# danielmtzbarba/carlabev-env

Hardware: NVIDIA B200
Metric: env-steps/sec (obs+reward+done) at N envs, 1/2/4/8 B200; % HBM roofline (higher is better)
Workload: dtype f64

## Files before the change

carlabev_env_b200/csrc/api.cu:

```cuda
#include <cuda.h>
#include <math.h>
#include <stdarg.h>
#include <stdio.h>
#include <stdlib.h>
#include <string.h>

#include <algorithm>
#include <chrono>
#include <cmath>
#include <new>
#include <random>
#include <vector>

#include "engine.h"

static thread_local char g_err[512] = "";

void cbev_set_error(const char* fmt, ...) {
  va_list ap;
  va_start(ap, fmt);
  vsnprintf(g_err, sizeof(g_err), fmt, ap);
  va_end(ap);
}

// ... 105 lines not shown
      cbev_set_error("cuTensorMapEncodeTiled failed with CUresult %d (map %dx%d, box %dx%d)", (int)r, e->map_w, e->map_h,
                     (int)box[0], (int)box[1]);
      return CBEV_ERR_CUDA;
    }
  }
  return CBEV_OK;
}

}

static int use_device(cbev_handle e) {
  if (!e) { cbev_set_error("null handle"); return CBEV_ERR_ARG; }
  int cur = -1;
  if (cudaGetDevice(&cur) != cudaSuccess || cur != e->device) CU_TRY(cudaSetDevice(e->device));
  return CBEV_OK;
}

static int install_pool(cbev_engine* e, PoolDev& d, const int32_t* actor_off_host, bool live) {
  const int n = d.n_scenes;
  const size_t na = (size_t)d.n_actors_total;
  const int max_retreat = d.max_retreat, max_tl = d.max_tl;
  int rc = 0;
  const size_t Rn = (size_t)(max_retreat ? max_retreat : 1), Ro = (size_t)(e->pool.max_retreat ? e->pool.max_retreat : 1);
  const int32_t new_max_rects = e->cfg.max_actors + CBEV_MAX_TARGETS + max_tl + 1;
  uint32_t* rects = nullptr;
  double* retreat = nullptr;
  int32_t* retreat_n = nullptr;
  const bool grow_rects = !e->rects || new_max_rects > e->max_rects;
  const bool grow_retreat = !e->st.retreat || !live || Rn != Ro;
  if (grow_rects) rc |= dev_alloc(&rects, (size_t)e->N * CBEV_RECT_WORDS * new_max_rects);
  if (grow_retreat) {
    rc |= dev_alloc(&retreat, (size_t)e->N * Rn * 3 * CBEV_SG_MAX);
    rc |= dev_alloc(&retreat_n, (size_t)e->N * Rn);
    if (!rc && live && e->st.retreat) {
      const size_t row_o = Ro * 3 * CBEV_SG_MAX * sizeof(double), row_n = Rn * 3 * CBEV_SG_MAX * sizeof(double);
      if (cudaMemcpy2D(retreat, row_n, e->st.retreat, row_o, row_o, (size_t)e->N, cudaMemcpyDeviceToDevice) != cudaSuccess ||
          cudaMemcpy2D(retreat_n, Rn * sizeof(int32_t), e->st.retreat_n, Ro * sizeof(int32_t), Ro * sizeof(int32_t),
                       (size_t)e->N, cudaMemcpyDeviceToDevice) != cudaSuccess) {
        cbev_set_error("copying the retreat routes failed");
        rc = CBEV_ERR_CUDA;
      }
    }
  }
  int T = live ? e->pool.traj_steps : e->cfg.trajectory_steps;
  if (!rc && T > 0 && na > 0) {
    const size_t budget = (size_t)4 << 30;
    if (!live) {
      while (T > 16 && (size_t)T * na * sizeof(double4) > budget) T /= 2;
    } else if ((size_t)T * na * sizeof(double4) > 2 * budget) {
      cbev_set_error("the extended pool needs %zu bytes of trajectory tables at the %d steps fixed by the first upload",
                     (size_t)T * na * sizeof(double4), T);
      rc = CBEV_ERR_NOMEM;
    }
    std::vector<long long> off((size_t)n);
    long long acc = 0;
    for (int s2 = 0; s2 < n; ++s2) {
      off[s2] = acc;
      acc += (long long)T * (actor_off_host[s2 + 1] - actor_off_host[s2]);
    }
    const size_t S = (size_t)n, A = (size_t)(e->cfg.max_actors > 0 ? e->cfg.max_actors : 1);
    EnvState& r = d.roll;
    if (!rc) {
      rc |= dev_upload(&d.traj_off, off.data(), S);
      rc |= dev_alloc(&d.traj, (size_t)acc);
      rc |= dev_alloc(&r.ax, S * A); rc |= dev_alloc(&r.ay, S * A); rc |= dev_alloc(&r.ayaw, S * A);
      rc |= dev_alloc(&r.av, S * A); rc |= dev_alloc(&r.atarget_mps, S * A); rc |= dev_alloc(&r.aelapsed, S * A);
      rc |= dev_alloc(&r.astate_elapsed, S * A); rc |= dev_alloc(&r.atidx, S * A); rc |= dev_alloc(&r.arxlen, S * A);
      rc |= dev_alloc(&r.aflags, S * A);
      rc |= dev_alloc(&r.retreat, S * Rn * 3 * CBEV_SG_MAX);
      rc |= dev_alloc(&r.retreat_n, S * Rn);
    }
    if (!rc) d.traj_steps = T;
  }
  if (rc) {
    free_pool(d);
    dev_free(rects); dev_free(retreat); dev_free(retreat_n);
    return rc;
  }
  free_pool(e->pool);
  e->pool = d;
  if (grow_rects) { dev_free(e->rects); e->rects = rects; e->max_rects = new_max_rects; }
  if (grow_retreat) { dev_free(e->st.retreat); dev_free(e->st.retreat_n); e->st.retreat = retreat; e->st.retreat_n = retreat_n; }
  e->has_pool = true;
  if (!live) e->pool_epoch += 1;
  if (e->pool.traj_steps > 0) {
    cbev_launch_rollout(e, 0);
    cudaError_t ce = cudaDeviceSynchronize();
    if (ce != cudaSuccess) {
      cbev_set_error("trajectory roll-out failed: %s", cudaGetErrorString(ce));
      e->has_pool = false;
      return CBEV_ERR_CUDA;
    }
  }
  return CBEV_OK;
}

extern "C" {

int cbev_version(void) { return CBEV_VERSION; }
const char* cbev_last_error(void) { return g_err; }

static void area_table(int ssize, int dsize, std::vector<int32_t>& off, std::vector<int32_t>& si,
                       std::vector<float>& alpha) {
  const double scale = (double)ssize / dsize;
  off.assign(1, 0);
  for (int dx = 0; dx < dsize; ++dx) {
    const double fsx1 = dx * scale, fsx2 = fsx1 + scale;
    const double cell = std::min(scale, ssize - fsx1);
    int sx1 = (int)std::ceil(fsx1), sx2 = (int)std::floor(fsx2);
    sx2 = std::min(sx2, ssize - 1);
    sx1 = std::min(sx1, sx2);
    if (sx1 - fsx1 > 1e-3) { si.push_back(sx1 - 1); alpha.push_back((float)((sx1 - fsx1) / cell)); }
    for (int sx = sx1; sx < sx2; ++sx) { si.push_back(sx); alpha.push_back((float)(1.0 / cell)); }
    if (fsx2 - sx2 > 1e-3) {
      si.push_back(sx2);
      alpha.push_back((float)(std::min(std::min(fsx2 - sx2, 1.0), cell) / cell));
    }
    off.push_back((int32_t)si.size());
  }
}

static void linear_area_table(int ssize, int dsize, std::vector<int32_t>& ofs, std::vector<int32_t>& a0,
                              std::vector<int32_t>& a1) {
  const double scale = (double)ssize / dsize, inv = 1.0 / scale;
  for (int dx = 0; dx < dsize; ++dx) {
    int sx = (int)std::floor(dx * scale);
    float fx = (float)((dx + 1) - (sx + 1) * inv);
    fx = fx <= 0 ? 0.f : fx - std::floor(fx);
    if (sx >= ssize - 1) { fx = 0.f; sx = ssize - 1; }
    ofs.push_back(sx);
    a0.push_back((int32_t)std::lrintf((1.f - fx) * 2048.f));
    a1.push_back((int32_t)std::lrintf(fx * 2048.f));
  }
}

static int build_resize_tables(cbev_engine* e) {
  const int S = e->cfg.fov_size, oh = e->cfg.obs_h, ow = e->cfg.obs_w;
  e->rs_words = 0;
  if (e->cfg.obs_mode == CBEV_OBS_RGB) { e->rs_mode = CBEV_RS_FAST96; return CBEV_OK; }
  if (oh > S || ow > S) {
    e->rs_mode = CBEV_RS_LINEAR;
    std::vector<int32_t> xo, xa0, xa1, yo, yb0, yb1, tab(2, 0);
    linear_area_table(S, ow, xo, xa0, xa1);
    linear_area_table(S, oh, yo, yb0, yb1);
    bool unit = true;
    for (size_t i = 0; i < xa0.size(); ++i) unit = unit && xa0[i] + xa1[i] == 2048;
    for (size_t i = 0; i < yb0.size(); ++i) unit = unit && yb0[i] + yb1[i] == 2048;
    tab[0] = unit ? 1 : 0;
    for (auto* v : {&xo, &yo, &xa0, &xa1, &yb0, &yb1}) tab.insert(tab.end(), v->begin(), v->end());
    e->rs_words = (int32_t)tab.size();
    return dev_upload(&e->rs_tab, tab.data(), tab.size());
  }
  if (S == 128 && oh == 96 && ow == 96) e->rs_mode = CBEV_RS_FAST96;
  else if (oh == S && ow == S) e->rs_mode = CBEV_RS_COPY;
  else if (2 * oh == S && 2 * ow == S) e->rs_mode = CBEV_RS_HALF;
  else e->rs_mode = CBEV_RS_TABLE;
  std::vector<int32_t> xo, yo, xs, ys;
  std::vector<float> xa, ya;
  area_table(S, ow, xo, xs, xa);
  area_table(S, oh, yo, ys, ya);
  std::vector<int32_t> tab;
  tab.push_back((int32_t)xs.size());
  tab.push_back((int32_t)ys.size());
  tab.insert(tab.end(), xo.begin(), xo.end());
  tab.insert(tab.end(), yo.begin(), yo.end());
  tab.insert(tab.end(), xs.begin(), xs.end());
  tab.insert(tab.end(), ys.begin(), ys.end());
  for (float a : xa) { int32_t b; memcpy(&b, &a, 4); tab.push_back(b); }
  for (float a : ya) { int32_t b; memcpy(&b, &a, 4); tab.push_back(b); }
  for (int d = 0; d < ow; ++d) tab.push_back(xs[xo[d]]);
  for (int d = 0; d < ow; ++d) tab.push_back(xs[xo[d + 1] - 1]);
  for (int d = 0; d < oh; ++d) tab.push_back(ys[yo[d]]);
  for (int d = 0; d < oh; ++d) tab.push_back(ys[yo[d + 1] - 1]);
  e->rs_words = (int32_t)tab.size();
  return dev_upload(&e->rs_tab, tab.data(), tab.size());
}

int cbev_create(const cbev_config* cfg, cbev_handle* out) {
  if (!cfg || !out) { cbev_set_error("null argument"); return CBEV_ERR_ARG; }
  *out = nullptr;
  if (cfg->num_envs < 1) { cbev_set_error("num_envs must be >= 1"); return CBEV_ERR_ARG; }
  if (cfg->fov_size != 64 && cfg->fov_size != 128 && cfg->fov_size != 256) {
    cbev_set_error("size must be 64, 128 or 256 (Town01 map scales the reference can reset on), got %d", cfg->fov_size);
    return CBEV_ERR_ARG;
  }
  if (cfg->obs_mode < 0 || cfg->obs_mode > 3) { cbev_set_error("bad obs_mode %d", cfg->obs_mode); return CBEV_ERR_ARG; }
  const bool masks = cfg->obs_mode == CBEV_OBS_SEMANTIC || cfg->obs_mode == CBEV_OBS_SEMANTIC_U8;
  if (cfg->obs_mode != CBEV_OBS_RGB) {
    const int px = cfg->obs_h * cfg->obs_w;
    const int mult = cfg->obs_mode == CBEV_OBS_SEMANTIC ? 4 : 16;
    if (cfg->obs_h < 8 || cfg->obs_w < 8 || cfg->obs_h > 256 || cfg->obs_w > 256 || px % mult != 0) {
      cbev_set_error("obs_size must be within 8..256 per side with height*width a multiple of %d (%s), got (%d, %d)",
                     mult, mult == 4 ? "float32 masks" : "16-byte stores of uint8 planes", cfg->obs_h, cfg->obs_w);
      return CBEV_ERR_ARG;
    }
  }
  if (masks && channels_of(cfg->mask_mode) < 0) { cbev_set_error("bad mask_mode %d", cfg->mask_mode); return CBEV_ERR_ARG; }
  if (cfg->frame_stack < 1) { cbev_set_error("frame_stack must be >= 1"); return CBEV_ERR_ARG; }
  if (!(cfg->anchor_x_frac >= 0.0 && cfg->anchor_x_frac <= 1.0 && cfg->anchor_y_frac >= 0.0 && cfg->anchor_y_frac <= 1.0)) {
    cbev_set_error("ego anchor fractions must be within [0, 1]");
    return CBEV_ERR_ARG;
  }
  const int F = cfg->obs_mode == CBEV_OBS_RGB ? 1 : cfg->frame_stack;
  if (F > 1 && cfg->ring_slots < 2 * F - 1) { cbev_set_error("ring_slots must be >= 2*frame_stack-1 (%d), got %d", 2 * F - 1, cfg->ring_slots); return CBEV_ERR_ARG; }
  if (F == 1 && cfg->ring_slots < 1) { cbev_set_error("ring_slots must be >= 1"); return CBEV_ERR_ARG; }
  if (cfg->action_mode == CBEV_ACTION_DISCRETE && (cfg->n_discrete < 1 || cfg->n_discrete > 16)) { cbev_set_error("n_discrete must be in [1, 16]"); return CBEV_ERR_ARG; }
  if (cfg->max_actors < 0) { cbev_set_error("max_actors must be >= 0"); return CBEV_ERR_ARG; }

  cbev_engine* e = new (std::nothrow) cbev_engine();
  if (!e) return CBEV_ERR_NOMEM;
  e->cfg = *cfg;
  e->cfg.frame_stack = F;
  if (F == 1) e->cfg.ring_slots = 1;
  e->N = cfg->num_envs;
  cudaGetDevice(&e->device);
  const int m = cfg->fov_size - 1;
  int ax = (int)nearbyint((double)m * cfg->anchor_x_frac), ay = (int)nearbyint((double)m * cfg->anchor_y_frac);
  ax = ax < 0 ? 0 : (ax > m ? m : ax);
  ay = ay < 0 ? 0 : (ay > m ? m : ay);
  e->anchor_x = ax;
  e->anchor_y = ay;
  int mx = ax > m - ax ? ax : m - ax, my = ay > m - ay ? ay : m - ay;
  int crop = (int)ceil(2.0 * hypot((double)mx, (double)my));
  if (crop < cfg->fov_size) crop = cfg->fov_size;
  e->crop = crop;
  e->pad = crop;
  {
    const int S = cfg->fov_size;
    const int win = (int)ceil(S * sqrt(2.0)) + 2;
    const int tile_h = (win + 7) & ~7;
    e->any_nby = (tile_h + 255) / 256;
    e->any_box_h = ((tile_h + e->any_nby - 1) / e->any_nby + 7) & ~7;
    e->any_nbx = (win + 15 + CBEV_ANY_BOX_W - 1) / CBEV_ANY_BOX_W;
    e->win_max = S == 128 ? CBEV_TILE_H : e->any_box_h * e->any_nby;
  }
  e->channels = masks ? channels_of(cfg->mask_mode) : 1;
  if (cfg->obs_mode == CBEV_OBS_SEMANTIC) e->frame_bytes = (int64_t)e->channels * cfg->obs_h * cfg->obs_w * 4;
  else if (cfg->obs_mode == CBEV_OBS_SEMANTIC_U8) e->frame_bytes = (int64_t)e->channels * cfg->obs_h * cfg->obs_w;
  else if (cfg->obs_mode == CBEV_OBS_GRAY) e->frame_bytes = (int64_t)cfg->obs_h * cfg->obs_w;
  else e->frame_bytes = (int64_t)cfg->fov_size * cfg->fov_size * 3;

  const size_t N = (size_t)e->N, A = (size_t)(cfg->max_actors > 0 ? cfg->max_actors : 1);
  int rc = 0;
  rc |= dev_alloc(&e->st.scene, N);
  rc |= dev_alloc(&e->st.episode, N);
  rc |= dev_alloc(&e->st.done, N);
  rc |= dev_alloc(&e->st.ego, N * 24);
  rc |= dev_alloc(&e->st.egoi, N * 8);
  rc |= dev_alloc(&e->st.tgt_vis, N * CBEV_TGT_WORDS);
  rc |= dev_alloc(&e->st.stats, N * 12);
  rc |= dev_alloc(&e->st.ax, N * A);
  rc |= dev_alloc(&e->st.ay, N * A);
  rc |= dev_alloc(&e->st.ayaw, N * A);
  rc |= dev_alloc(&e->st.av, N * A);
  rc |= dev_alloc(&e->st.atarget_mps, N * A);
  rc |= dev_alloc(&e->st.aelapsed, N * A);
  rc |= dev_alloc(&e->st.astate_elapsed, N * A);
  rc |= dev_alloc(&e->st.atidx, N * A);
  rc |= dev_alloc(&e->st.arxlen, N * A);
  rc |= dev_alloc(&e->st.aflags, N * A);
  rc |= dev_alloc(&e->desc, N * CBEV_DESC_WORDS);
  rc |= dev_alloc(&e->order, N);
  rc |= dev_alloc(&e->order_cnt, (size_t)2);
  rc |= dev_alloc(&e->move_order, N);
  rc |= dev_alloc(&e->move_cnt, (size_t)2);
  rc |= dev_alloc(&e->fov, N * (size_t)cfg->fov_size * cfg->fov_size);
  rc |= dev_alloc(&e->gstats, (size_t)CBEV_STATS_FIELDS);
  rc |= build_resize_tables(e);
  rc |= dev_alloc((uint8_t**)&e->h_reward_dev, N * 10);
  e->h_term_dev = (uint8_t*)e->h_reward_dev + N * 8;
  e->h_trunc_dev = e->h_term_dev + N;
  rc |= dev_alloc((uint8_t**)&e->h_actions_dev, N * 16);
  if (rc) { cbev_destroy(e); return rc; }
  cudaMemset(e->st.scene, 0xff, N * sizeof(int32_t));
  {
    uint64_t z = (uint64_t)std::chrono::steady_clock::now().time_since_epoch().count() ^ (uint64_t)(uintptr_t)e;
    try {
      std::random_device rd;
      z ^= ((uint64_t)rd() << 32) | (uint64_t)rd();
    } catch (...) {
    }
    z += 0x9E3779B97F4A7C15ull;
    z = (z ^ (z >> 30)) * 0xBF58476D1CE4E5B9ull;
    z = (z ^ (z >> 27)) * 0x94D049BB133111EBull;
    e->token = z ^ (z >> 31);
  }
  *out = e;
  return CBEV_OK;
}

int cbev_destroy(cbev_handle e) {
  if (!e) return CBEV_OK;
  use_device(e);
  free_pool(e->pool);
  free_state(e->st);
  free_state(e->branch);
  dev_free(e->br_stage_desc); dev_free(e->br_stage_rects); dev_free(e->br_desc); dev_free(e->br_rects);
  dev_free(e->br_window);
  dev_free(e->fov_mask); dev_free(e->rs_tab); dev_free(e->trace);
  dev_free(e->order); dev_free(e->order_cnt); dev_free(e->move_order); dev_free(e->move_cnt);
  dev_free(e->map); dev_free(e->desc); dev_free(e->rects); dev_free(e->fov); dev_free(e->gstats);
  dev_free(e->h_reward_dev);
  { uint8_t* p = (uint8_t*)e->h_actions_dev; dev_free(p); }
  if (e->side_stream) cudaStreamDestroy(e->side_stream);
  if (e->ev_sim) cudaEventDestroy(e->ev_sim);
  if (e->ev_copy) cudaEventDestroy(e->ev_copy);
  if (e->ev_judge) cudaEventDestroy(e->ev_judge);
  if (e->prof_ev) {
    for (int i = 0; i < CBEV_PROF_EVENTS * CBEV_PROF_MAX; ++i) cudaEventDestroy(e->prof_ev[i]);
    delete[] e->prof_ev;
  }
  delete e;
  return CBEV_OK;
}

int cbev_upload_map(cbev_handle e, const uint8_t* cls_host, int32_t w, int32_t h_px) {
  if (!e || !cls_host) { cbev_set_error("null argument"); return CBEV_ERR_ARG; }
  { int rc0 = use_device(e); if (rc0) return rc0; }
  if (w < 16 || h_px < 16 || (w % 16) != 0) { cbev_set_error("map width must be a multiple of 16 (TMA row pitch), got %dx%d", w, h_px); return CBEV_ERR_ARG; }
  for (size_t i = 0; i < (size_t)w * h_px; ++i)
    if (cls_host[i] > 2) { cbev_set_error("map classes must be 0 (non-drivable), 1 (drivable) or 2 (sidewalk)"); return CBEV_ERR_ARG; }
  dev_free(e->map);
  int rc = dev_upload(&e->map, cls_host, (size_t)w * h_px);
  if (rc) return rc;
  e->map_w = w;
  e->map_h = h_px;
  rc = build_tensor_map(e);
  if (rc) return rc;
  e->has_map = true;
  return CBEV_OK;
}

int cbev_upload_scene_pool(cbev_handle e, const cbev_pool_desc* p) {
  if (!e || !p) { cbev_set_error("null argument"); return CBEV_ERR_ARG; }
  { int rc0 = use_device(e); if (rc0) return rc0; }
  if (p->n_scenes < 1) { cbev_set_error("scene pool is empty"); return CBEV_ERR_ARG; }
  const int n = p->n_scenes;
  int max_actors = 0, max_targets = 0, max_tl = 0, max_retreat = 0;
  std::vector<int32_t> slots((size_t)(p->n_actors_total > 0 ? p->n_actors_total : 1), -1);
  for (int s = 0; s < n; ++s) {
    int nt = p->ego_off[s + 1] - p->ego_off[s];
    if (nt < 2 || nt > CBEV_MAX_TARGETS) { cbev_set_error("scene %d: ego route has %d points, supported range is [2, %d]", s, nt, CBEV_MAX_TARGETS); return CBEV_ERR_ARG; }
    if (p->ego_tidx0[s] < 0 || p->ego_tidx0[s] >= nt) { cbev_set_error("scene %d: ego target index out of range", s); return CBEV_ERR_ARG; }
    int a0 = p->actor_off[s], a1 = p->actor_off[s + 1];
    if (a1 < a0 || a1 > p->n_actors_total) { cbev_set_error("scene %d: bad actor offsets", s); return CBEV_ERR_ARG; }
    int nret = 0;
    bool seen_ped = false;
    for (int a = a0; a < a1; ++a) {
      if (p->act_kind[a] > 1) { cbev_set_error("scene %d: bad actor kind", s); return CBEV_ERR_ARG; }
      if (p->act_kind[a] == 1) seen_ped = true;
      else if (seen_ped) { cbev_set_error("scene %d: vehicles must precede pedestrians (draw / collision order)", s); return CBEV_ERR_ARG; }
      int np = p->act_route_off[a + 1] - p->act_route_off[a];
      if (np < 2) { cbev_set_error("scene %d: actor route needs >= 2 points", s); return CBEV_ERR_ARG; }
      if (p->act_beh[a] > CBEV_BEH_STOP_RETURN) { cbev_set_error("scene %d: unknown behaviour id %d", s, p->act_beh[a]); return CBEV_ERR_ARG; }
      if (p->act_beh[a] == CBEV_BEH_STOP_RETURN) {
        if (!p->sg_mat) { cbev_set_error("scene %d: StopReturn behaviour needs sg_mat (retreat smoothing operators)", s); return CBEV_ERR_ARG; }
        int nr = p->act_raw_off[a + 1] - p->act_raw_off[a];
        if (nr + 1 > CBEV_SG_MAX) { cbev_set_error("scene %d: retreat route of %d points exceeds CBEV_SG_MAX", s, nr + 1); return CBEV_ERR_ARG; }
        slots[a] = nret++;
      }
    }
    if (a1 - a0 > max_actors) max_actors = a1 - a0;
    if (nt > max_targets) max_targets = nt;
    int ntl = p->tl_off[s + 1] - p->tl_off[s];
    if (ntl > max_tl) max_tl = ntl;
    if (nret > max_retreat) max_retreat = nret;
  }
  if (max_actors > e->cfg.max_actors) { cbev_set_error("pool has scenes with %d actors but the engine was created with max_actors=%d", max_actors, e->cfg.max_actors); return CBEV_ERR_ARG; }

  const bool live = e->was_reset && e->has_pool;
  if (live) {
    if (n < e->pool.n_scenes) { cbev_set_error("a pool uploaded while environments are running must extend the previous one (%d scenes < %d)", n, e->pool.n_scenes); return CBEV_ERR_ARG; }
    CU_TRY(cudaDeviceSynchronize());
    if (max_retreat < e->pool.max_retreat) max_retreat = e->pool.max_retreat;
  }
  PoolDev d;
  d.n_scenes = n;
  d.n_actors_total = p->n_actors_total;
  d.max_actors = max_actors;
  d.max_targets = max_targets;
  d.max_tl = max_tl;
  d.max_retreat = max_retreat;
  const size_t na = (size_t)p->n_actors_total, nr = (size_t)p->ego_off[n], nq = (size_t)p->rew_off[n];
  const size_t npts = na ? (size_t)p->act_route_off[na] : 0, nraw = na ? (size_t)p->act_raw_off[na] : 0;
  const size_t ntl = (size_t)p->tl_off[n];
  int rc = 0;
  rc |= dev_upload(&d.ego_state0, p->ego_state0, (size_t)n * 4);
  rc |= dev_upload(&d.ego_target_speed, p->ego_target_speed, (size_t)n);
  rc |= dev_upload(&d.len_ego_route, p->len_ego_route, (size_t)n);
  rc |= dev_upload(&d.ego_tidx0, p->ego_tidx0, (size_t)n);
  rc |= dev_upload(&d.num_vehicles, p->num_vehicles, (size_t)n);
  rc |= dev_upload(&d.ego_off, p->ego_off, (size_t)n + 1);
  rc |= dev_upload(&d.rew_off, p->rew_off, (size_t)n + 1);
  rc |= dev_upload(&d.actor_off, p->actor_off, (size_t)n + 1);
  rc |= dev_upload(&d.tl_off, p->tl_off, (size_t)n + 1);
  rc |= dev_upload(&d.ego_cx, p->ego_cx, nr);
  rc |= dev_upload(&d.ego_cy, p->ego_cy, nr);
  rc |= dev_upload(&d.ego_cyaw, p->ego_cyaw, nr);
  rc |= dev_upload(&d.rew_rx, p->rew_rx, nq);
  rc |= dev_upload(&d.rew_ry, p->rew_ry, nq);
  rc |= dev_upload(&d.rew_cum, p->rew_cum, nq);
  rc |= dev_upload(&d.act_kind, p->act_kind, na);
  rc |= dev_upload(&d.act_beh, p->act_beh, na);
  rc |= dev_upload(&d.act_state0, p->act_state0, na * 4);
  rc |= dev_upload(&d.act_cruise_px, p->act_cruise_px, na);
  rc |= dev_upload(&d.act_cruise_mps, p->act_cruise_mps, na);
  rc |= dev_upload(&d.act_beh_p, p->act_beh_p, na * 4);
  rc |= dev_upload(&d.act_tidx0, p->act_tidx0, na);
  rc |= dev_upload(&d.act_route_off, p->act_route_off, na + 1);
// ... 83 lines not shown
    cbev_launch_generate(e, d, kinds_d, levels_d, seeds_d, att_d, 0);
    cudaError_t ce = cudaDeviceSynchronize();
    if (ce == cudaSuccess) ce = cudaMemcpy(att.data(), att_d, (size_t)n * sizeof(int32_t), cudaMemcpyDeviceToHost);
    if (ce != cudaSuccess) { cbev_set_error("scene generation failed: %s", cudaGetErrorString(ce)); rc = CBEV_ERR_CUDA; }
  }
  dev_free(kinds_d); dev_free(levels_d); dev_free(seeds_d); dev_free(att_d);
  if (!rc)
    for (int s = 0; s < n; ++s)
      if (att[s] < 0) {
        cbev_set_error("Failed to reset into a valid initial state after 10 attempts (scene %d, seed %lld)", s, (long long)seeds[s]);
        rc = CBEV_ERR_ARG;
        break;
      }
  if (attempts_host) memcpy(attempts_host, att.data(), (size_t)n * sizeof(int32_t));
  if (rc) { free_pool(d); return rc; }
  return install_pool(e, d, actor_off.data(), live);
}

int cbev_pool_counts(cbev_handle e, int32_t counts[8]) {
  if (!e || !counts) { cbev_set_error("null argument"); return CBEV_ERR_ARG; }
  { int rc0 = use_device(e); if (rc0) return rc0; }
  if (!e->has_pool) { cbev_set_error("no scene pool"); return CBEV_ERR_STATE; }
  const PoolDev& d = e->pool;
  int32_t last[5] = {0, 0, 0, 0, 0};
  const int n = d.n_scenes, na = d.n_actors_total;
  CU_TRY(cudaMemcpy(&last[0], d.ego_off + n, 4, cudaMemcpyDeviceToHost));
  CU_TRY(cudaMemcpy(&last[1], d.rew_off + n, 4, cudaMemcpyDeviceToHost));
  CU_TRY(cudaMemcpy(&last[2], d.tl_off + n, 4, cudaMemcpyDeviceToHost));
  if (na) {
    CU_TRY(cudaMemcpy(&last[3], d.act_route_off + na, 4, cudaMemcpyDeviceToHost));
    CU_TRY(cudaMemcpy(&last[4], d.act_raw_off + na, 4, cudaMemcpyDeviceToHost));
  }
  counts[0] = n; counts[1] = na; counts[2] = last[0]; counts[3] = last[1]; counts[4] = last[3]; counts[5] = last[4];
  counts[6] = last[2]; counts[7] = d.traj_steps;
  return CBEV_OK;
}

int cbev_read_scene_pool(cbev_handle e, const cbev_pool_desc* dst) {
  if (!e || !dst) { cbev_set_error("null argument"); return CBEV_ERR_ARG; }
  { int rc0 = use_device(e); if (rc0) return rc0; }
  if (!e->has_pool) { cbev_set_error("no scene pool"); return CBEV_ERR_STATE; }
  int32_t c[8];
  int rc = cbev_pool_counts(e, c);
  if (rc) return rc;
  const PoolDev& d = e->pool;
  const size_t n = (size_t)c[0], na = (size_t)c[1], nr = (size_t)c[2], nq = (size_t)c[3], np = (size_t)c[4], nw = (size_t)c[5],
               ntl = (size_t)c[6];
#define RD(field, count)                                                                                          \
  if (dst->field && (count))                                                                                      \
    CU_TRY(cudaMemcpy((void*)dst->field, d.field, (count) * sizeof(*d.field), cudaMemcpyDeviceToHost));
  RD(ego_state0, n * 4) RD(ego_target_speed, n) RD(ego_tidx0, n) RD(len_ego_route, n) RD(num_vehicles, n)
  RD(ego_off, n + 1) RD(rew_off, n + 1) RD(actor_off, n + 1) RD(tl_off, n + 1)
  RD(ego_cx, nr) RD(ego_cy, nr) RD(ego_cyaw, nr) RD(rew_rx, nq) RD(rew_ry, nq) RD(rew_cum, nq)
  RD(act_kind, na) RD(act_state0, na * 4) RD(act_tidx0, na) RD(act_cruise_px, na) RD(act_cruise_mps, na)
  RD(act_beh, na) RD(act_beh_p, na * 4) RD(act_route_off, na + 1) RD(act_raw_off, na + 1)
  RD(act_cx, np) RD(act_cy, np) RD(act_cyaw, np) RD(act_raw_x, nw) RD(act_raw_y, nw) RD(tl_rect, ntl * 4) RD(tl_color, ntl)
#undef RD
  return CBEV_OK;
}

int64_t cbev_frame_bytes(cbev_handle e) { return e ? e->frame_bytes : -1; }

int cbev_bind_obs_ring(cbev_handle e, void* ring_dev, int64_t bytes) {
  if (!e || !ring_dev) { cbev_set_error("null argument"); return CBEV_ERR_ARG; }
  { int rc0 = use_device(e); if (rc0) return rc0; }
  int64_t need = (int64_t)e->N * e->cfg.ring_slots * e->frame_bytes;
  if (bytes < need) { cbev_set_error("observation ring needs %lld bytes, got %lld", (long long)need, (long long)bytes); return CBEV_ERR_ARG; }
  if (((uintptr_t)ring_dev & 15) != 0) { cbev_set_error("observation ring must be 16-byte aligned"); return CBEV_ERR_ARG; }
  e->ring = ring_dev;
  e->ring_bytes = bytes;
  return CBEV_OK;
}

static int check_ready(cbev_handle e, bool need_reset) {
  if (!e) { cbev_set_error("null handle"); return CBEV_ERR_ARG; }
  { int rc0 = use_device(e); if (rc0) return rc0; }
  if (!e->has_map) { cbev_set_error("no map uploaded (cbev_upload_map)"); return CBEV_ERR_STATE; }
  if (!e->has_pool) { cbev_set_error("no scene pool uploaded (cbev_upload_scene_pool)"); return CBEV_ERR_STATE; }
  if (!e->ring) { cbev_set_error("no observation ring bound (cbev_bind_obs_ring)"); return CBEV_ERR_STATE; }
  if (need_reset && !e->was_reset) { cbev_set_error("step() called before reset()"); return CBEV_ERR_STATE; }
  return CBEV_OK;
}

int cbev_reset(cbev_handle e, const uint8_t* mask_dev, const int32_t* scene_ids_dev, void* stream) {
  int rc = check_ready(e, false);
  if (rc) return rc;
  if (!scene_ids_dev) { cbev_set_error("scene_ids is required"); return CBEV_ERR_ARG; }
  if (mask_dev && !e->was_reset) { cbev_set_error("the first reset must cover every env (mask = NULL)"); return CBEV_ERR_STATE; }
  cudaStream_t s = (cudaStream_t)stream;
  const int F = e->cfg.frame_stack, L = e->cfg.ring_slots;
  if (e->head < 0) e->head = F - 1;
  cbev_launch_reset(e, mask_dev, scene_ids_dev, s);
  if ((rc = debug_sync("k_reset", s))) return rc;
  if (cbev_launch_render(e, e->head, F > 1 ? L - F + 1 : 0, s)) return CBEV_ERR_CUDA;
  if ((rc = debug_sync("k_render (reset frame)", s))) return rc;
  CU_TRY(cudaGetLastError());
  e->was_reset = true;
  return CBEV_OK;
}

static int ensure_side_stream(cbev_engine* e) {
  if (e->side_stream) return CBEV_OK;
  int lo = 0, hi = 0;
  CU_TRY(cudaDeviceGetStreamPriorityRange(&lo, &hi));
  CU_TRY(cudaStreamCreateWithPriority(&e->side_stream, cudaStreamNonBlocking, hi));
  CU_TRY(cudaEventCreateWithFlags(&e->ev_sim, cudaEventDisableTiming));
  CU_TRY(cudaEventCreateWithFlags(&e->ev_judge, cudaEventDisableTiming));
  CU_TRY(cudaEventCreateWithFlags(&e->ev_copy, cudaEventDisableTiming));
  return CBEV_OK;
}

int cbev_step_ex(cbev_handle e, const void* actions_dev, const cbev_step_out* out, const cbev_host_out* host, void* stream);

int cbev_step(cbev_handle e, const void* actions_dev, const cbev_step_out* out, void* stream) {
  return cbev_step_ex(e, actions_dev, out, nullptr, stream);
}

int cbev_step_ex(cbev_handle e, const void* actions_dev, const cbev_step_out* out, const cbev_host_out* host,
                 void* stream) {
  int rc = check_ready(e, true);
  if (rc) return rc;
  if (!actions_dev || !out || !out->reward || !out->terminated || !out->truncated) { cbev_set_error("actions, reward, terminated and truncated are required"); return CBEV_ERR_ARG; }
  if (host && (!host->reward || !host->terminated || !host->truncated)) { cbev_set_error("null host buffer"); return CBEV_ERR_ARG; }
  if ((rc = ensure_side_stream(e))) return rc;
  cudaStream_t s = (cudaStream_t)stream;
  const int F = e->cfg.frame_stack, L = e->cfg.ring_slots;
  int head = e->head + 1;
  if (head >= L) head = F - 1;
  const int mirror = F > 1 ? L - F + 1 : 0;
  const bool prof = e->profiling && e->prof_n < CBEV_PROF_MAX;
  cudaEvent_t* pe = prof ? e->prof_ev + CBEV_PROF_EVENTS * e->prof_n : nullptr;
  if (prof) cudaEventRecord(pe[0], s);
  cbev_launch_move(e, actions_dev, out, s);
  if (prof) cudaEventRecord(pe[1], s);
  if ((rc = debug_sync("k_move", s))) return rc;
  cudaStream_t js = (e->debug_flags & CBEV_DBG_JUDGE_SERIAL) ? s : e->side_stream;
  if (js != s) {
    CU_TRY(cudaEventRecord(e->ev_sim, s));
    CU_TRY(cudaStreamWaitEvent(js, e->ev_sim, 0));
  }
  if (prof) cudaEventRecord(pe[3], js);
  cbev_launch_judge(e, out, js);
  if (prof) cudaEventRecord(pe[4], js);
  if ((rc = debug_sync("k_judge", js))) return rc;
  if (host) {
    const size_t N = (size_t)e->N;
    const cbev_host_out* ho = host;
    const bool packed_dev = out->terminated == (uint8_t*)out->reward + N * 8 && out->truncated == out->terminated + N;
    const bool packed_host = ho->terminated == (uint8_t*)ho->reward + N * 8 && ho->truncated == ho->terminated + N;
    if (packed_dev && packed_host) {
      CU_TRY(cudaMemcpyAsync(ho->reward, out->reward, N * 10, cudaMemcpyDeviceToHost, js));
    } else {
      CU_TRY(cudaMemcpyAsync(ho->reward, out->reward, N * 8, cudaMemcpyDeviceToHost, js));
      CU_TRY(cudaMemcpyAsync(ho->terminated, out->terminated, N, cudaMemcpyDeviceToHost, js));
      CU_TRY(cudaMemcpyAsync(ho->truncated, out->truncated, N, cudaMemcpyDeviceToHost, js));
    }
    if (ho->cause && out->cause) CU_TRY(cudaMemcpyAsync(ho->cause, out->cause, N, cudaMemcpyDeviceToHost, js));
    if (ho->episode && out->episode)
      CU_TRY(cudaMemcpyAsync(ho->episode, out->episode, N * CBEV_EPISODE_FIELDS * sizeof(double), cudaMemcpyDeviceToHost,
                             js));
    CU_TRY(cudaEventRecord(e->ev_copy, js));
    e->host_copy_pending = true;
  }
  CU_TRY(cudaEventRecord(e->ev_judge, js));
  if (cbev_launch_render(e, head, mirror, s)) return CBEV_ERR_CUDA;
  if (prof) { cudaEventRecord(pe[2], s); e->prof_n += 1; }
  if ((rc = debug_sync("k_render", s))) return rc;
  CU_TRY(cudaStreamWaitEvent(s, e->ev_judge, 0));
  CU_TRY(cudaGetLastError());
  e->head = head;
  e->steps += 1;
  return CBEV_OK;
}

int cbev_step_host_ex(cbev_handle e, const void* actions_host, const cbev_step_out* dev_out, const cbev_host_out* host,
                      void* stream) {
  int rc = check_ready(e, true);
  if (rc) return rc;
  if (!actions_host || !host || !host->reward || !host->terminated || !host->truncated) { cbev_set_error("null host buffer"); return CBEV_ERR_ARG; }
  cudaStream_t s = (cudaStream_t)stream;
  const size_t N = (size_t)e->N;
  const size_t abytes = e->cfg.action_mode == CBEV_ACTION_DISCRETE ? N * 8 : N * 12;
  CU_TRY(cudaMemcpyAsync(e->h_actions_dev, actions_host, abytes, cudaMemcpyHostToDevice, s));
  cbev_step_out out;
  if (dev_out) {
    out = *dev_out;
  } else {
    memset(&out, 0, sizeof(out));
    out.reward = e->h_reward_dev;
    out.terminated = e->h_term_dev;
    out.truncated = e->h_trunc_dev;
  }
  return cbev_step_ex(e, e->h_actions_dev, &out, host, stream);
}

int cbev_step_host(cbev_handle e, const void* actions_host, double* reward_host, uint8_t* terminated_host,
                   uint8_t* truncated_host, void* stream) {
  cbev_host_out host;
  memset(&host, 0, sizeof(host));
  host.reward = reward_host;
  host.terminated = terminated_host;
  host.truncated = truncated_host;
  return cbev_step_host_ex(e, actions_host, nullptr, &host, stream);
}

int cbev_invalidate(cbev_handle e) {
  if (!e) { cbev_set_error("null handle"); return CBEV_ERR_ARG; }
  { int rc0 = use_device(e); if (rc0) return rc0; }
  CU_TRY(cudaDeviceSynchronize());
  e->was_reset = false;
  e->pool_epoch += 1;
  return CBEV_OK;
}

int64_t cbev_snapshot_row_bytes(cbev_handle e) { return e ? cbev_snap_layout(e, e->pool.max_retreat).row_bytes : -1; }

static int check_snapshot_args(cbev_handle e, const void* rows_mem, int32_t n, const char* what) {
  int rc = check_ready(e, false);
  if (rc) return rc;
  if (!e->was_reset) { cbev_set_error("%s before the first reset (or after cbev_invalidate): no env state", what); return CBEV_ERR_STATE; }
  if (n < 1 || n > e->N) { cbev_set_error("%s: n must be within 1..%d (num_envs), got %d", what, e->N, n); return CBEV_ERR_ARG; }
  if (((uintptr_t)rows_mem & 15) != 0) { cbev_set_error("%s: snapshot rows must be 16-byte aligned", what); return CBEV_ERR_ARG; }
  return CBEV_OK;
// ... 199 lines not shown
    if (si->row_bytes != src.L.row_bytes) {
      cbev_set_error("%s: src row_bytes %lld does not match the %lld of this engine at %d retreat slots", what,
                     (long long)si->row_bytes, (long long)src.L.row_bytes, si->retreat_slots);
      return CBEV_ERR_ARG;
    }
    if (si->n_rows < 1 || (!io->roots && n_branches > si->n_rows)) {
      cbev_set_error("%s: with NULL roots branch b starts from row b, so n_branches must be <= %d (src n_rows), got %d",
                     what, si->n_rows, n_branches);
      return CBEV_ERR_ARG;
    }
    src.rows = io->src_rows;
    src.n_rows = si->n_rows;
  }
  const int64_t win_bytes = (int64_t)n_branches * e->cfg.frame_stack * e->frame_bytes;
  if (io->obs) {
    if (((uintptr_t)io->obs & 15) != 0) { cbev_set_error("%s: obs must be 16-byte aligned", what); return CBEV_ERR_ARG; }
    if (io->obs_bytes < win_bytes) {
      cbev_set_error("%s: obs holds %lld bytes, %d leaf windows of %d frames need %lld", what,
                     (long long)io->obs_bytes, n_branches, e->cfg.frame_stack, (long long)win_bytes);
      return CBEV_ERR_ARG;
    }
  }
  const int64_t row_bytes = cbev_snap_layout(e, e->pool.max_retreat).row_bytes;
  if (io->leaf_rows) {
    if (!io->leaf_info) { cbev_set_error("%s: leaf_info is required with leaf_rows", what); return CBEV_ERR_ARG; }
    if (((uintptr_t)io->leaf_rows & 15) != 0) { cbev_set_error("%s: leaf_rows must be 16-byte aligned", what); return CBEV_ERR_ARG; }
    if (io->leaf_bytes < (int64_t)n_branches * row_bytes) {
      cbev_set_error("%s: leaf_rows holds %lld bytes, %d leaf rows need %lld (%lld per row)", what,
                     (long long)io->leaf_bytes, n_branches, (long long)n_branches * row_bytes, (long long)row_bytes);
      return CBEV_ERR_ARG;
    }
  }
  const bool frames = io->obs || io->leaf_rows;
  if (frames && !out->steps) { cbev_set_error("%s: out->steps is required with obs or leaf_rows (the window copy reads it)", what); return CBEV_ERR_ARG; }
  if (frames && !e->ring) { cbev_set_error("%s: no observation ring bound (cbev_bind_obs_ring)", what); return CBEV_ERR_STATE; }
  if ((rc = check_ready(e, false))) return rc;
  if (!e->was_reset) { cbev_set_error("%s before the first reset (or after cbev_invalidate): no env state", what); return CBEV_ERR_STATE; }
  if ((rc = ensure_branch_state(e, n_branches))) return rc;
  if (frames && (rc = ensure_branch_render(e, n_branches))) return rc;
  if (io->leaf_rows && !io->obs && (rc = ensure_branch_window(e, win_bytes))) return rc;
  cudaStream_t s = (cudaStream_t)stream;
  const RowSource* sp = si ? &src : nullptr;
  void* win = io->obs ? io->obs : (io->leaf_rows ? (void*)e->br_window : nullptr);
  cbev_launch_lookahead(e, io->roots, n_branches, horizon, actions_dev, gamma, out, frames, sp, io->leaf_rows != nullptr,
                        s);
  if ((rc = debug_sync("k_lookahead_ex", s))) return rc;
  if (frames) {
    if (cbev_launch_render_branches(e, n_branches * e->cfg.frame_stack, win, s)) return CBEV_ERR_CUDA;
    if ((rc = debug_sync("k_render (leaf windows)", s))) return rc;
    cbev_launch_leaf_window(e, io->roots, n_branches, out->steps, win, sp, s);
    if ((rc = debug_sync("k_leaf_window", s))) return rc;
  }
  if (io->leaf_rows) {
    cbev_launch_leaf_rows(e, n_branches, win, io->leaf_rows, s);
    if ((rc = debug_sync("k_leaf_rows", s))) return rc;
  }
  CU_TRY(cudaGetLastError());
  if (io->leaf_rows) {
    cbev_snapshot_info* li = io->leaf_info;
    memset(li, 0, sizeof(*li));
    li->engine_token = e->token;
    li->pool_epoch = e->pool_epoch;
    li->retreat_slots = e->pool.max_retreat;
    li->row_bytes = row_bytes;
    li->n_rows = n_branches;
  }
  return CBEV_OK;
}

int cbev_wait_host_outputs(cbev_handle e) {
  if (!e) { cbev_set_error("null handle"); return CBEV_ERR_ARG; }
  { int rc0 = use_device(e); if (rc0) return rc0; }
  if (!e->host_copy_pending) return CBEV_OK;
  CU_TRY(cudaEventSynchronize(e->ev_copy));
  e->host_copy_pending = false;
  return CBEV_OK;
}

int cbev_upload_fov_mask(cbev_handle e, const uint8_t* mask_host) {
  if (!e) { cbev_set_error("null handle"); return CBEV_ERR_ARG; }
  { int rc0 = use_device(e); if (rc0) return rc0; }
  CU_TRY(cudaDeviceSynchronize());
  dev_free(e->fov_mask);
  if (!mask_host) return CBEV_OK;
  const size_t n = (size_t)e->cfg.fov_size * e->cfg.fov_size;
  std::vector<uint8_t> m(n);
  for (size_t i = 0; i < n; ++i) m[i] = mask_host[i] ? 0xff : 0x00;
  return dev_upload(&e->fov_mask, m.data(), n);
}

static int check_fuse_mode(cbev_handle e, int32_t mode) {
  if (mode != CBEV_FUSE_VEHICLE_TEMPORAL && mode != CBEV_FUSE_VEHICLE_WEIGHTED) { cbev_set_error("bad fusion mode %d", mode); return CBEV_ERR_ARG; }
  if (e->cfg.obs_mode != CBEV_OBS_SEMANTIC && e->cfg.obs_mode != CBEV_OBS_SEMANTIC_U8) { cbev_set_error("temporal_fusion_mode requires obs_mode='bev_semantic'"); return CBEV_ERR_ARG; }
  if (e->cfg.frame_stack < 3) { cbev_set_error("temporal_fusion_mode requires frame_stack >= 3"); return CBEV_ERR_ARG; }
  return CBEV_OK;
}

int cbev_fuse(cbev_handle e, int32_t mode, void* out_dev, void* stream) {
  int rc = check_ready(e, true);
  if (rc) return rc;
  if (!out_dev) { cbev_set_error("null output"); return CBEV_ERR_ARG; }
  if ((rc = check_fuse_mode(e, mode))) return rc;
  if (cbev_launch_fuse(e, mode, e->ring, e->N, e->cfg.ring_slots, e->head, out_dev, (cudaStream_t)stream)) {
    cbev_set_error("temporal_fusion_mode requires a semantic_mask_ch with a vehicle channel");
    return CBEV_ERR_ARG;
  }
  CU_TRY(cudaGetLastError());
  return CBEV_OK;
}

int cbev_fuse_windows(cbev_handle e, int32_t mode, const void* windows_dev, int32_t n, void* out_dev, void* stream) {
  if (!e) { cbev_set_error("null handle"); return CBEV_ERR_ARG; }
  if (!windows_dev || !out_dev) { cbev_set_error("cbev_fuse_windows: null windows or output"); return CBEV_ERR_ARG; }
  if ((((uintptr_t)windows_dev | (uintptr_t)out_dev) & 15) != 0) { cbev_set_error("cbev_fuse_windows: windows and output must be 16-byte aligned"); return CBEV_ERR_ARG; }
  if (n < 1) { cbev_set_error("cbev_fuse_windows: n must be >= 1, got %d", n); return CBEV_ERR_ARG; }
  int rc = check_fuse_mode(e, mode);
  if (rc) return rc;
  { int rc0 = use_device(e); if (rc0) return rc0; }
  const int F = e->cfg.frame_stack;
  if (cbev_launch_fuse(e, mode, windows_dev, n, F, F - 1, out_dev, (cudaStream_t)stream)) {
    cbev_set_error("temporal_fusion_mode requires a semantic_mask_ch with a vehicle channel");
    return CBEV_ERR_ARG;
  }
  CU_TRY(cudaGetLastError());
  return CBEV_OK;
}

int cbev_obs_head(cbev_handle e, int32_t* head) {
  if (!e || !head) { cbev_set_error("null argument"); return CBEV_ERR_ARG; }
  *head = e->head;
  return CBEV_OK;
}

int cbev_get_state(cbev_handle e, double* ego_host, double* actors_host) {
  if (!e) { cbev_set_error("null handle"); return CBEV_ERR_ARG; }
  { int rc0 = use_device(e); if (rc0) return rc0; }
  CU_TRY(cudaDeviceSynchronize());
  const size_t N = (size_t)e->N, A = (size_t)(e->cfg.max_actors > 0 ? e->cfg.max_actors : 1);
  if (ego_host) {
    std::vector<double> eg(N * 24);
    std::vector<int32_t> ei(N * 8);
    std::vector<unsigned long long> tv(N * CBEV_TGT_WORDS);
    CU_TRY(cudaMemcpy(eg.data(), e->st.ego, N * 24 * 8, cudaMemcpyDeviceToHost));
    CU_TRY(cudaMemcpy(ei.data(), e->st.egoi, N * 8 * 4, cudaMemcpyDeviceToHost));
    CU_TRY(cudaMemcpy(tv.data(), e->st.tgt_vis, N * CBEV_TGT_WORDS * 8, cudaMemcpyDeviceToHost));
    for (size_t i = 0; i < N; ++i) {
      double* o = ego_host + i * 16;
      for (int k = 0; k < 9; ++k) o[k] = eg[i * 24 + k];
      o[9] = (double)ei[i * 8 + 0];
      o[10] = eg[i * 24 + 9];
      o[11] = eg[i * 24 + 10];
      o[12] = eg[i * 24 + 11];
      o[13] = eg[i * 24 + 12];
      o[14] = (double)(uint32_t)(tv[i * CBEV_TGT_WORDS] & 0xffffffffull);
      o[15] = (double)(uint32_t)(tv[i * CBEV_TGT_WORDS] >> 32);
    }
  }
  if (actors_host) {
    std::vector<double> x(N * A), y(N * A), yaw(N * A), v(N * A), tm(N * A);
    std::vector<int32_t> ti(N * A);
    std::vector<uint8_t> fl(N * A);
    CU_TRY(cudaMemcpy(x.data(), e->st.ax, N * A * 8, cudaMemcpyDeviceToHost));
    CU_TRY(cudaMemcpy(y.data(), e->st.ay, N * A * 8, cudaMemcpyDeviceToHost));
    CU_TRY(cudaMemcpy(yaw.data(), e->st.ayaw, N * A * 8, cudaMemcpyDeviceToHost));
    CU_TRY(cudaMemcpy(v.data(), e->st.av, N * A * 8, cudaMemcpyDeviceToHost));
    CU_TRY(cudaMemcpy(tm.data(), e->st.atarget_mps, N * A * 8, cudaMemcpyDeviceToHost));
// ... 1 lines not shown
    CU_TRY(cudaMemcpy(fl.data(), e->st.aflags, N * A, cudaMemcpyDeviceToHost));
    for (size_t i = 0; i < N * A; ++i) {
      double* o = actors_host + i * 8;
      o[0] = x[i]; o[1] = y[i]; o[2] = yaw[i]; o[3] = v[i]; o[4] = (double)ti[i]; o[5] = (double)(fl[i] & 15);
      o[6] = tm[i]; o[7] = (double)fl[i];
    }
  }
  return CBEV_OK;
}

int cbev_set_ego_state(cbev_handle e, const double* ego_host) {
  if (!e || !ego_host) { cbev_set_error("null argument"); return CBEV_ERR_ARG; }
  { int rc0 = use_device(e); if (rc0) return rc0; }
  CU_TRY(cudaDeviceSynchronize());
  const size_t N = (size_t)e->N;
  std::vector<double> eg(N * 24);
  std::vector<int32_t> ei(N * 8);
  CU_TRY(cudaMemcpy(eg.data(), e->st.ego, N * 24 * 8, cudaMemcpyDeviceToHost));
  CU_TRY(cudaMemcpy(ei.data(), e->st.egoi, N * 8 * 4, cudaMemcpyDeviceToHost));
  for (size_t i = 0; i < N; ++i) {
    const double* o = ego_host + i * 16;
    for (int k = 0; k < 9; ++k) eg[i * 24 + k] = o[k];
    ei[i * 8 + 0] = (int32_t)o[9];
  }
  CU_TRY(cudaMemcpy(e->st.ego, eg.data(), N * 24 * 8, cudaMemcpyHostToDevice));
  CU_TRY(cudaMemcpy(e->st.egoi, ei.data(), N * 8 * 4, cudaMemcpyHostToDevice));
  return CBEV_OK;
}

int cbev_set_state(cbev_handle e, const double* ego_host, const double* actors_host) {
  if (!e) { cbev_set_error("null handle"); return CBEV_ERR_ARG; }
  { int rc0 = use_device(e); if (rc0) return rc0; }
  if (ego_host) {
    int rc = cbev_set_ego_state(e, ego_host);
    if (rc) return rc;
  }
  if (actors_host) {
    CU_TRY(cudaDeviceSynchronize());
    const size_t N = (size_t)e->N, A = (size_t)(e->cfg.max_actors > 0 ? e->cfg.max_actors : 1);
    std::vector<double> x(N * A), y(N * A), yaw(N * A), v(N * A), tm(N * A);
    std::vector<int32_t> ti(N * A);
    std::vector<uint8_t> fl(N * A);
    for (size_t i = 0; i < N * A; ++i) {
      const double* o = actors_host + i * 8;
      x[i] = o[0]; y[i] = o[1]; yaw[i] = o[2]; v[i] = o[3];
      ti[i] = (int32_t)o[4];
      tm[i] = o[6];
      fl[i] = (uint8_t)(((int)o[7] & ~15) | ((int)o[5] & 15));
    }
    CU_TRY(cudaMemcpy(e->st.ax, x.data(), N * A * 8, cudaMemcpyHostToDevice));
    CU_TRY(cudaMemcpy(e->st.ay, y.data(), N * A * 8, cudaMemcpyHostToDevice));
    CU_TRY(cudaMemcpy(e->st.ayaw, yaw.data(), N * A * 8, cudaMemcpyHostToDevice));
    CU_TRY(cudaMemcpy(e->st.av, v.data(), N * A * 8, cudaMemcpyHostToDevice));
    CU_TRY(cudaMemcpy(e->st.atarget_mps, tm.data(), N * A * 8, cudaMemcpyHostToDevice));
    CU_TRY(cudaMemcpy(e->st.atidx, ti.data(), N * A * 4, cudaMemcpyHostToDevice));
    CU_TRY(cudaMemcpy(e->st.aflags, fl.data(), N * A, cudaMemcpyHostToDevice));
  }
  return CBEV_OK;
}

int cbev_set_debug_flags(cbev_handle e, int32_t flags) {
  if (!e) { cbev_set_error("null handle"); return CBEV_ERR_ARG; }
  if (flags & ~CBEV_DBG_KNOWN) {
    cbev_set_error("unknown debug flags 0x%x (accepted bits: 1, 2, 4, 32, 128, 256, 512)",
                   (unsigned)(flags & ~CBEV_DBG_KNOWN));
    return CBEV_ERR_ARG;
  }
  e->debug_flags = flags;
  if ((flags & CBEV_DBG_TRACE) && !e->trace) return dev_alloc(&e->trace, (size_t)e->N * 8);
  return CBEV_OK;
}

int cbev_debug_read_trace(cbev_handle e, uint64_t* host_out) {
  if (!e || !host_out) { cbev_set_error("null argument"); return CBEV_ERR_ARG; }
  { int rc0 = use_device(e); if (rc0) return rc0; }
  if (!e->trace) { cbev_set_error("tracing is off (set debug flag 4 first)"); return CBEV_ERR_STATE; }
  CU_TRY(cudaDeviceSynchronize());
  CU_TRY(cudaMemcpy(host_out, e->trace, (size_t)e->N * 8 * sizeof(uint64_t), cudaMemcpyDeviceToHost));
  return CBEV_OK;
}

int cbev_keep_fov(cbev_handle e, int32_t on) {
  if (!e) { cbev_set_error("null handle"); return CBEV_ERR_ARG; }
  e->keep_fov = on != 0;
  return CBEV_OK;
}

int cbev_copy_fov(cbev_handle e, uint8_t* fov_dev, void* stream) {
  if (!e || !fov_dev) { cbev_set_error("null argument"); return CBEV_ERR_ARG; }
  { int rc0 = use_device(e); if (rc0) return rc0; }
  if (!e->keep_fov) { cbev_set_error("palette frames are not kept: call cbev_keep_fov(h, 1) before stepping"); return CBEV_ERR_STATE; }
  size_t bytes = (size_t)e->N * e->cfg.fov_size * e->cfg.fov_size;
  CU_TRY(cudaMemcpyAsync(fov_dev, e->fov, bytes, cudaMemcpyDeviceToDevice, (cudaStream_t)stream));
  return CBEV_OK;
}

int cbev_read_stats(cbev_handle e, double* stats_dev, int32_t reset_after, void* stream) {
  if (!e || !stats_dev) { cbev_set_error("null argument"); return CBEV_ERR_ARG; }
  { int rc0 = use_device(e); if (rc0) return rc0; }
  cudaStream_t s = (cudaStream_t)stream;
  CU_TRY(cudaMemcpyAsync(stats_dev, e->gstats, CBEV_STATS_FIELDS * sizeof(double), cudaMemcpyDeviceToDevice, s));
  double steps = (double)e->steps * (double)e->N;
  CU_TRY(cudaMemcpyAsync(stats_dev + CBEV_S_STEPS, &steps, sizeof(double), cudaMemcpyHostToDevice, s));
  CU_TRY(cudaStreamSynchronize(s));
  if (reset_after) {
    CU_TRY(cudaMemsetAsync(e->gstats, 0, CBEV_STATS_FIELDS * sizeof(double), s));
    e->steps = 0;
  }
  return CBEV_OK;
}

int64_t cbev_launch_count(cbev_handle e) { return e ? e->launches : -1; }

int cbev_profile_enable(cbev_handle e, int32_t on) {
  if (!e) { cbev_set_error("null handle"); return CBEV_ERR_ARG; }
  { int rc0 = use_device(e); if (rc0) return rc0; }
  if (on && !e->prof_ev) {
    e->prof_ev = new (std::nothrow) cudaEvent_t[CBEV_PROF_EVENTS * CBEV_PROF_MAX];
    if (!e->prof_ev) return CBEV_ERR_NOMEM;
    for (int i = 0; i < CBEV_PROF_EVENTS * CBEV_PROF_MAX; ++i) CU_TRY(cudaEventCreate(&e->prof_ev[i]));
  }
  e->profiling = on != 0;
  e->prof_n = 0;
  return CBEV_OK;
}

int cbev_profile_read_ex(cbev_handle e, double* move_ms, double* render_ms, double* judge_ms, int64_t* steps) {
  if (!e || !move_ms || !render_ms || !judge_ms || !steps) { cbev_set_error("null argument"); return CBEV_ERR_ARG; }
  { int rc0 = use_device(e); if (rc0) return rc0; }
  double a = 0.0, b = 0.0, c = 0.0;
  if (e->prof_n > 0) CU_TRY(cudaDeviceSynchronize());
  for (int i = 0; i < e->prof_n; ++i) {
    const cudaEvent_t* pe = e->prof_ev + CBEV_PROF_EVENTS * i;
    float t0 = 0.f, t1 = 0.f, t2 = 0.f;
    CU_TRY(cudaEventElapsedTime(&t0, pe[0], pe[1]));
    CU_TRY(cudaEventElapsedTime(&t1, pe[1], pe[2]));
    CU_TRY(cudaEventElapsedTime(&t2, pe[3], pe[4]));
    a += t0;
    b += t1;
    c += t2;
  }
  *move_ms = a;
  *render_ms = b;
  *judge_ms = c;
  *steps = e->prof_n;
  e->prof_n = 0;
  return CBEV_OK;
}

int cbev_profile_read(cbev_handle e, double* sim_ms, double* render_ms, int64_t* steps) {
  double judge = 0.0;
  return cbev_profile_read_ex(e, sim_ms, render_ms, &judge, steps);
}

int cbev_abi_sizes(int32_t* config_bytes, int32_t* pool_desc_bytes, int32_t* step_out_bytes) {
  if (config_bytes) *config_bytes = (int32_t)sizeof(cbev_config);
  if (pool_desc_bytes) *pool_desc_bytes = (int32_t)sizeof(cbev_pool_desc);
  if (step_out_bytes) *step_out_bytes = (int32_t)sizeof(cbev_step_out);
  return CBEV_OK;
}

}
```

carlabev_env_b200/csrc/engine.h:

```cpp
#pragma once
#include <cuda_runtime.h>
#include <stdint.h>

#include "../../include/cbev.h"

#define CBEV_TGT_WORDS 2
#define CBEV_MAX_TARGETS (64 * CBEV_TGT_WORDS)
#define CBEV_RECT_WORDS 2
#define CBEV_DESC_WORDS 20
#define CBEV_TILE_H 184
#define CBEV_TILE_W 208
#define CBEV_WARPS_PER_BLOCK 4
#define CBEV_PROF_MAX 2048
#define CBEV_PROF_EVENTS 5

enum {
  RD_OX = 0,
  RD_OY,
  RD_MODE,
  RD_TURNS,
  RD_NX, RD_NY, RD_ISIN, RD_ICOS, RD_AX, RD_AY, RD_XD, RD_YD, RD_CY,
  RD_NRECTS,
  RD_FLAGS,
  RD_FX, RD_FY,
  RD_BG
};

struct EnvState {
  int32_t* scene = nullptr;
  int32_t* episode = nullptr;
  uint8_t* done = nullptr;
  double* ego = nullptr;
  int32_t* egoi = nullptr;
  unsigned long long* tgt_vis = nullptr;
  double* stats = nullptr;
  double *ax = nullptr, *ay = nullptr, *ayaw = nullptr, *av = nullptr, *atarget_mps = nullptr;
  double *aelapsed = nullptr, *astate_elapsed = nullptr;
  int32_t *atidx = nullptr, *arxlen = nullptr;
  uint8_t* aflags = nullptr;
  double* retreat = nullptr;
  int32_t* retreat_n = nullptr;
};

#define CBEV_STATE_SECTIONS 16
struct StateSections {
  void** field[CBEV_STATE_SECTIONS];
  int32_t esize[CBEV_STATE_SECTIONS], count[CBEV_STATE_SECTIONS];
};
inline StateSections cbev_state_sections(EnvState& st, int32_t A, int32_t R) {
  return StateSections{
      {(void**)&st.ego, (void**)&st.egoi, (void**)&st.tgt_vis, (void**)&st.stats, (void**)&st.ax, (void**)&st.ay,
       (void**)&st.ayaw, (void**)&st.av, (void**)&st.atarget_mps, (void**)&st.aelapsed, (void**)&st.astate_elapsed,
       (void**)&st.atidx, (void**)&st.arxlen, (void**)&st.aflags, (void**)&st.retreat, (void**)&st.retreat_n},
      {8, 4, 8, 8, 8, 8, 8, 8, 8, 8, 8, 4, 4, 1, 8, 4},
      {24, 8, CBEV_TGT_WORDS, 12, A, A, A, A, A, A, A, A, A, A, R * 3 * CBEV_SG_MAX, R}};
}

__device__ __forceinline__ void cbev_copy_elem(uint8_t* d, const uint8_t* s, int es) {
  if (es == 8) *(uint64_t*)d = *(const uint64_t*)s;
  else if (es == 4) *(uint32_t*)d = *(const uint32_t*)s;
  else *d = *s;
}
__device__ __forceinline__ void cbev_zero_elem(uint8_t* d, int es) {
  if (es == 8) *(uint64_t*)d = 0;
  else if (es == 4) *(uint32_t*)d = 0;
  else *d = 0;
}

struct PoolDev {
  int32_t n_scenes = 0, n_actors_total = 0, max_actors = 0, max_targets = 0, max_tl = 0, max_retreat = 0;
  double *ego_state0 = nullptr, *ego_target_speed = nullptr, *len_ego_route = nullptr;
  int32_t *ego_tidx0 = nullptr, *num_vehicles = nullptr;
  int32_t *ego_off = nullptr, *rew_off = nullptr, *actor_off = nullptr, *tl_off = nullptr;
  double *ego_cx = nullptr, *ego_cy = nullptr, *ego_cyaw = nullptr;
  int32_t *rew_rx = nullptr, *rew_ry = nullptr;
  double* rew_cum = nullptr;
  uint8_t *act_kind = nullptr, *act_beh = nullptr;
  double *act_state0 = nullptr, *act_cruise_px = nullptr, *act_cruise_mps = nullptr, *act_beh_p = nullptr;
  int32_t *act_tidx0 = nullptr, *act_route_off = nullptr, *act_raw_off = nullptr;
  int32_t* act_retreat_slot = nullptr;
  double *act_cx = nullptr, *act_cy = nullptr, *act_cyaw = nullptr, *act_raw_x = nullptr, *act_raw_y = nullptr;
  int32_t* tl_rect = nullptr;
  uint8_t* tl_color = nullptr;
  double* sg_mat = nullptr;
  int32_t traj_steps = 0;
  double4* traj = nullptr;
  long long* traj_off = nullptr;
  EnvState roll;
};

struct SimParams {
  int32_t N, max_actors, max_rects, max_retreat;
  int32_t map_w, map_h, fov, crop, pad, anchor_x, anchor_y;
  int32_t hero_w, win_max;
  float hero_scale;
  int32_t action_mode, n_discrete, reward_mode, autoreset;
  uint64_t seed;
  const uint8_t* map;
  float discrete_table[16 * 3];
  cbev_config cfg;
};

#define CBEV_RS_FAST96 0
#define CBEV_RS_TABLE 1
#define CBEV_RS_HALF 2
#define CBEV_RS_COPY 3
#define CBEV_RS_LINEAR 4
#define CBEV_ANY_BOX_W 128

enum {
  CBEV_DBG_GENERIC_ROTATE = 1,
  CBEV_DBG_JUDGE_SERIAL = 2,
  CBEV_DBG_TRACE = 4,
  CBEV_DBG_IDENTITY_RENDER_ORDER = 32,
  CBEV_DBG_IDENTITY_MOVE_ORDER = 128,
  CBEV_DBG_RENDER_ANY = 256,
  CBEV_DBG_NO_BLOCK83 = 512,
  CBEV_DBG_KNOWN = CBEV_DBG_GENERIC_ROTATE | CBEV_DBG_JUDGE_SERIAL | CBEV_DBG_TRACE | CBEV_DBG_IDENTITY_RENDER_ORDER |
                   CBEV_DBG_IDENTITY_MOVE_ORDER | CBEV_DBG_RENDER_ANY | CBEV_DBG_NO_BLOCK83
};

struct cbev_engine {
  cbev_config cfg;
  int device = 0;
  int32_t N = 0, crop = 0, pad = 0, anchor_x = 0, anchor_y = 0;
  int32_t map_w = 0, map_h = 0;
  uint8_t* map = nullptr;
  alignas(64) unsigned char tmap[128];
  alignas(64) unsigned char tmap_any[128];
  int32_t win_max = 0;
  int32_t any_nbx = 0, any_nby = 0, any_box_h = 0;
  bool has_map = false, has_pool = false, was_reset = false, keep_fov = false;
  PoolDev pool;
  EnvState st;
  int32_t max_rects = 0;
  int32_t debug_flags = 0;
  int32_t* desc = nullptr;
  uint32_t* rects = nullptr;
  int32_t* order = nullptr;
  int32_t* order_cnt = nullptr;
  int32_t* move_order = nullptr;
  int32_t* move_cnt = nullptr;
  uint8_t* fov = nullptr;
  unsigned long long* trace = nullptr;
  int32_t rs_mode = 0, rs_words = 0;
  int32_t* rs_tab = nullptr;
  uint8_t* fov_mask = nullptr;
  void* ring = nullptr;
  int64_t ring_bytes = 0, frame_bytes = 0;
  int32_t channels = 0;
  int32_t head = -1;
  double* gstats = nullptr;
  void* h_actions_dev = nullptr;
  double* h_reward_dev = nullptr;
  uint8_t *h_term_dev = nullptr, *h_trunc_dev = nullptr;
  cudaStream_t side_stream = nullptr;
  cudaEvent_t ev_sim = nullptr, ev_copy = nullptr, ev_judge = nullptr;
  bool host_copy_pending = false;
  int64_t launches = 0;
  int64_t steps = 0;
  bool profiling = false;
  cudaEvent_t* prof_ev = nullptr;
  int32_t prof_n = 0;
  uint64_t token = 0;
  int32_t pool_epoch = 0;
  EnvState branch;
  int32_t branch_rows = 0, branch_retreat = 0;
  uint8_t* br_window = nullptr;
  int64_t br_window_bytes = 0;
  int32_t* br_stage_desc = nullptr;
  uint32_t* br_stage_rects = nullptr;
  int32_t* br_desc = nullptr;
  uint32_t* br_rects = nullptr;
  int32_t br_rows = 0, br_max_rects = 0;
};

struct SnapLayout {
  int64_t off[CBEV_STATE_SECTIONS];
  int32_t esize[CBEV_STATE_SECTIONS], count[CBEV_STATE_SECTIONS];
  int64_t frames_off, row_bytes;
};
SnapLayout cbev_snap_layout(const cbev_engine* e, int32_t retreat_slots);
struct RowSource {
  SnapLayout L;
  const void* rows;
  int32_t n_rows;
};

void cbev_launch_reset(cbev_engine* e, const uint8_t* mask, const int32_t* scene_ids, cudaStream_t s);
void cbev_launch_move(cbev_engine* e, const void* actions, const cbev_step_out* out, cudaStream_t s);
void cbev_launch_judge(cbev_engine* e, const cbev_step_out* out, cudaStream_t s);
int cbev_launch_render(cbev_engine* e, int32_t head, int32_t mirror, cudaStream_t s);
void cbev_set_error(const char* fmt, ...);
int cbev_launch_fuse(cbev_engine* e, int32_t mode, const void* ring, int32_t n, int32_t L, int32_t head, void* out,
                     cudaStream_t s);
int cbev_launch_render_branches(cbev_engine* e, int32_t n, void* windows, cudaStream_t s);
void cbev_launch_rollout(cbev_engine* e, cudaStream_t s);
void cbev_launch_generate(cbev_engine* e, const PoolDev& pool, const uint8_t* kinds, const int32_t* levels,
                          const long long* seeds, int32_t* attempts, cudaStream_t s);
void cbev_launch_snapshot(cbev_engine* e, const int32_t* env_ids, int32_t n, void* dst, cudaStream_t s);
void cbev_launch_restore(cbev_engine* e, const SnapLayout& L, const void* src, int32_t n_rows, const int32_t* rows,
                         const int32_t* env_ids, int32_t n, cudaStream_t s);
void cbev_launch_lookahead(cbev_engine* e, const int32_t* roots, int32_t n_branches, int32_t horizon,
                           const void* actions, double gamma, const cbev_lookahead_out* out, bool record,
                           const RowSource* src, bool leaf, cudaStream_t s);
void cbev_launch_leaf_window(cbev_engine* e, const int32_t* roots, int32_t n_branches, const int32_t* steps,
                             void* windows, const RowSource* src, cudaStream_t s);
void cbev_launch_leaf_rows(cbev_engine* e, int32_t n_branches, const void* windows, void* dst, cudaStream_t s);
```

carlabev_env_b200/csrc/render.cu:

```cuda
#include <cuda.h>
#include <stdlib.h>

#include <type_traits>

#include "engine.h"

namespace {

constexpr int RT = 256;

__constant__ uint32_t c_pal_rg[CBEV_PAL_COUNT];
__constant__ uint32_t c_pal_b[CBEV_PAL_COUNT];
__constant__ uint32_t c_pal_key[CBEV_PAL_COUNT];
__constant__ uint8_t c_chan_mask[6][CBEV_PAL_COUNT + 1];

__device__ __forceinline__ uint32_t smem_u32(const void* p) { return (uint32_t)__cvta_generic_to_shared(p); }

__device__ __forceinline__ void mbar_init(uint64_t* bar, int count) {
  asm volatile("mbarrier.init.shared::cta.b64 [%0], %1;" ::"r"(smem_u32(bar)), "r"(count));
}
__device__ __forceinline__ void mbar_expect_tx(uint64_t* bar, uint32_t bytes) {
  asm volatile("mbarrier.arrive.expect_tx.shared::cta.b64 _, [%0], %1;" ::"r"(smem_u32(bar)), "r"(bytes) : "memory");
}
__device__ __forceinline__ void mbar_wait(uint64_t* bar, uint32_t parity) {
  asm volatile(
      "{\n"
      ".reg .pred p;\n"
      "WAIT_%=:\n"
      "mbarrier.try_wait.parity.shared::cta.b64 p, [%0], %1;\n"
      "@p bra DONE_%=;\n"
      "bra WAIT_%=;\n"
      "DONE_%=:\n"
      "}\n" ::"r"(smem_u32(bar)),
      "r"(parity)
      : "memory");
}
__device__ __forceinline__ void tma_load_2d(void* dst, const CUtensorMap* tmap, int x, int y, uint64_t* bar) {
  asm volatile(
      "cp.async.bulk.tensor.2d.shared::cluster.global.mbarrier::complete_tx::bytes [%0], [%1, {%3, %4}], [%2];" ::"r"(
          smem_u32(dst)),
      "l"(tmap), "r"(smem_u32(bar)), "r"(x), "r"(y)
      : "memory");
}
__device__ __forceinline__ void st_f4(float* p, float a, float b, float c, float d) {
  asm volatile("st.global.cs.v4.f32 [%0], {%1, %2, %3, %4};" ::"l"(p), "f"(a), "f"(b), "f"(c), "f"(d) : "memory");
}
__device__ __forceinline__ uint32_t bit_to_f32(uint32_t m, int pos) {
  int32_t s;
  asm("bfe.s32 %0, %1, %2, 1;" : "=r"(s) : "r"(m), "r"(pos));
  return (uint32_t)s & 0x3f800000u;
}
__device__ __forceinline__ void st_b4(void* p, uint32_t a, uint32_t b, uint32_t c, uint32_t d) {
  asm volatile("st.global.cs.v4.b32 [%0], {%1, %2, %3, %4};" ::"l"(p), "r"(a), "r"(b), "r"(c), "r"(d) : "memory");
}
__device__ __forceinline__ void st_u4(void* p, uint4 v) {
  asm volatile("st.global.cs.v4.u32 [%0], {%1, %2, %3, %4};" ::"l"(p), "r"(v.x), "r"(v.y), "r"(v.z), "r"(v.w)
               : "memory");
}

struct RenderParams {
  int32_t N, fov, crop, anchor_x, anchor_y;
  int32_t frame_stack, ring_slots, head, mirror;
  int64_t frame_bytes;
  int32_t generic_rotate;
  int32_t blk83;
  int32_t list_cap;
  const int32_t* desc;
  const uint32_t* rects;
  const int32_t* order;
  int32_t* order_cnt;
  int32_t max_rects;
  uint8_t* fov_out;
  const uint8_t* fov_mask;
  void* ring;
  int32_t obs_h, obs_w, rs_mode, rs_words;
  const int32_t* rs_tab;
  unsigned long long* trace;
  int32_t hero_w;
  int32_t nbx, nby, box_h, region_bytes;
};

__device__ __forceinline__ void trace_mark(const RenderParams& P, int env, int slot) {
  if (P.trace != nullptr && threadIdx.x == 0) {
    unsigned long long t;
    asm volatile("mov.u64 %0, %%globaltimer;" : "=l"(t));
    P.trace[(size_t)env * 8 + slot] = t;
    if (slot == 0) {
      unsigned sm;
      asm volatile("mov.u32 %0, %%smid;" : "=r"(sm));
      P.trace[(size_t)env * 8 + 6] = sm;
    }
  }
}

__device__ __forceinline__ uint32_t round_half_even_16(uint32_t s) {
  uint32_t q = s >> 4, r = s & 15u;
  return q + ((r > 8u) || (r == 8u && (q & 1u)));
}

__device__ __forceinline__ uint32_t blend_rgb(uint32_t c00, uint32_t c01, uint32_t c10, uint32_t c11, uint32_t wx0,
                                              uint32_t wx1, uint32_t wy0, uint32_t wy1, const uint32_t* s_rg,
                                              const uint32_t* s_b) {
  uint32_t rg = wy0 * (wx0 * s_rg[c00] + wx1 * s_rg[c01]) + wy1 * (wx0 * s_rg[c10] + wx1 * s_rg[c11]);
  uint32_t b = wy0 * (wx0 * s_b[c00] + wx1 * s_b[c01]) + wy1 * (wx0 * s_b[c10] + wx1 * s_b[c11]);
  uint32_t R = round_half_even_16(rg & 0xffffu), G = round_half_even_16(rg >> 16), B = round_half_even_16(b);
  return R | (G << 8) | (B << 16);
}

template <int OBS_MODE>
__device__ __forceinline__ uint32_t resolve_px(uint32_t c00, uint32_t c01, uint32_t c10, uint32_t c11, uint32_t wx0,
                                               uint32_t wx1, uint32_t wy0, uint32_t wy1, const uint32_t* s_rg,
                                               const uint32_t* s_b, const uint32_t* s_key, const uint8_t* s_cm) {
  const bool same = c00 == c01 && c00 == c10 && c00 == c11;
  if (OBS_MODE == CBEV_OBS_SEMANTIC) {
    uint32_t cls = c00;
    if (!same) {
      const uint32_t key = blend_rgb(c00, c01, c10, c11, wx0, wx1, wy0, wy1, s_rg, s_b);
      cls = CBEV_PAL_COUNT;
#pragma unroll
      for (int q = 0; q < CBEV_PAL_TL_YELLOW; ++q) cls = (key == s_key[q]) ? q : cls;
    }
    return s_cm[cls];
  }
  const uint32_t key = same ? s_key[c00] : blend_rgb(c00, c01, c10, c11, wx0, wx1, wy0, wy1, s_rg, s_b);
  const double g = __dadd_rn(__dadd_rn(__dmul_rn((double)(key & 255u), 0.2125),
                                       __dmul_rn((double)((key >> 8) & 255u), 0.7154)),
                             __dmul_rn((double)(key >> 16), 0.0721));
  return (uint32_t)(int)g & 255u;
}

template <int OBS_MODE>
__device__ __forceinline__ uint32_t classify_key(uint32_t key, const uint32_t* s_key, const uint8_t* s_cm) {
  if (OBS_MODE == CBEV_OBS_SEMANTIC) {
    uint32_t cls = CBEV_PAL_COUNT;
#pragma unroll
    for (int q = 0; q < CBEV_PAL_TL_YELLOW; ++q) cls = (key == s_key[q]) ? q : cls;
    return s_cm[cls];
  }
  const double g = __dadd_rn(__dadd_rn(__dmul_rn((double)(key & 255u), 0.2125),
                                       __dmul_rn((double)((key >> 8) & 255u), 0.7154)),
                             __dmul_rn((double)(key >> 16), 0.0721));
  return (uint32_t)(int)g & 255u;
}

template <int CHANNELS>
__device__ __forceinline__ void store_u8_planes(uint8_t* base, const uint8_t* s_out, int plane, int tid, int nt) {
  for (int q = tid; q < plane / 16; q += nt) {
    const uint4 m = ((const uint4*)s_out)[q];
#pragma unroll
    for (int c = 0; c < CHANNELS; ++c)
      st_u4(base + (size_t)c * plane + 16 * q,
            make_uint4((m.x >> c) & 0x01010101u, (m.y >> c) & 0x01010101u, (m.z >> c) & 0x01010101u,
                       (m.w >> c) & 0x01010101u));
  }
}

__device__ __forceinline__ int fov_word(int row, int cw) { return row * 32 + ((((cw >> 2) ^ row) & 7) << 2) + (cw & 3); }
__device__ __forceinline__ int fov_byte(int row, int x) { return row * 128 + ((((x >> 4) ^ row) & 7) << 4) + (x & 15); }

template <int OBS_MODE, int CHANNELS, bool U8 = false>
__global__ void __launch_bounds__(RT, 4)
k_render(RenderParams P, const __grid_constant__ CUtensorMap tmap, int mask_mode) {
  extern __shared__ __align__(128) uint8_t smem[];
  constexpr int S = 128;
  constexpr int pitch = CBEV_TILE_W;
  constexpr int tile_bytes = CBEV_TILE_W * CBEV_TILE_H;
  uint8_t* s_tile = smem;
  uint8_t* const s_region = smem;
  uint8_t* s_fov = smem + tile_bytes;
  uint32_t* s_rg = (uint32_t*)(s_fov + S * S);
  uint32_t* s_b = s_rg + 16;
  uint32_t* s_key = s_b + 16;
  int32_t* s_desc = (int32_t*)(s_key + 16);
  uint64_t* s_bar = (uint64_t*)(s_desc + CBEV_DESC_WORDS);
  uint8_t* s_cm = (uint8_t*)(s_bar + 2);
  int* s_count = (int*)(s_cm + 16);
  uint32_t* s_rects = (uint32_t*)(s_count + 4);

  const int env = P.order != nullptr ? P.order[blockIdx.x] : blockIdx.x;
  const int tid = threadIdx.x;
  const int lane = tid & 31, warp = tid >> 5;
  if (blockIdx.x == 0 && tid < 2 && P.order_cnt != nullptr) P.order_cnt[tid] = 0;
  const int32_t* d = P.desc + (size_t)env * CBEV_DESC_WORDS;
  const int flags = d[RD_FLAGS];
  if (flags & 2) return;
  trace_mark(P, env, 0);

  if (tid == 0) {
    mbar_init(s_bar, 1);
    asm volatile("fence.mbarrier_init.release.cluster;" ::: "memory");
    mbar_expect_tx(s_bar, (uint32_t)tile_bytes);
    tma_load_2d(s_tile, &tmap, d[RD_OX] & ~15, d[RD_OY], s_bar);
    *s_count = 0;
  }
  if (tid < CBEV_DESC_WORDS) s_desc[tid] = d[tid];
  if (tid < CBEV_PAL_COUNT) {
    s_rg[tid] = c_pal_rg[tid];
    s_b[tid] = c_pal_b[tid];
    s_key[tid] = c_pal_key[tid];
  }
  if (tid <= CBEV_PAL_COUNT) s_cm[tid] = c_chan_mask[mask_mode][tid];
  const int nrects = d[RD_NRECTS];
  {
    const uint32_t* rl = P.rects + (size_t)env * P.max_rects * CBEV_RECT_WORDS;
    for (int r = tid; r < P.max_rects * CBEV_RECT_WORDS; r += RT) s_rects[r] = rl[r];
  }
  __syncthreads();
  mbar_wait(s_bar, 0);
  s_tile += s_desc[RD_OX] & 15;
  trace_mark(P, env, 1);

  if (nrects > 0) {
    int r = 0;
    while (r < nrects) {
      const uint32_t pal = s_rects[2 * r + 1] >> 24;
      int e = r;
      for (;;) {
        const int idx = e + lane;
        const unsigned same = __ballot_sync(0xffffffffu, idx < nrects && (s_rects[2 * idx + 1] >> 24) == pal);
        if (same == 0xffffffffu) { e += 32; continue; }
        e += __ffs(~same) - 1;
        break;
      }
      for (int q = r + tid; q < e; q += RT) {
        const uint32_t w0 = s_rects[2 * q], w1 = s_rects[2 * q + 1];
        const int x0 = w0 & 0xffff, y0 = w0 >> 16, w = (w1 & 0xfff) + 1, h = ((w1 >> 12) & 0xfff) + 1;
        uint8_t* row = s_tile + y0 * pitch + x0;
        for (int yy = 0; yy < h; ++yy, row += pitch)
          for (int xx = 0; xx < w; ++xx) row[xx] = (uint8_t)pal;
      }
      r = e;
      __syncthreads();
    }
    trace_mark(P, env, 7);
  }

  trace_mark(P, env, 2);
// ... 33 lines not shown
          uint32_t pk = 0;
#pragma unroll
          for (int k = 0; k < 4; ++k) {
            pk |= (uint32_t)tile0[(dy >> 16) * pitch + (dx >> 16)] << (8 * k);
            dx += icos;
            dy += isin;
          }
          packed[g] = pk;
        }
#pragma unroll
        for (int g = 0; g < 4; ++g) {
          const int p = warp * 16 + i0 + g;
          fov32[fov_word((p >> 3) * 8 + ly, (p & 7) * 4 + lx)] = packed[g];
        }
      }
    } else if (fast) {
      int base, stepx, stepy;
      if (turns == 0) { base = 0; stepx = 1; stepy = pitch; }
      else if (turns == 1) { base = crop - 1; stepx = pitch; stepy = -1; }
      else if (turns == 2) { base = (crop - 1) * pitch + crop - 1; stepx = -1; stepy = -pitch; }
      else { base = (crop - 1) * pitch; stepx = -pitch; stepy = 1; }
      base += -left * stepx - top * stepy;
#pragma unroll 4
      for (int i = 0; i < 16; ++i) {
        const int p = warp * 16 + i;
        const int oy = (p >> 3) * 8 + ly, ox0 = (p & 7) * 16 + lx * 4;
        const int a = base + ox0 * stepx + oy * stepy;
        fov32[fov_word(oy, ox0 >> 2)] = (uint32_t)tile0[a] | ((uint32_t)tile0[a + stepx] << 8) |
                                         ((uint32_t)tile0[a + 2 * stepx] << 16) | ((uint32_t)tile0[a + 3 * stepx] << 24);
      }
    } else {
      for (int i = 0; i < 16; ++i) {
        const int p = warp * 16 + i;
        const int oy = (p >> 3) * 8 + ly, ox0 = (p & 7) * 16 + lx * 4;
        const int ryp = oy - top;
        const bool row_in = ryp >= 0 && ryp < ny;
        const int bx = rax + isin * (rcy - ryp);
        const int by = ray - icos * (rcy - ryp);
        uint32_t packed = 0;
#pragma unroll
        for (int k = 0; k < 4; ++k) {
          const int rxp = ox0 + k - left;
          uint32_t v = CBEV_PAL_BLACK;
          if (row_in && rxp >= 0 && rxp < nx) {
            if (mode == 0) {
              int sx, sy;
              if (turns == 0) { sx = rxp; sy = ryp; }
              else if (turns == 1) { sx = crop - 1 - ryp; sy = rxp; }
              else if (turns == 2) { sx = crop - 1 - rxp; sy = crop - 1 - ryp; }
              else { sx = ryp; sy = crop - 1 - rxp; }
              v = tile0[sy * pitch + sx];
            } else {
              int dx = bx + rxp * icos, dy = by + rxp * isin;
              if (dx < 0 || dy < 0 || dx > lim || dy > lim) v = bg;
              else v = tile0[(dy >> 16) * pitch + (dx >> 16)];
            }
          }
          packed |= v << (8 * k);
        }
        fov32[fov_word(oy, ox0 >> 2)] = packed;
      }
    }
    __syncthreads();
    if (P.fov_mask != nullptr) {
      for (int u = tid; u < S * S / 4; u += RT) {
        const uint32_t mk = ((const uint32_t*)P.fov_mask)[u];
        uint32_t* px = fov32 + fov_word(u >> 5, u & 31);
        *px = (*px & ~mk) | ((CBEV_PAL_BLACK * 0x01010101u) & mk);
      }
      __syncthreads();
    }
    if (tid < 16) {
      const int x = ex0 + (tid & 3), y = ey0 + (tid >> 2);
      if (x >= 0 && x < S && y >= 0 && y < S) s_fov[fov_byte(y, x)] = CBEV_PAL_BLACK;
    }
  }
  __syncthreads();
  trace_mark(P, env, 3);
  if (P.fov_out != nullptr) {
    uint4* dst = (uint4*)(P.fov_out + (size_t)env * S * S);
    for (int u = tid; u < S * S / 16; u += RT) dst[u] = *(const uint4*)(s_fov + fov_byte(u >> 3, (u & 7) << 4));
  }

  const int F = P.frame_stack;
  const int first = (flags & 1) ? P.head - F + 1 : P.head;

  if (OBS_MODE == CBEV_OBS_RGB) {
    uint32_t f[S * S / 4 / RT];
#pragma unroll
    for (int i = 0; i < S * S / 4 / RT; ++i) {
      const int u = tid + i * RT;
      f[i] = ((const uint32_t*)s_fov)[fov_word(u >> 5, u & 31)];
    }
    __syncthreads();
    uint8_t* s_rgb = s_region;
#pragma unroll
    for (int i = 0; i < S * S / 4 / RT; ++i) {
      const int u = tid + i * RT;
      const uint32_t p4 = f[i];
      const uint32_t k0 = s_key[p4 & 255u], k1 = s_key[(p4 >> 8) & 255u], k2 = s_key[(p4 >> 16) & 255u],
                     k3 = s_key[p4 >> 24];
      uint32_t* o = (uint32_t*)s_rgb + 3 * u;
      o[0] = k0 | (k1 << 24);
      o[1] = (k1 >> 8) | (k2 << 16);
      o[2] = (k2 >> 16) | (k3 << 8);
    }
    __syncthreads();
    uint8_t* dst = (uint8_t*)P.ring + (size_t)env * P.ring_slots * P.frame_bytes + (size_t)P.head * P.frame_bytes;
    for (int u = tid; u < S * S * 3 / 16; u += RT) st_u4(dst + 16 * u, ((const uint4*)s_rgb)[u]);
    return;
  }

  constexpr int OH = 96, OW = 96;
  uint8_t* s_out = s_region;
  {
  constexpr int O = 96;
  uint16_t* s_list = (uint16_t*)(s_region + O * O);
  {
    const int br = tid >> 3, j = tid & 7;
    uint4 R[4];
#pragma unroll
    for (int i = 0; i < 4; ++i) R[i] = *(const uint4*)(s_fov + fov_byte(4 * br + i, 16 * j));
    uint32_t m[4];
    uint32_t mixed = 0;
#pragma unroll
    for (int b = 0; b < 4; ++b) {
      const uint32_t w0 = (&R[0].x)[b], w1 = (&R[1].x)[b], w2 = (&R[2].x)[b], w3 = (&R[3].x)[b];
      const uint32_t c = w0 & 255u;
      const bool uni = w0 == w1 && w0 == w2 && w0 == w3 && w0 == c * 0x01010101u;
      m[b] = 0;
      if (uni) {
        if (OBS_MODE == CBEV_OBS_SEMANTIC) m[b] = s_cm[c];
        else m[b] = resolve_px<OBS_MODE>(c, c, c, c, 2, 2, 2, 2, s_rg, s_b, s_key, s_cm);
      } else {
        mixed |= 1u << b;
      }
    }
    const uint32_t o0 = m[0] | (m[0] << 8) | (m[0] << 16) | (m[1] << 24);
    const uint32_t o1 = m[1] | (m[1] << 8) | (m[2] << 16) | (m[2] << 24);
    const uint32_t o2 = m[2] | (m[3] << 8) | (m[3] << 16) | (m[3] << 24);
#pragma unroll
    for (int i = 0; i < 3; ++i) {
      uint32_t* o = (uint32_t*)(s_out + (3 * br + i) * O + 12 * j);
      o[0] = o0; o[1] = o1; o[2] = o2;
    }
    if (mixed) {
      const int n = __popc(mixed);
      int pos = atomicAdd(s_count, n);
#pragma unroll
      for (int b = 0; b < 4; ++b)
        if (mixed & (1u << b)) s_list[pos++] = (uint16_t)(br * 32 + j * 4 + b);
    }
  }
  __syncthreads();
  {
    const int n9 = *s_count * 9;
    for (int idx = tid; idx < n9; idx += RT) {
      const int blk = s_list[idx / 9], px = idx % 9;
      const int i = px / 3, jj = px % 3;
      const int bry = blk >> 5, bcx = blk & 31;
      const uint8_t* src0 = s_fov + fov_byte(4 * bry + i, 4 * bcx + jj);
      const uint8_t* src1 = s_fov + fov_byte(4 * bry + i + 1, 4 * bcx + jj);
      const uint32_t res = resolve_px<OBS_MODE>(src0[0], src0[1], src1[0], src1[1], 3 - jj, 1 + jj, 3 - i, 1 + i, s_rg,
                                                s_b, s_key, s_cm);
      s_out[(3 * bry + i) * O + 3 * bcx + jj] = (uint8_t)res;
    }
  }
  __syncthreads();
  }

  trace_mark(P, env, 4);
  for (int slot = first; slot <= P.head; ++slot) {
#pragma unroll 1
    for (int rep = 0; rep < 2; ++rep) {
      int sl = slot;
      if (rep == 1) {
        sl = slot - P.mirror;
        if (P.mirror <= 0 || sl < 0) break;
      }
      uint8_t* base = (uint8_t*)P.ring + ((size_t)env * P.ring_slots + sl) * P.frame_bytes;
      if (U8) {
        store_u8_planes<CHANNELS>(base, s_out, OH * OW, tid, RT);
      } else if (OBS_MODE == CBEV_OBS_SEMANTIC) {
        float* fb = (float*)base;
        const int plane = OH * OW;
        for (int q = tid; q < plane / 4; q += RT) {
          const uint32_t m4 = ((const uint32_t*)s_out)[q];
#pragma unroll
          for (int c = 0; c < CHANNELS; ++c)
            st_b4(fb + c * plane + 4 * q, bit_to_f32(m4, c), bit_to_f32(m4, c + 8), bit_to_f32(m4, c + 16),
                  bit_to_f32(m4, c + 24));
        }
      } else {
        for (int q = tid; q < OH * OW / 16; q += RT) st_u4(base + 16 * q, ((const uint4*)s_out)[q]);
      }
    }
  }
  trace_mark(P, env, 5);
}

template <int OBS_MODE, int CHANNELS, bool U8 = false>
__global__ void __launch_bounds__(1024, 1)
k_render_any(RenderParams P, const __grid_constant__ CUtensorMap tmap, int mask_mode) {
  extern __shared__ __align__(1024) uint8_t smem_raw[];
  uint8_t* const smem = smem_raw;
  if (smem_u32(smem_raw) & 1023u) __trap();
  const int S = P.fov, NT = blockDim.x;
  const int FP = S + 16;
  constexpr int BW = CBEV_ANY_BOX_W;
  const int tile_h = P.box_h * P.nby;
  const int tile_bytes = BW * P.nbx * tile_h;
  uint8_t* const s_tile = smem;
  uint8_t* const s_fov = smem + P.region_bytes;
  uint32_t* s_rg = (uint32_t*)(s_fov + S * FP);
  uint32_t* s_b = s_rg + 16;
  uint32_t* s_key = s_b + 16;
  int32_t* s_desc = (int32_t*)(s_key + 16);
  uint64_t* s_bar = (uint64_t*)(s_desc + CBEV_DESC_WORDS);
  uint8_t* s_cm = (uint8_t*)(s_bar + 2);
  uint8_t* s_cmu = s_cm + 16;
  float4* s_palf = (float4*)(s_cmu + 16);
  uint32_t* s_rects = (uint32_t*)(s_palf + 16);
  int32_t* s_tab = (int32_t*)(s_rects + ((P.max_rects * CBEV_RECT_WORDS + 3) & ~3));
  uint8_t* s_bflag = (uint8_t*)(s_tab + P.rs_words);
  uint8_t* s_out_sep = s_bflag + ((((S >> 3) * (S >> 3)) + 15) & ~15);

  const int env = P.order != nullptr ? P.order[blockIdx.x] : blockIdx.x;
  const int tid = threadIdx.x;
  const int lane = tid & 31, warp = tid >> 5, nwarps = NT >> 5;
  if (blockIdx.x == 0 && tid < 2 && P.order_cnt != nullptr) P.order_cnt[tid] = 0;
  const int32_t* d = P.desc + (size_t)env * CBEV_DESC_WORDS;
  const int flags = d[RD_FLAGS];
  if (flags & 2) return;
  trace_mark(P, env, 0);

  if (tid == 0) {
    mbar_init(s_bar, 1);
    asm volatile("fence.mbarrier_init.release.cluster;" ::: "memory");
    mbar_expect_tx(s_bar, (uint32_t)tile_bytes);
    const int x0 = d[RD_OX] & ~15, y0 = d[RD_OY];
    for (int bx = 0; bx < P.nbx; ++bx)
      for (int by = 0; by < P.nby; ++by)
        tma_load_2d(s_tile + (size_t)(bx * tile_h + by * P.box_h) * BW, &tmap, x0 + bx * BW, y0 + by * P.box_h, s_bar);
  }
  if (tid < CBEV_DESC_WORDS) s_desc[tid] = d[tid];
  if (tid < CBEV_PAL_COUNT) {
    s_rg[tid] = c_pal_rg[tid];
    s_b[tid] = c_pal_b[tid];
    s_key[tid] = c_pal_key[tid];
  }
  if (tid <= CBEV_PAL_COUNT) s_cm[tid] = c_chan_mask[mask_mode][tid];
  const int nrects = d[RD_NRECTS];
  {
    const uint32_t* rl = P.rects + (size_t)env * P.max_rects * CBEV_RECT_WORDS;
    for (int r = tid; r < P.max_rects * CBEV_RECT_WORDS; r += NT) s_rects[r] = rl[r];
  }
  for (int u = tid; u < P.rs_words; u += NT) s_tab[u] = P.rs_tab[u];
  __syncthreads();
  if (OBS_MODE != CBEV_OBS_RGB && tid < CBEV_PAL_COUNT) {
    const uint32_t kk = s_key[tid];
    s_cmu[tid] = (uint8_t)classify_key<OBS_MODE>(kk, s_key, s_cm);
    s_palf[tid] = make_float4((float)(kk & 255u), (float)((kk >> 8) & 255u), (float)(kk >> 16), 0.f);
  }
  mbar_wait(s_bar, 0);
  const int shift = s_desc[RD_OX] & 15;
  const int xmax = BW * P.nbx - 1, ymax = tile_h - 1;
  auto tile_raw = [&](int x, int y) { return (((x >> 7) * tile_h + y) * BW + (x & (BW - 1))) ^ ((y & 7) << 4); };
  auto tile_off = [&](int x, int y) { return tile_raw(min(max(x + shift, 0), xmax), min(max(y, 0), ymax)); };
  trace_mark(P, env, 1);

  {
    int r = 0;
    while (r < nrects) {
      const uint32_t pal = s_rects[2 * r + 1] >> 24;
      int e = r + 1;
      while (e < nrects && (s_rects[2 * e + 1] >> 24) == pal) ++e;
      for (int q = r + tid; q < e; q += NT) {
        const uint32_t w0 = s_rects[2 * q], w1 = s_rects[2 * q + 1];
        const int x0 = w0 & 0xffff, y0 = w0 >> 16, w = (w1 & 0xfff) + 1, h = ((w1 >> 12) & 0xfff) + 1;
// ... 50 lines not shown
        dy += isin;
      }
      return packed;
    };
    auto gather_generic = [&](int p) {
      const int oy = (p >> pw_log) * 8 + ly, ox0 = (p & (pw - 1)) * 16 + lx * 4;
      const int ryp = oy - top;
      const bool row_in = ryp >= 0 && ryp < ny;
      const int bx = rax + isin * (rcy - ryp);
      const int by = ray - icos * (rcy - ryp);
      uint32_t packed = 0;
#pragma unroll
      for (int k = 0; k < 4; ++k) {
        const int rxp = ox0 + k - left;
        uint32_t v = CBEV_PAL_BLACK;
        if (row_in && rxp >= 0 && rxp < nx) {
          if (mode == 0) {
            int sx, sy;
            if (turns == 0) { sx = rxp; sy = ryp; }
            else if (turns == 1) { sx = crop - 1 - ryp; sy = rxp; }
            else if (turns == 2) { sx = crop - 1 - rxp; sy = crop - 1 - ryp; }
            else { sx = ryp; sy = crop - 1 - rxp; }
            v = s_tile[tile_off(sx - s_desc[RD_FX], sy - fy)];
          } else {
            const int dx = bx + rxp * icos, dy = by + rxp * isin;
            if (dx < 0 || dy < 0 || dx > lim || dy > lim) v = bg;
            else v = s_tile[tile_off((dx >> 16) - s_desc[RD_FX], (dy >> 16) - fy)];
          }
        }
        packed |= v << (8 * k);
      }
      return packed;
    };
    auto finish = [&](int p, uint32_t packed) {
      const int oy = (p >> pw_log) * 8 + ly, ox0 = (p & (pw - 1)) * 16 + lx * 4;
      bool keep = true;
      if (blk83) {
        const uint32_t c = __shfl_sync(0xffffffffu, packed, lane & 2) & 255u;
        const unsigned agree = __ballot_sync(0xffffffffu, packed == c * 0x01010101u);
        const int pxp = p & (pw - 1), by = p >> pw_log, bx = 2 * pxp + (lx >> 1);
        const bool ego = (unsigned)(bx - ebx0) <= (unsigned)ebxn && (unsigned)(by - eby0) <= (unsigned)ebyn;
        const bool uni = (agree & mine) == mine && !ego;
        keep = !uni;
        if (local == 0) s_bflag[2 * p + (lx >> 1)] = uni ? 0 : 1;
        if (uni && local < 9) s_out_sep[3 * by * P.obs_w + 6 * pxp + loc_out] = s_cmu[c];
      }
      if (keep) *(uint32_t*)(s_fov + oy * FP + ox0) = packed;
    };
    if (fast) {
#pragma unroll 1
      for (int p = warp; p < npatch; p += 4 * nwarps) {
        uint32_t pk[4];
#pragma unroll
        for (int g = 0; g < 4; ++g) pk[g] = gather_fast(p + g * nwarps);
#pragma unroll
        for (int g = 0; g < 4; ++g) finish(p + g * nwarps, pk[g]);
      }
    } else {
      for (int p = warp; p < npatch; p += nwarps) finish(p, gather_generic(p));
    }
    __syncthreads();
    if (P.fov_mask != nullptr) {
      const int wq = S >> 2, wq_log = 31 - __clz(wq);
      for (int u = tid; u < S * wq; u += NT) {
        const uint32_t mk = ((const uint32_t*)P.fov_mask)[u];
        uint32_t* px = (uint32_t*)(s_fov + (u >> wq_log) * FP) + (u & (wq - 1));
        *px = (*px & ~mk) | ((CBEV_PAL_BLACK * 0x01010101u) & mk);
      }
      __syncthreads();
    }
    const int hw = P.hero_w;
    if (tid < hw * hw) {
      const int x = P.anchor_x - (hw >> 1) + tid % hw, y = P.anchor_y - (hw >> 1) + tid / hw;
      if (x >= 0 && x < S && y >= 0 && y < S) s_fov[y * FP + x] = CBEV_PAL_BLACK;
    }
  }
  __syncthreads();
  trace_mark(P, env, 3);
  const int cq = S >> 4, cq_log = 31 - __clz(cq);
  if (P.fov_out != nullptr) {
    uint4* dst = (uint4*)(P.fov_out + (size_t)env * S * S);
    for (int u = tid; u < S * cq; u += NT) dst[u] = *(const uint4*)(s_fov + (u >> cq_log) * FP + ((u & (cq - 1)) << 4));
  }

  const int F = P.frame_stack;
  const int first = (flags & 1) ? P.head - F + 1 : P.head;

  if (OBS_MODE == CBEV_OBS_RGB) {
    uint8_t* dst = (uint8_t*)P.ring + (size_t)env * P.ring_slots * P.frame_bytes + (size_t)P.head * P.frame_bytes;
    for (int u = tid; u < S * cq; u += NT) {
      const uint4 p16 = *(const uint4*)(s_fov + (u >> cq_log) * FP + ((u & (cq - 1)) << 4));
      uint32_t o[12];
#pragma unroll
      for (int g = 0; g < 4; ++g) {
        const uint32_t p4 = (&p16.x)[g];
        const uint32_t k0 = s_key[p4 & 255u], k1 = s_key[(p4 >> 8) & 255u], k2 = s_key[(p4 >> 16) & 255u],
                       k3 = s_key[p4 >> 24];
        o[3 * g] = k0 | (k1 << 24);
        o[3 * g + 1] = (k1 >> 8) | (k2 << 16);
        o[3 * g + 2] = (k2 >> 16) | (k3 << 8);
      }
#pragma unroll
      for (int g = 0; g < 3; ++g) st_b4(dst + 48 * (size_t)u + 16 * g, o[4 * g], o[4 * g + 1], o[4 * g + 2], o[4 * g + 3]);
    }
    return;
  }

  const int OH = P.obs_h, OW = P.obs_w;
  const bool blk83 = P.blk83 != 0;
  uint8_t* const s_out = blk83 ? s_out_sep : smem;
  uint8_t* const s_scratch = blk83 ? smem : smem + ((OH * OW + 15) & ~15);
  {
    const int rs_mode = P.rs_mode == CBEV_RS_FAST96 ? CBEV_RS_TABLE : P.rs_mode;
    const int nxt = s_tab[0], nyt = s_tab[1];
    const int32_t* xoff = s_tab + 2;
    const int32_t* yoff = xoff + OW + 1;
    const int32_t* xsi = yoff + OH + 1;
    const int32_t* ysi = xsi + nxt;
    const float* xal = (const float*)(ysi + nyt);
    const float* yal = xal + nxt;
    const int32_t* lxo = s_tab + 2;
    const int32_t* lyo = lxo + OW;
    const int32_t* lxa = lyo + OH;
    const int32_t* lyb = lxa + 2 * OW;
    const int qN = NT / OW, rN = NT - qN * OW;
    if (rs_mode == CBEV_RS_TABLE) {
      const int32_t* fxlo = (const int32_t*)(yal + nyt);
      const int32_t* fxhi = fxlo + OW;
      const int32_t* fylo = fxhi + OW;
      const int32_t* fyhi = fylo + OH;
      uint16_t* s_list = (uint16_t*)s_scratch;
      int* s_count = (int*)(s_bar + 1);
      if (tid < 2) s_count[tid] = 0;
      __syncthreads();
      auto pass_a = [&](bool valid, int o, int dx, int dy) {
        bool uni = true;
        if (valid) {
          uint32_t c0 = 0;
          const int xl = fxlo[dx], xh = fxhi[dx], yl = fylo[dy], yh = fyhi[dy];
          if (xh - xl < 4 && yh - yl < 4) {
            const int sh8 = (xl & 3) * 8, wlo = xl >> 2, whi = xh >> 2;
            const uint32_t msk = 0xffffffffu >> (8 * (3 - (xh - xl)));
            uint32_t diff = 0, c4 = 0;
#pragma unroll
            for (int i = 0; i < 4; ++i) {
              const uint32_t* row = (const uint32_t*)(s_fov + min(yl + i, yh) * FP);
              const uint32_t win = __funnelshift_r(row[wlo], row[whi], sh8);
              if (i == 0) { c0 = win & 255u; c4 = c0 * 0x01010101u; }
              diff |= (win ^ c4) & msk;
            }
            uni = diff == 0;
          } else {
            c0 = s_fov[yl * FP + xl];
            for (int yy = yl; yy <= yh; ++yy)
              for (int xx = xl; xx <= xh; ++xx) uni = uni && s_fov[yy * FP + xx] == c0;
          }
          if (uni) s_out[o] = s_cmu[c0];
        }
        const unsigned mixed = __ballot_sync(0xffffffffu, valid && !uni);
        if (mixed) {
          int pos = 0;
          if (lane == 0) pos = atomicAdd(s_count, __popc(mixed));
          pos = __shfl_sync(0xffffffffu, pos, 0);
          if (valid && !uni) s_list[pos + __popc(mixed & ((1u << lane) - 1u))] = (uint16_t)o;
        }
      };
      const int total = OH * OW, band = blk83 ? total : min(total, P.list_cap);
      int nmixed_all = 0;
      for (int b0 = 0; b0 < total; b0 += band) {
// ... 97 lines not shown
      }
      if (P.trace != nullptr && tid == 0)
        P.trace[(size_t)env * 8 + 7] = (unsigned)s_count[1] | ((unsigned long long)(unsigned)nmixed_all << 32);
    } else {
      uint16_t* s_list = (uint16_t*)s_scratch;
      int* s_count = (int*)(s_bar + 1);
      if (tid == 0) s_count[0] = 0;
      __syncthreads();
      const bool unit_taps = s_tab[0] == 1;
      const int total = OH * OW, band = min(total, P.list_cap);
      int nmixed_all = 0;
      for (int b0 = 0; b0 < total; b0 += band) {
        const int b1 = min(b0 + band, total);
        if (b0 > 0) {
          __syncthreads();
          if (tid == 0) s_count[0] = 0;
          __syncthreads();
        }
        int dy = (b0 + tid) / OW, dx = (b0 + tid) - dy * OW;
        for (int o0 = b0; o0 < b1; o0 += NT) {
          const int o = o0 + tid;
          const bool valid = o < b1;
          int same = -1;
          if (valid) {
            if (rs_mode == CBEV_RS_COPY) {
              same = s_fov[dy * FP + dx];
            } else if (rs_mode == CBEV_RS_HALF) {
              const uint8_t* q0 = s_fov + (2 * dy) * FP + 2 * dx;
              const uint32_t c0 = q0[0], c1 = q0[1], c2 = q0[FP], c3 = q0[FP + 1];
              if (c0 == c1 && c0 == c2 && c0 == c3) same = (int)c0;
            } else {
              const int sx0 = lxo[dx], sx1 = min(sx0 + 1, S - 1), sy0 = lyo[dy], sy1 = min(sy0 + 1, S - 1);
              const uint32_t i00 = s_fov[sy0 * FP + sx0], i01 = s_fov[sy0 * FP + sx1], i10 = s_fov[sy1 * FP + sx0],
                             i11 = s_fov[sy1 * FP + sx1];
              if (unit_taps && i00 == i01 && i00 == i10 && i00 == i11) same = (int)i00;
            }
            if (same >= 0) s_out[o] = s_cmu[same];
          }
          const unsigned mixed = __ballot_sync(0xffffffffu, valid && same < 0);
          if (mixed) {
            int pos = 0;
            if (lane == 0) pos = atomicAdd(s_count, __popc(mixed));
            pos = __shfl_sync(0xffffffffu, pos, 0);
            if (valid && same < 0) s_list[pos + __popc(mixed & ((1u << lane) - 1u))] = (uint16_t)o;
          }
          dy += qN;
          dx += rN;
          if (dx >= OW) { dx -= OW; ++dy; }
        }
        __syncthreads();
        const int nmixed = s_count[0];
        nmixed_all += nmixed;
        for (int idx = tid; idx < nmixed; idx += NT) {
          const int o = s_list[idx];
          const int oy = o / OW, ox = o - oy * OW;
          uint32_t key = 0;
          if (rs_mode == CBEV_RS_HALF) {
            const uint8_t* q0 = s_fov + (2 * oy) * FP + 2 * ox;
            const uint32_t c0 = q0[0], c1 = q0[1], c2 = q0[FP], c3 = q0[FP + 1];
            const uint32_t rg = s_rg[c0] + s_rg[c1] + s_rg[c2] + s_rg[c3] + 0x00020002u;
            const uint32_t b = s_b[c0] + s_b[c1] + s_b[c2] + s_b[c3] + 2u;
            key = ((rg & 0xffffu) >> 2) | ((rg >> 18) << 8) | ((b >> 2) << 16);
          } else {
            const int sx0 = lxo[ox], sx1 = min(sx0 + 1, S - 1), sy0 = lyo[oy], sy1 = min(sy0 + 1, S - 1);
            const int a0 = lxa[ox], a1 = lxa[OW + ox], b0 = lyb[oy], b1 = lyb[OH + oy];
            const uint32_t k00 = s_key[s_fov[sy0 * FP + sx0]], k01 = s_key[s_fov[sy0 * FP + sx1]],
                           k10 = s_key[s_fov[sy1 * FP + sx0]], k11 = s_key[s_fov[sy1 * FP + sx1]];
  #pragma unroll
            for (int ch = 0; ch < 3; ++ch) {
              const int r0 = (int)((k00 >> (8 * ch)) & 255u) * a0 + (int)((k01 >> (8 * ch)) & 255u) * a1;
              const int r1 = (int)((k10 >> (8 * ch)) & 255u) * a0 + (int)((k11 >> (8 * ch)) & 255u) * a1;
              const int v = (((b0 * (r0 >> 4)) >> 16) + ((b1 * (r1 >> 4)) >> 16) + 2) >> 2;
              key |= (uint32_t)min(max(v, 0), 255) << (8 * ch);
            }
          }
          s_out[o] = (uint8_t)classify_key<OBS_MODE>(key, s_key, s_cm);
        }
      }
      if (P.trace != nullptr && tid == 0) P.trace[(size_t)env * 8 + 7] = (unsigned long long)(unsigned)nmixed_all << 32;
    }
  }
  __syncthreads();

  trace_mark(P, env, 4);
  for (int slot = first; slot <= P.head; ++slot) {
#pragma unroll 1
    for (int rep = 0; rep < 2; ++rep) {
      int sl = slot;
      if (rep == 1) {
        sl = slot - P.mirror;
        if (P.mirror <= 0 || sl < 0) break;
      }
      uint8_t* base = (uint8_t*)P.ring + ((size_t)env * P.ring_slots + sl) * P.frame_bytes;
      if (U8) {
        store_u8_planes<CHANNELS>(base, s_out, OH * OW, tid, NT);
      } else if (OBS_MODE == CBEV_OBS_SEMANTIC) {
        float* fb = (float*)base;
        const int plane = OH * OW;
        for (int q = tid; q < plane / 4; q += NT) {
          const uint32_t m4 = ((const uint32_t*)s_out)[q];
#pragma unroll
          for (int c = 0; c < CHANNELS; ++c)
            st_b4(fb + c * plane + 4 * q, bit_to_f32(m4, c), bit_to_f32(m4, c + 8), bit_to_f32(m4, c + 16),
                  bit_to_f32(m4, c + 24));
        }
      } else {
        for (int q = tid; q < OH * OW / 16; q += NT) st_u4(base + 16 * q, ((const uint4*)s_out)[q]);
      }
    }
  }
  trace_mark(P, env, 5);
}

__device__ __forceinline__ float weighted3(float a, float b, float d) {
  return fminf(fmaxf(__fadd_rn(__fadd_rn(a, __fmul_rn(0.5f, b)), __fmul_rn(0.25f, d)), 0.f), 1.f);
}
__device__ __forceinline__ float u8_lane(const uint4& v, int k) { return (float)(((&v.x)[k >> 2] >> (8 * (k & 3))) & 255u); }

template <typename V, typename OutT>
__global__ void __launch_bounds__(256)
k_fuse(const V* __restrict__ ring, OutT* __restrict__ out, int N, int L, int C, int head, int veh, int mode,
       int HWV) {
  constexpr bool RING_U8 = std::is_same<V, uint4>::value;
  const int Cout = mode == CBEV_FUSE_VEHICLE_TEMPORAL ? C - 1 + 3 : C;
  const long long total = (long long)N * Cout * HWV;
  for (long long i = (long long)blockIdx.x * blockDim.x + threadIdx.x; i < total; i += (long long)gridDim.x * blockDim.x) {
    const int q = (int)(i % HWV);
    const int c = (int)((i / HWV) % Cout);
    const int env = (int)(i / ((long long)HWV * Cout));
    const V* frame = ring + ((size_t)env * L + head) * C * HWV;
    if (c == C - 1 && mode == CBEV_FUSE_VEHICLE_WEIGHTED) {
      const V a = frame[(size_t)veh * HWV + q];
      const V b = (frame - (size_t)C * HWV)[(size_t)veh * HWV + q];
      const V d = (frame - (size_t)2 * C * HWV)[(size_t)veh * HWV + q];
      if constexpr (RING_U8) {
        float* o = (float*)out + 16 * i;
#pragma unroll
        for (int g = 0; g < 4; ++g)
          st_f4(o + 4 * g, weighted3(u8_lane(a, 4 * g), u8_lane(b, 4 * g), u8_lane(d, 4 * g)),
                weighted3(u8_lane(a, 4 * g + 1), u8_lane(b, 4 * g + 1), u8_lane(d, 4 * g + 1)),
                weighted3(u8_lane(a, 4 * g + 2), u8_lane(b, 4 * g + 2), u8_lane(d, 4 * g + 2)),
                weighted3(u8_lane(a, 4 * g + 3), u8_lane(b, 4 * g + 3), u8_lane(d, 4 * g + 3)));
      } else {
        st_f4((float*)out + 4 * i, weighted3(a.x, b.x, d.x), weighted3(a.y, b.y, d.y), weighted3(a.z, b.z, d.z),
              weighted3(a.w, b.w, d.w));
      }
      continue;
    }
    V v;
    if (c < C - 1) {
      const int src = c < veh ? c : c + 1;
      v = frame[(size_t)src * HWV + q];
    } else {
      const int age = c - (C - 1);
      v = (frame - (size_t)age * C * HWV)[(size_t)veh * HWV + q];
    }
    if constexpr (!RING_U8) {
      st_f4((float*)out + 4 * i, v.x, v.y, v.z, v.w);
    } else if constexpr (sizeof(OutT) == 1) {
      st_u4((uint8_t*)out + 16 * i, v);
    } else {
      float* o = (float*)out + 16 * i;
#pragma unroll
      for (int g = 0; g < 4; ++g) st_f4(o + 4 * g, u8_lane(v, 4 * g), u8_lane(v, 4 * g + 1), u8_lane(v, 4 * g + 2), u8_lane(v, 4 * g + 3));
    }
  }
}

constexpr int MAX_DEVICES = 64;
bool g_tables_ready[MAX_DEVICES] = {};

void upload_tables() {
  static const uint8_t pal[CBEV_PAL_COUNT][3] = {{150, 150, 150}, {255, 255, 255}, {220, 220, 220}, {0, 7, 175},
                                                 {255, 0, 0},     {0, 255, 0},     {255, 64, 64},    {255, 255, 0},
                                                 {0, 0, 0},       {100, 100, 100}};
  uint32_t rg[CBEV_PAL_COUNT], b[CBEV_PAL_COUNT], key[CBEV_PAL_COUNT];
  for (int i = 0; i < CBEV_PAL_COUNT; ++i) {
    rg[i] = pal[i][0] | ((uint32_t)pal[i][1] << 16);
    b[i] = pal[i][2];
    key[i] = pal[i][0] | ((uint32_t)pal[i][1] << 8) | ((uint32_t)pal[i][2] << 16);
  }
  uint8_t cm[6][CBEV_PAL_COUNT + 1] = {};
  const int ND = CBEV_PAL_NON_DRIVABLE, DR = CBEV_PAL_DRIVABLE, SW = CBEV_PAL_SIDEWALK, VE = CBEV_PAL_VEHICLE,
            PE = CBEV_PAL_PEDESTRIAN, RO = CBEV_PAL_ROUTE, TL = CBEV_PAL_TL_RED;
  cm[CBEV_MASK_BINARY][DR] = 1; cm[CBEV_MASK_BINARY][RO] = 1;
  cm[CBEV_MASK_2][DR] = 1; cm[CBEV_MASK_2][RO] = 1 | 2;
  cm[CBEV_MASK_4][DR] = 1; cm[CBEV_MASK_4][VE] = 2; cm[CBEV_MASK_4][PE] = 4; cm[CBEV_MASK_4][RO] = 1 | 8;
  cm[CBEV_MASK_5][DR] = 1; cm[CBEV_MASK_5][SW] = 2; cm[CBEV_MASK_5][VE] = 4; cm[CBEV_MASK_5][PE] = 8;
  cm[CBEV_MASK_5][RO] = 1 | 16;
  for (int m = CBEV_MASK_6; m <= CBEV_MASK_7; ++m) {
    cm[m][ND] = 1; cm[m][DR] = 2; cm[m][SW] = 4; cm[m][VE] = 8; cm[m][PE] = 16; cm[m][RO] = 2 | 32;
  }
  cm[CBEV_MASK_7][TL] = 64;
  cudaMemcpyToSymbol(c_pal_rg, rg, sizeof(rg));
  cudaMemcpyToSymbol(c_pal_b, b, sizeof(b));
  cudaMemcpyToSymbol(c_pal_key, key, sizeof(key));
  cudaMemcpyToSymbol(c_chan_mask, cm, sizeof(cm));
}

template <int MODE, int CH, bool U8 = false>
int launch(cbev_engine* e, const RenderParams& P, size_t smem, size_t smem_any, bool any, cudaStream_t s) {
  static bool attr_done[MAX_DEVICES][2] = {};
  const int dev = e->device >= 0 && e->device < MAX_DEVICES ? e->device : 0;
  if (any) {
    auto kern = k_render_any<MODE, CH, U8>;
    if (!attr_done[dev][1]) {
      if (cudaFuncSetAttribute(kern, cudaFuncAttributeMaxDynamicSharedMemorySize, 227 * 1024) != cudaSuccess) {
        cbev_set_error("k_render_any: cannot opt in to 227 KB of dynamic shared memory: %s",
                       cudaGetErrorString(cudaGetLastError()));
        return 1;
      }
      attr_done[dev][1] = true;
    }
    kern<<<P.N, P.fov > 128 ? 1024 : 256, smem_any, s>>>(P, *reinterpret_cast<const CUtensorMap*>(e->tmap_any),
                                                        e->cfg.mask_mode);
    return 0;
  }
  auto kern = k_render<MODE, CH, U8>;
  if (!attr_done[dev][0]) {
    if (cudaFuncSetAttribute(kern, cudaFuncAttributeMaxDynamicSharedMemorySize, 100 * 1024) != cudaSuccess) {
      cbev_set_error("k_render: cannot opt in to 100 KB of dynamic shared memory: %s",
                     cudaGetErrorString(cudaGetLastError()));
      return 1;
    }
    attr_done[dev][0] = true;
  }
  kern<<<P.N, RT, smem, s>>>(P, *reinterpret_cast<const CUtensorMap*>(e->tmap), e->cfg.mask_mode);
  return 0;
}

template <bool U8>
int launch_semantic(cbev_engine* e, const RenderParams& P, size_t smem, size_t smem_any, bool any, cudaStream_t s) {
  switch (e->channels) {
    case 1: return launch<CBEV_OBS_SEMANTIC, 1, U8>(e, P, smem, smem_any, any, s);
    case 2: return launch<CBEV_OBS_SEMANTIC, 2, U8>(e, P, smem, smem_any, any, s);
    case 4: return launch<CBEV_OBS_SEMANTIC, 4, U8>(e, P, smem, smem_any, any, s);
    case 5: return launch<CBEV_OBS_SEMANTIC, 5, U8>(e, P, smem, smem_any, any, s);
    case 6: return launch<CBEV_OBS_SEMANTIC, 6, U8>(e, P, smem, smem_any, any, s);
    case 7: return launch<CBEV_OBS_SEMANTIC, 7, U8>(e, P, smem, smem_any, any, s);
    default: cbev_set_error("no raster kernel for %d mask channels", e->channels); return 1;
  }
}

int render_launch(cbev_engine* e, RenderParams& P, cudaStream_t s) {
  {
    const int dev = e->device >= 0 && e->device < MAX_DEVICES ? e->device : 0;
    if (!g_tables_ready[dev]) {
      upload_tables();
      g_tables_ready[dev] = true;
    }
  }
  P.fov = e->cfg.fov_size;
  P.crop = e->crop;
  P.anchor_x = e->anchor_x;
  P.anchor_y = e->anchor_y;
  P.frame_stack = e->cfg.frame_stack;
  P.frame_bytes = e->frame_bytes;
  P.max_rects = e->max_rects;
  P.fov_mask = e->fov_mask;
  const int S = P.fov;
  const size_t tile = (size_t)CBEV_TILE_W * CBEV_TILE_H;
  P.generic_rotate = (e->debug_flags & CBEV_DBG_GENERIC_ROTATE) != 0;
  P.obs_h = e->cfg.obs_h;
  P.obs_w = e->cfg.obs_w;
  P.rs_mode = e->rs_mode;
  P.rs_words = e->rs_words;
  P.rs_tab = e->rs_tab;
  P.hero_w = 32 / (1024 / S);
  P.nbx = e->any_nbx;
  P.nby = e->any_nby;
  P.box_h = e->any_box_h;
  const bool any = S != 128 || (e->cfg.obs_mode != CBEV_OBS_RGB && e->rs_mode != CBEV_RS_FAST96) ||
                   (e->debug_flags & CBEV_DBG_RENDER_ANY);
  const size_t rects_bytes = (size_t)((e->max_rects * CBEV_RECT_WORDS + 3) & ~3) * 4;
  const size_t smem = tile + (size_t)S * S + 3 * 16 * 4 + CBEV_DESC_WORDS * 4 + 16 + 16 + 16 + rects_bytes;
  size_t region = (size_t)CBEV_ANY_BOX_W * P.nbx * P.box_h * P.nby;
  const size_t ohw = (size_t)e->cfg.obs_h * e->cfg.obs_w, ohw16 = (ohw + 15) & ~(size_t)15;
  const size_t out_bytes = ohw16 + 2 * (ohw < 4096 ? ohw : 4096) + 16;
  const size_t nblk = (size_t)(S / 8) * (S / 8);
  P.blk83 = e->cfg.obs_mode != CBEV_OBS_RGB && e->rs_mode == CBEV_RS_TABLE && 3 * S == 8 * e->cfg.obs_w &&
            3 * S == 8 * e->cfg.obs_h && e->fov_mask == nullptr && !e->keep_fov &&
            !(e->debug_flags & CBEV_DBG_NO_BLOCK83);
  if (P.blk83 && 2 * ohw + 2 * nblk + 16 > region) P.blk83 = 0;
  if (e->cfg.obs_mode != CBEV_OBS_RGB && out_bytes > region) region = out_bytes;
  P.region_bytes = (int32_t)region;
  {
    const size_t room = region > ohw16 + 16 ? (region - ohw16 - 16) / 2 : 0;
    P.list_cap = (int32_t)(room < ohw ? room : ohw);
  }
  size_t sep_bytes = P.blk83 ? ((nblk + 15) & ~(size_t)15) + (((size_t)e->cfg.obs_h * e->cfg.obs_w + 15) & ~(size_t)15) : 0;
  size_t smem_any = region + (size_t)S * (S + 16) + 3 * 16 * 4 + CBEV_DESC_WORDS * 4 + 16 + 16 + 16 + 16 * 16 + rects_bytes +
                    (size_t)e->rs_words * 4;
  if (smem_any + sep_bytes > 227 * 1024) {
    P.blk83 = 0;
    sep_bytes = 0;
  }
  smem_any += sep_bytes;
  if (any && smem_any > 227 * 1024) {
    cbev_set_error("k_render_any needs %zu bytes of shared memory (max_rects %d): over the 227 KB of one CTA", smem_any,
                   e->max_rects);
    return 1;
  }
  int rc = 1;
  if (e->cfg.obs_mode == CBEV_OBS_RGB) rc = launch<CBEV_OBS_RGB, 1>(e, P, smem, smem_any, any, s);
  else if (e->cfg.obs_mode == CBEV_OBS_GRAY) rc = launch<CBEV_OBS_GRAY, 1>(e, P, smem, smem_any, any, s);
  else if (e->cfg.obs_mode == CBEV_OBS_SEMANTIC_U8) rc = launch_semantic<true>(e, P, smem, smem_any, any, s);
  else rc = launch_semantic<false>(e, P, smem, smem_any, any, s);
  if (rc == 0) e->launches += 1;
  return rc;
}

}

int cbev_launch_render(cbev_engine* e, int32_t head, int32_t mirror, cudaStream_t s) {
  RenderParams P;
  P.N = e->N;
  P.ring_slots = e->cfg.ring_slots;
  P.head = head;
  P.mirror = mirror;
  P.desc = e->desc;
  P.rects = e->rects;
  P.order = (e->debug_flags & CBEV_DBG_IDENTITY_RENDER_ORDER) ? nullptr : e->order;
  P.order_cnt = e->order_cnt;
  P.fov_out = e->keep_fov ? e->fov : nullptr;
  P.ring = e->ring;
  P.trace = (e->debug_flags & CBEV_DBG_TRACE) ? e->trace : nullptr;
  return render_launch(e, P, s);
}

int cbev_launch_render_branches(cbev_engine* e, int32_t n, void* windows, cudaStream_t s) {
  RenderParams P;
  P.N = n;
  P.ring_slots = 1;
  P.head = 0;
  P.mirror = 0;
  P.desc = e->br_desc;
  P.rects = e->br_rects;
  P.order = nullptr;
  P.order_cnt = nullptr;
  P.fov_out = nullptr;
  P.ring = windows;
  P.trace = nullptr;
  return render_launch(e, P, s);
}

int cbev_launch_fuse(cbev_engine* e, int32_t mode, const void* ring, int32_t n, int32_t L, int32_t head, void* out,
                     cudaStream_t s) {
  static const int veh_of[6] = {-1, -1, 1, 2, 3, 3};
  const int veh = veh_of[e->cfg.mask_mode];
  if (veh < 0) return 1;
  const int C = e->channels;
  const int Cout = mode == CBEV_FUSE_VEHICLE_TEMPORAL ? C - 1 + 3 : C;
  const bool u8 = e->cfg.obs_mode == CBEV_OBS_SEMANTIC_U8;
  const int HWV = e->cfg.obs_h * e->cfg.obs_w / (u8 ? 16 : 4);
  long long total = (long long)n * Cout * HWV;
  int blocks = (int)((total + 255) / 256);
  if (blocks > 148 * 32) blocks = 148 * 32;
  if (!u8)
    k_fuse<<<blocks, 256, 0, s>>>((const float4*)ring, (float*)out, n, L, C, head, veh, mode, HWV);
  else if (mode == CBEV_FUSE_VEHICLE_TEMPORAL)
    k_fuse<<<blocks, 256, 0, s>>>((const uint4*)ring, (uint8_t*)out, n, L, C, head, veh, mode, HWV);
  else
    k_fuse<<<blocks, 256, 0, s>>>((const uint4*)ring, (float*)out, n, L, C, head, veh, mode, HWV);
  e->launches += 1;
  return 0;
}
```

carlabev_env_b200/csrc/sim.cu:

```cuda
#include <limits.h>
#include <math.h>

#include "engine.h"

#ifndef CBEV_SIM_BLOCKS_PER_SM
#define CBEV_SIM_BLOCKS_PER_SM 7
#endif

namespace {

constexpr double DT = 0.1;
constexpr double WB = 2.9;
constexpr double KST = 2.0;
constexpr double KPS = 1.0;
constexpr double MPP = 0.3125;
constexpr double MAX_STEER = 0x1.0c152382d7365p-1;
constexpr double PI = 0x1.921fb54442d18p+1;
constexpr double TWO_PI = 0x1.921fb54442d18p+2;
constexpr double HALF_PI = 0x1.921fb54442d18p+0;
constexpr double DEG2RAD = 0x1.1df46a2529d39p-6;
constexpr double RAD2DEG = 0x1.ca5dc1a63c1f8p+5;
constexpr unsigned FULL = 0xffffffffu;

enum { E_X = 0, E_Y, E_YAW, E_V, E_X1, E_Y1, E_YAW1, E_V1, E_ACC, E_T, E_D2G, E_D2G1, E_SPREV, E_LAST_DYAW,
       E_PC_AL, E_PC_AT, E_PC_YR, E_TARGET, E_GAS, E_STEER, E_BRAKE, E_DELTA, E_SLOTS = 24 };
enum { I_TIDX = 0, I_FLAGS, I_K, I_OFFROAD, I_STEP, I_SLOTS = 8 };
enum { S_RET = 0, S_LEN, S_SPEED, S_C0, S_VIOL = 9, S_HARSH, S_CAUSE, S_SLOTS = 12 };
enum { FL_COMFORT = 1, FL_SPREV = 2 };
enum { ST_IDLE = 0, ST_WAITING, ST_ENTERING, ST_YIELDING, ST_CROSSING, ST_STALLED, ST_RETREATING, ST_CLEARED,
       ST_RETREATED };
enum { HIT_NONE = 0, HIT_VEHICLE, HIT_PEDESTRIAN, HIT_TARGET };

__device__ __forceinline__ double clipd(double x, double lo, double hi) { return fmin(fmax(x, lo), hi); }

__device__ __forceinline__ double angle_mod(double x) {
  double a = x + PI;
  double m = fmod(a, TWO_PI);
  if (m != 0.0) {
    if (m < 0.0) m += TWO_PI;
  } else {
    m = 0.0;
  }
  return m - PI;
}

__device__ __forceinline__ int rect_left(double c, int pad, int size) {
  return (int)rint((double)pad + c * 1.0) - (size >> 1);
}

__device__ __forceinline__ bool overlap(int ax, int ay, int aw, int bx, int by, int bw) {
  return ax < bx + bw && ay < by + bw && ax + aw > bx && ay + aw > by;
}

__device__ __forceinline__ uint64_t splitmix64(uint64_t z) {
  z += 0x9E3779B97F4A7C15ull;
  z = (z ^ (z >> 30)) * 0xBF58476D1CE4E5B9ull;
  z = (z ^ (z >> 27)) * 0x94D049BB133111EBull;
  return z ^ (z >> 31);
}

template <int G>
__device__ int warp_nearest(double fx, double fy, const double* __restrict__ cx, const double* __restrict__ cy, int n,
                            int lane, unsigned GM) {
  double best = INFINITY;
  int bi = 0x7fffffff;
  for (int i = lane; i < n; i += G) {
    double dx = fx - cx[i], dy = fy - cy[i];
    double d = dx * dx + dy * dy;
    if (d < best) { best = d; bi = i; }
  }
#pragma unroll
  for (int o = G / 2; o > 0; o >>= 1) {
    double ob = __shfl_xor_sync(GM, best, o);
    int oi = __shfl_xor_sync(GM, bi, o);
    if (ob < best || (ob == best && oi < bi)) { best = ob; bi = oi; }
  }
  return bi;
}

__device__ int scalar_nearest(double fx, double fy, const double* cx, const double* cy, int n) {
  double best = INFINITY;
  int bi = 0;
  for (int i = 0; i < n; ++i) {
    double dx = fx - cx[i], dy = fy - cy[i];
    double d = dx * dx + dy * dy;
    if (d < best) { best = d; bi = i; }
  }
  return bi;
}

struct Body {
  double x, y, yaw, v, x1, y1, yaw1, v1;
};

__device__ __forceinline__ void body_update(Body& b, double acc, double delta, double target) {
  delta = clipd(delta, -MAX_STEER, MAX_STEER);
  b.x1 = b.x; b.y1 = b.y; b.yaw1 = b.yaw; b.v1 = b.v;
  double sn, cs;
  sincos(b.yaw, &sn, &cs);
  b.x += (b.v * cs) * DT;
  b.y += (b.v * sn) * DT;
  b.yaw += ((b.v / WB) * tan(delta)) * DT;
  b.v += acc * DT;
  b.yaw = angle_mod(b.yaw);
  b.v = clipd(b.v, -1.0 * target, target);
}

struct View {
  int xmin, ymin;
  int mode, turns, nx, ny, isin, icos, ax, ay, xd, yd, cy;
  int fx, fy, bw, bh;
};

__device__ void compute_view(const SimParams& P, double x, double y, double theta, View& v) {
  const int crop = P.crop, pad = P.pad;
  int offx = (int)(((double)pad + x * 1.0) + (-(double)crop / 2.0));
  int offy = (int)(((double)pad + y * 1.0) + (-(double)crop / 2.0));
  int cx = (int)rint((double)offx + (double)crop / 2.0);
  int cy = (int)rint((double)offy + (double)crop / 2.0);
  v.xmin = max(0, min(max(0, P.map_w + 2 * pad - crop), cx - crop / 2));
  v.ymin = max(0, min(max(0, P.map_h + 2 * pad - crop), cy - crop / 2));
  float anglef = (float)(theta * RAD2DEG + 90.0);
  double angle = (double)anglef;
  if (fmod(angle, 90.0) == 0.0) {
    int a = (int)angle;
    int turns = (a / 90) % 4;
    if (turns < 0) turns += 4;
    v.mode = 0;
    v.turns = turns;
    v.nx = v.ny = crop;
    v.isin = v.icos = v.ax = v.ay = v.xd = v.yd = v.cy = 0;
  } else {
    double rad = angle * 0.01745329251994329;
    double s = sin(rad), c = cos(rad);
    double w = (double)crop, h = (double)crop;
    double cxx = c * w, cyy = c * h, sx = s * w, sy = s * h;
    int nx = (int)fmax(fmax(fmax(fabs(cxx + sy), fabs(cxx - sy)), fabs(-cxx + sy)), fabs(-cxx - sy));
    int ny = (int)fmax(fmax(fmax(fabs(sx + cyy), fabs(sx - cyy)), fabs(-sx + cyy)), fabs(-sx - cyy));
    v.mode = 1;
    v.turns = 0;
    v.nx = nx;
// ... 15 lines not shown
    int sx, sy;
    if (v.mode == 0) {
      if (v.turns == 0) { sx = rxp; sy = ryp; }
      else if (v.turns == 1) { sx = crop - 1 - ryp; sy = rxp; }
      else if (v.turns == 2) { sx = crop - 1 - rxp; sy = crop - 1 - ryp; }
      else { sx = ryp; sy = crop - 1 - rxp; }
    } else {
      sx = ((v.ax + v.xd) + v.isin * (v.cy - ryp) + rxp * v.icos) >> 16;
      sy = ((v.ay + v.yd) - v.icos * (v.cy - ryp) + rxp * v.isin) >> 16;
    }
    x_lo = min(x_lo, sx); x_hi = max(x_hi, sx);
    y_lo = min(y_lo, sy); y_hi = max(y_hi, sy);
  }
  x_lo = max(x_lo, 0); y_lo = max(y_lo, 0);
  x_hi = min(x_hi, crop - 1); y_hi = min(y_hi, crop - 1);
  if (x_hi < x_lo || y_hi < y_lo) { x_lo = y_lo = 0; x_hi = y_hi = 0; }
  v.fx = x_lo;
  v.fy = y_lo;
  v.bw = min(x_hi - x_lo + 1, P.win_max);
  v.bh = min(y_hi - y_lo + 1, P.win_max);
}

__device__ void write_desc_header(const SimParams& P, int32_t* __restrict__ d, const View& v, int nrects, int flags,
                                  int bg) {
  d[RD_OX] = v.xmin + v.fx - P.pad;
  d[RD_OY] = v.ymin + v.fy - P.pad;
  d[RD_MODE] = v.mode;
  d[RD_TURNS] = v.turns;
  d[RD_NX] = v.nx;
  d[RD_NY] = v.ny;
  d[RD_ISIN] = v.isin;
  d[RD_ICOS] = v.icos;
  d[RD_AX] = v.ax;
  d[RD_AY] = v.ay;
  d[RD_XD] = v.xd;
  d[RD_YD] = v.yd;
  d[RD_CY] = v.cy;
  d[RD_NRECTS] = nrects;
  d[RD_FLAGS] = flags;
  d[RD_FX] = v.fx;
  d[RD_FY] = v.fy;
  d[RD_BG] = bg;
}

__device__ __forceinline__ int crop_corner_class(const SimParams& P, const View& v) {
  const int mx = v.xmin - P.pad, my = v.ymin - P.pad;
  if (mx < 0 || my < 0 || mx >= P.map_w || my >= P.map_h) return CBEV_PAL_NON_DRIVABLE;
  return P.map[(size_t)my * P.map_w + mx];
}

__device__ __forceinline__ bool pack_rect(int rx, int ry, int rw, int rh, int pal, const View& v, uint32_t& w0,
                                          uint32_t& w1, bool& covers00) {
  covers00 = rx <= v.xmin && v.xmin < rx + rw && ry <= v.ymin && v.ymin < ry + rh;
  const int wx = v.xmin + v.fx, wy = v.ymin + v.fy;
  int x0 = max(rx - wx, 0), y0 = max(ry - wy, 0);
  int x1 = min(rx + rw - wx, v.bw), y1 = min(ry + rh - wy, v.bh);
  if (x1 <= x0 || y1 <= y0) return false;
  w0 = (uint32_t)x0 | ((uint32_t)y0 << 16);
  w1 = (uint32_t)(x1 - x0 - 1) | ((uint32_t)(y1 - y0 - 1) << 12) | ((uint32_t)pal << 24);
  return true;
}

__device__ void init_actors(const SimParams& P, const PoolDev& pool, const EnvState& S, size_t row, int scene, int lane,
                            int stride) {
  const int A0 = pool.actor_off[scene], A = pool.actor_off[scene + 1] - A0;
  for (int a = lane; a < A; a += stride) {
    size_t o = row * P.max_actors + a;
    const double* s0 = pool.act_state0 + (size_t)(A0 + a) * 4;
    S.ax[o] = s0[0];
    S.ay[o] = s0[1];
    S.ayaw[o] = s0[2];
    S.av[o] = s0[3];
    S.atidx[o] = pool.act_tidx0[A0 + a];
    int beh = pool.act_beh[A0 + a];
    bool jay = beh == CBEV_BEH_CROSS || beh == CBEV_BEH_STOP_MID || beh == CBEV_BEH_STOP_RETURN;
    S.atarget_mps[o] = jay ? 0.0 : pool.act_cruise_mps[A0 + a];
    S.aelapsed[o] = 0.0;
    S.astate_elapsed[o] = 0.0;
    S.arxlen[o] = pool.act_raw_off[A0 + a + 1] - pool.act_raw_off[A0 + a];
    S.aflags[o] = jay ? ST_WAITING : ST_IDLE;
  }
}

__device__ void reset_env(const SimParams& P, const PoolDev& pool, const EnvState& st, int env, int scene, int lane,
                          int stride = 32) {
  const int r0 = pool.ego_off[scene], nt = pool.ego_off[scene + 1] - r0;
  if (lane == 0) {
    double* e = st.ego + (size_t)env * E_SLOTS;
    const double* s0 = pool.ego_state0 + (size_t)scene * 4;
    e[E_X] = e[E_X1] = s0[0];
    e[E_Y] = e[E_Y1] = s0[1];
    e[E_YAW] = e[E_YAW1] = s0[2];
    e[E_V] = e[E_V1] = s0[3];
    e[E_ACC] = 0.0;
    e[E_T] = 0.0;
    double gx = pool.ego_cx[r0 + nt - 1], gy = pool.ego_cy[r0 + nt - 1];
    double dx = s0[0] - gx, dy = s0[1] - gy;
    double d2g = sqrt(dx * dx + dy * dy);
    e[E_D2G] = e[E_D2G1] = d2g;
    e[E_SPREV] = 0.0;
    e[E_LAST_DYAW] = 0.0;
    e[E_PC_AL] = e[E_PC_AT] = e[E_PC_YR] = 0.0;
    e[E_TARGET] = pool.ego_target_speed[scene];
    int32_t* ei = st.egoi + (size_t)env * I_SLOTS;
    ei[I_TIDX] = pool.ego_tidx0[scene];
    ei[I_FLAGS] = 0;
    ei[I_K] = 0;
    ei[I_OFFROAD] = 0;
    ei[I_STEP] = 0;
    st.scene[env] = scene;
    st.done[env] = 0;
    for (int w = 0; w < CBEV_TGT_WORDS; ++w) {
      const int n = nt - 64 * w;
      st.tgt_vis[(size_t)env * CBEV_TGT_WORDS + w] = n >= 64 ? ~0ull : (n > 0 ? ((1ull << n) - 1ull) : 0ull);
    }
    double* sa = st.stats + (size_t)env * S_SLOTS;
    for (int k = 0; k < S_SLOTS; ++k) sa[k] = 0.0;
  }
  init_actors(P, pool, st, (size_t)env, scene, lane, stride);
}

__global__ void __launch_bounds__(32 * CBEV_WARPS_PER_BLOCK)
k_reset(SimParams P, PoolDev pool, EnvState st, const uint8_t* __restrict__ mask,
        const int32_t* __restrict__ scene_ids, int32_t* __restrict__ desc, int32_t* __restrict__ order,
        int32_t* __restrict__ move_order) {
  const int env = blockIdx.x * CBEV_WARPS_PER_BLOCK + (threadIdx.x >> 5);
  const int lane = threadIdx.x & 31;
  if (env >= P.N) return;
  if (lane == 0) { order[env] = env; move_order[env] = env; }
  if (mask != nullptr && mask[env] == 0) {
    if (lane == 0) desc[(size_t)env * CBEV_DESC_WORDS + RD_FLAGS] = 2;
    return;
  }
  int scene = scene_ids[env];
  scene = min(max(scene, 0), pool.n_scenes - 1);
  reset_env(P, pool, st, env, scene, lane);
  if (lane == 0) {
    const double* s0 = pool.ego_state0 + (size_t)scene * 4;
    View v;
    compute_view(P, s0[0], s0[1], 0.0, v);
    write_desc_header(P, desc + (size_t)env * CBEV_DESC_WORDS, v, 0, 1, crop_corner_class(P, v));
  }
}

__device__ void start_retreat(const PoolDev& pool, double* rbuf, int32_t* rn, int ga, Body& b, int& tidx, int& rxlen) {
  const int w0 = pool.act_raw_off[ga];
  const double* rawx = pool.act_raw_x + w0;
  const double* rawy = pool.act_raw_y + w0;
  int cur = max(0, min(tidx, rxlen - 1));
  double ax[CBEV_SG_MAX], ay[CBEV_SG_MAX];
  int n0 = min(cur + 2, CBEV_SG_MAX);
  ax[0] = b.x;
  ay[0] = b.y;
  for (int i = 1; i < n0; ++i) {
    ax[i] = rawx[cur - (i - 1)];
    ay[i] = rawy[cur - (i - 1)];
  }
  int n = 1;
  for (int i = 1; i < n0; ++i) {
    double d = hypot(ax[i] - ax[i - 1], ay[i] - ay[i - 1]);
    if (d > 1e-9) { ax[n] = ax[i]; ay[n] = ay[i]; ++n; }
  }
  if (n < 2) { ax[1] = ax[0] + 1e-3; ay[1] = ay[0]; n = 2; }
  double* cx = rbuf;
  double* cy = rbuf + CBEV_SG_MAX;
  double* cyaw = rbuf + 2 * CBEV_SG_MAX;
  const double* M = pool.sg_mat + (size_t)n * CBEV_SG_MAX * CBEV_SG_MAX;
  for (int i = 0; i < n; ++i) {
    double sx = 0.0, sy = 0.0;
    for (int j = 0; j < n; ++j) {
      sx += M[i * CBEV_SG_MAX + j] * ax[j];
      sy += M[i * CBEV_SG_MAX + j] * ay[j];
    }
    cx[i] = sx;
    cy[i] = sy;
  }
  double s[CBEV_SG_MAX];
  s[0] = 0.0;
  for (int i = 1; i < n; ++i) s[i] = s[i - 1] + hypot(cx[i] - cx[i - 1], cy[i] - cy[i - 1]);
  if (s[n - 1] <= 1e-9) {
    for (int i = 0; i < n; ++i) cyaw[i] = 0.0;
  } else {
    double prev = 0.0, corr = 0.0;
    for (int i = 0; i < n; ++i) {
      double gx, gy;
      if (i == 0) {
        gx = (cx[1] - cx[0]) / (s[1] - s[0]);
        gy = (cy[1] - cy[0]) / (s[1] - s[0]);
      } else if (i == n - 1) {
        gx = (cx[n - 1] - cx[n - 2]) / (s[n - 1] - s[n - 2]);
        gy = (cy[n - 1] - cy[n - 2]) / (s[n - 1] - s[n - 2]);
      } else {
        double d1 = s[i] - s[i - 1], d2 = s[i + 1] - s[i];
        double a = -(d2) / (d1 * (d1 + d2)), bb = (d2 - d1) / (d1 * d2), c = d1 / (d2 * (d1 + d2));
        gx = a * cx[i - 1] + bb * cx[i] + c * cx[i + 1];
        gy = a * cy[i - 1] + bb * cy[i] + c * cy[i + 1];
      }
      double p = atan2(gy, gx);
      if (i > 0) {
        double dd = p - prev;
        double m = fmod(dd + PI, TWO_PI);
        if (m != 0.0 && m < 0.0) m += TWO_PI;
        double ddmod = m - PI;
        if (ddmod == -PI && dd > 0.0) ddmod = PI;
        double pc = ddmod - dd;
        if (fabs(dd) < PI) pc = 0.0;
        corr += pc;
      }
      prev = p;
      cyaw[i] = i > 0 ? p + corr : p;
    }
  }
  *rn = n;
  b.x = cx[0];
  b.y = cy[0];
  double fx = b.x + WB * cos(b.yaw), fy = b.y + WB * sin(b.yaw);
  tidx = scalar_nearest(fx, fy, cx, cy, n);
  b.yaw = cyaw[tidx];
  rxlen = cur + 2;
}

template <int G>
__device__ __forceinline__ void actor_chunk_step(const SimParams& P, const PoolDev& pool, const EnvState& S, size_t row,
                                                 int ga, size_t o, bool has, double t_sim, int lane, int gb, unsigned GM,
                                                 Body& b, int& kind) {
// ... 81 lines not shown
          } else if (fsm == ST_RETREATING) {
            target_mps = fmax(0.0, cruise_mps);
            int w0 = pool.act_raw_off[ga];
            double gx = b.x - pool.act_raw_x[w0], gy = b.y - pool.act_raw_y[w0];
            bool reached = sqrt(gx * gx + gy * gy) <= 1.0;
            if (reached || complete) { fsm = ST_RETREATED; state_elapsed = 0.0; target_mps = 0.0; }
          } else if (fsm == ST_CLEARED || fsm == ST_RETREATED) {
            target_mps = 0.0;
          }
        }
      }
    }
    const bool active = has && (atidx < np - 1);
    double fx = 0.0, fy = 0.0;
    if (active) {
      double sn, cs;
      sincos(b.yaw, &sn, &cs);
      fx = b.x + WB * cs; fy = b.y + WB * sn;
    }
    int my_idx = 0;
    unsigned am = __ballot_sync(GM, active) >> gb;
    while (am) {
      int src = __ffs(am) - 1;
      am &= am - 1;
      double bfx = __shfl_sync(GM, fx, gb + src), bfy = __shfl_sync(GM, fy, gb + src);
      unsigned long long pcx = __shfl_sync(GM, (unsigned long long)cxp, gb + src);
      unsigned long long pcy = __shfl_sync(GM, (unsigned long long)cyp, gb + src);
      int bn = __shfl_sync(GM, np, gb + src);
      int idx = warp_nearest<G>(bfx, bfy, (const double*)pcx, (const double*)pcy, bn, lane, GM);
      if (lane == src) my_idx = idx;
    }
    if (active) {
      const double target = target_mps / MPP;
      double ai = KPS * (target - b.v);
      double ddx = fx - cxp[my_idx], ddy = fy - cyp[my_idx];
      double sn2, cs2;
      sincos(b.yaw + HALF_PI, &sn2, &cs2);
      double err = ddx * (-cs2) + ddy * (-sn2);
      int cur = atidx >= my_idx ? atidx : my_idx;
      double theta_e = angle_mod(cyawp[cur] - b.yaw);
      double theta_d = atan2(KST * err, fmax(b.v, 1e-3));
      double di = clipd(theta_e + theta_d, -MAX_STEER, MAX_STEER);
      atidx = cur;
      body_update(b, ai, di, target);
    }
    if (has) {
      S.ax[o] = b.x; S.ay[o] = b.y; S.ayaw[o] = b.yaw; S.av[o] = b.v;
      S.atidx[o] = atidx;
      S.arxlen[o] = rxlen;
      S.atarget_mps[o] = target_mps;
      S.aelapsed[o] = elapsed;
      S.astate_elapsed[o] = state_elapsed;
      S.aflags[o] = (uint8_t)(fsm | (braking ? 16 : 0) | (on_retreat ? 32 : 0));
    }
}

template <int G>
__device__ __forceinline__ void live_actor_chunk(const SimParams& P, const PoolDev& pool, const EnvState& S, size_t row, int ga,
                                              size_t o, bool has, double t_sim, int lane, int gb, unsigned GM, Body& b,
                                              int& kind) {
  actor_chunk_step<G>(P, pool, S, row, ga, o, has, t_sim, lane, gb, GM, b, kind);
}

template <int G>
__device__ __forceinline__ void hand_over_to_live(const SimParams& P, const PoolDev& pool, const EnvState& st, int env, int scene,
                                               int A, int lane, unsigned GM) {
  for (int a = lane; a < A; a += G) {
    const size_t o = (size_t)env * P.max_actors + a, r = (size_t)scene * P.max_actors + a;
    st.ax[o] = pool.roll.ax[r]; st.ay[o] = pool.roll.ay[r]; st.ayaw[o] = pool.roll.ayaw[r]; st.av[o] = pool.roll.av[r];
    st.atarget_mps[o] = pool.roll.atarget_mps[r]; st.aelapsed[o] = pool.roll.aelapsed[r];
    st.astate_elapsed[o] = pool.roll.astate_elapsed[r]; st.atidx[o] = pool.roll.atidx[r];
    st.arxlen[o] = pool.roll.arxlen[r]; st.aflags[o] = pool.roll.aflags[r];
  }
  for (int k = lane; k < P.max_retreat * 3 * CBEV_SG_MAX; k += G)
    st.retreat[(size_t)env * P.max_retreat * 3 * CBEV_SG_MAX + k] = pool.roll.retreat[(size_t)scene * P.max_retreat * 3 * CBEV_SG_MAX + k];
  for (int k = lane; k < P.max_retreat; k += G)
    st.retreat_n[(size_t)env * P.max_retreat + k] = pool.roll.retreat_n[(size_t)scene * P.max_retreat + k];
  __syncwarp(GM);
}

template <int G>
__device__ __forceinline__ void auto_reset_env(const SimParams& P, const PoolDev& pool, const EnvState& st, const cbev_step_out& out,
                                            int32_t* d, int32_t* order, int32_t* order_cnt, int env, int lane, unsigned GM) {
  int ep = st.episode[env];
  uint64_t h = splitmix64(P.seed + (uint64_t)env * 0x9E3779B97F4A7C15ull + (uint64_t)ep * 0xD1B54A32D192ED03ull);
  int scene = (int)(h % (uint64_t)pool.n_scenes);
  __syncwarp(GM);
  reset_env(P, pool, st, env, scene, lane, G);
  if (lane == 0) {
    order[atomicAdd(order_cnt, 1)] = env;
    const double* s0 = pool.ego_state0 + (size_t)scene * 4;
    View v;
    compute_view(P, s0[0], s0[1], 0.0, v);
    write_desc_header(P, d, v, 0, 1, crop_corner_class(P, v));
    out.reward[env] = 0.0;
    out.terminated[env] = 0;
    out.truncated[env] = 0;
    if (out.cause) out.cause[env] = CBEV_CAUSE_NONE;
    if (out.hero) {
      double* hb = out.hero + (size_t)env * CBEV_HERO_FIELDS;
      for (int k = 0; k < CBEV_HERO_FIELDS; ++k) hb[k] = 0.0;
      hb[CBEV_H_X] = s0[0]; hb[CBEV_H_Y] = s0[1]; hb[CBEV_H_YAW] = s0[2]; hb[CBEV_H_V] = s0[3];
      hb[CBEV_H_SCENE] = (double)scene;
    }
  }
}

template <int G>
struct Group {
  int warp, lane, gb, grp;
  unsigned GM;
  int env;
  __device__ __forceinline__ Group(const SimParams& P, const int32_t* __restrict__ perm = nullptr) {
    constexpr int EPW = 32 / G;
    warp = threadIdx.x >> 5;
    const int wl = threadIdx.x & 31;
    lane = wl & (G - 1);
    gb = wl & ~(G - 1);
    grp = wl / G;
    GM = G == 32 ? 0xffffffffu : (((1u << G) - 1u) << gb);
    env = (blockIdx.x * CBEV_WARPS_PER_BLOCK + warp) * EPW + grp;
    if (perm != nullptr && env < P.N) env = perm[env];
  }
};

enum { MV_LIVE = 0, MV_BRANCH = 1, MV_BRANCH_DRAW = 2 };
template <int G, int MODE>
__device__ __forceinline__ void move_body(const SimParams& P, const PoolDev& pool, const EnvState& st,
                                          const void* __restrict__ actions, const cbev_step_out& out,
                                          int32_t* __restrict__ desc, uint32_t* __restrict__ rects,
                                          int32_t* __restrict__ order, int32_t* __restrict__ order_cnt, int env,
                                          int lane, int gb, unsigned GM) {
  constexpr bool BRANCH = MODE != MV_LIVE, DRAW = MODE != MV_BRANCH;
  int32_t* d = desc + (size_t)env * CBEV_DESC_WORDS;
  uint32_t* rl = rects + (size_t)env * P.max_rects * CBEV_RECT_WORDS;

  const uint8_t was_done = BRANCH ? 0 : st.done[env];
  const int scene = st.scene[env];
  double* eg = st.ego + (size_t)env * E_SLOTS;
  const int32_t* ei = st.egoi + (size_t)env * I_SLOTS;
  Body e;
  e.x = eg[E_X]; e.y = eg[E_Y]; e.yaw = eg[E_YAW]; e.v = eg[E_V];
  double acc = eg[E_ACC];
  const double etarget = eg[E_TARGET];
  const double t_sim = eg[E_T] + DT;
  const int step_idx = ei[I_STEP];
  const unsigned long long tv0 = st.tgt_vis[(size_t)env * CBEV_TGT_WORDS], tv1 = st.tgt_vis[(size_t)env * CBEV_TGT_WORDS + 1];
  float gas, steer, brake;
  if (P.action_mode == CBEV_ACTION_DISCRETE) {
    long long id = ((const long long*)actions)[env];
    const int nd = P.n_discrete;
    id = id < 0 ? 0 : (id >= nd ? nd - 1 : id);
    gas = P.discrete_table[id * 3 + 0];
    steer = P.discrete_table[id * 3 + 1];
    brake = P.discrete_table[id * 3 + 2];
  } else {
    const float* a = (const float*)actions + (size_t)env * 3;
    gas = fminf(fmaxf(a[0], 0.0f), 1.0f);
    steer = fminf(fmaxf(a[1], -1.0f), 1.0f);
    brake = fminf(fmaxf(a[2], 0.0f), 1.0f);
  }

  if constexpr (!BRANCH) {
    if (P.autoreset == CBEV_AUTORESET_NEXT_STEP && was_done) {
      auto_reset_env<G>(P, pool, st, out, d, order, order_cnt, env, lane, GM);
      return;
    }
  }

  const int r0 = pool.ego_off[scene], nt = pool.ego_off[scene + 1] - r0;
  const int A0 = pool.actor_off[scene], A = pool.actor_off[scene + 1] - A0;
  const int tl0 = pool.tl_off[scene], ntl = pool.tl_off[scene + 1] - tl0;
  const bool use_table = step_idx < pool.traj_steps;
  const long long toff = pool.traj_steps > 0 ? pool.traj_off[scene] : 0;
  const double* __restrict__ ecx = pool.ego_cx + r0;
  const double* __restrict__ ecy = pool.ego_cy + r0;

// ... 430 lines not shown
    for (int w = 0; w < CBEV_TGT_WORDS; ++w) st.tgt_vis[(size_t)env * CBEV_TGT_WORDS + w] = tvis[w];
    if constexpr (MODE == JG_BRANCH_ROW) {
      if (terminated) {
        st.episode[env] += 1;
        st.done[env] = 1;
        for (int k = 0; k < S_SLOTS; ++k) sa[k] = 0.0;
      } else {
        sa[S_RET] = ep_ret; sa[S_LEN] = ep_len; sa[S_SPEED] = ep_speed;
        for (int k = 0; k < 6; ++k) sa[S_C0 + k] += cm6[k];
        sa[S_VIOL] = ep_viol; sa[S_HARSH] = ep_harsh; sa[S_CAUSE] = ep_cause;
      }
    }
    if constexpr (!BRANCH) {
      out.reward[env] = reward;
      out.terminated[env] = terminated;
      out.truncated[env] = truncated;
      if (out.cause) out.cause[env] = (uint8_t)cause;
      if (terminated) {
        double inv = 1.0 / ep_len;
        if (out.episode) {
          double* ep = out.episode + (size_t)env * CBEV_EPISODE_FIELDS;
          ep[CBEV_E_RETURN] = ep_ret; ep[CBEV_E_LENGTH] = ep_len; ep[CBEV_E_CAUSE] = ep_cause;
          ep[CBEV_E_MEAN_SPEED] = ep_speed / ep_len;
          for (int k = 0; k < 6; ++k) ep[CBEV_E_ABS_ACCEL_LONG + k] = (sa[S_C0 + k] + cm6[k]) / ep_len;
          ep[CBEV_E_VIOL_RATE] = ep_viol / ep_len; ep[CBEV_E_HARSH_RATE] = ep_harsh / ep_len;
          ep[CBEV_E_SCENE] = (double)scene; ep[CBEV_E_NUM_VEHICLES] = (double)pool.num_vehicles[scene];
          ep[CBEV_E_LEN_ROUTE] = pool.len_ego_route[scene]; ep[CBEV_E_EPISODE] = (double)st.episode[env];
        }
        atomicAdd(gstats + CBEV_S_EPISODES, 1.0);
        atomicAdd(gstats + CBEV_S_RETURN, ep_ret);
        atomicAdd(gstats + CBEV_S_LENGTH, ep_len);
        atomicAdd(gstats + CBEV_S_MEAN_SPEED, ep_speed * inv);
        atomicAdd(gstats + CBEV_S_CAUSE0 + (int)ep_cause, 1.0);
        for (int k = 0; k < 6; ++k) atomicAdd(gstats + CBEV_S_ABS_COMFORT0 + k, (sa[S_C0 + k] + cm6[k]) * inv);
        atomicAdd(gstats + CBEV_S_VIOL_RATE, ep_viol * inv);
        atomicAdd(gstats + CBEV_S_HARSH_RATE, ep_harsh * inv);
        st.episode[env] += 1;
        st.done[env] = 1;
        move_order[atomicAdd(move_cnt, 1)] = env;
        for (int k = 0; k < S_SLOTS; ++k) sa[k] = 0.0;
      } else {
        move_order[P.N - 1 - atomicAdd(move_cnt + 1, 1)] = env;
        sa[S_RET] = ep_ret; sa[S_LEN] = ep_len; sa[S_SPEED] = ep_speed;
        for (int k = 0; k < 6; ++k) sa[S_C0 + k] += cm6[k];
        sa[S_VIOL] = ep_viol; sa[S_HARSH] = ep_harsh; sa[S_CAUSE] = ep_cause;
      }
    }
    if (hero_now) {
      double* hb = hb_s;
      hb[CBEV_H_X] = e.x; hb[CBEV_H_Y] = e.y; hb[CBEV_H_YAW] = e.yaw; hb[CBEV_H_V] = e.v;
      hb[CBEV_H_X1] = e.x1; hb[CBEV_H_Y1] = e.y1; hb[CBEV_H_YAW1] = e.yaw1; hb[CBEV_H_V1] = e.v1;
      hb[CBEV_H_DIST2WP] = dist2wp; hb[CBEV_H_SP_X] = ecx[tidx]; hb[CBEV_H_SP_Y] = ecy[tidx];
      hb[CBEV_H_SP_YAW] = ecyaw[tidx];
      hb[CBEV_H_CMD_GAS] = eg[E_GAS]; hb[CBEV_H_CMD_STEER] = eg[E_STEER]; hb[CBEV_H_CMD_BRAKE] = eg[E_BRAKE];
      hb[CBEV_H_DELTA] = eg[E_DELTA];
      hb[CBEV_H_SPEED_MPS] = speed_mps; hb[CBEV_H_ACCEL_LONG] = accel_long; hb[CBEV_H_ACCEL_LAT] = accel_lat;
      hb[CBEV_H_JERK_LONG] = jerk_long; hb[CBEV_H_JERK_LAT] = jerk_lat; hb[CBEV_H_YAW_RATE] = yaw_rate_deg;
      hb[CBEV_H_YAW_ACC] = yaw_acc;
      hb[CBEV_H_ACC] = acc; hb[CBEV_H_TIDX] = (double)tidx; hb[CBEV_H_HIT] = (double)hit;
      hb[CBEV_H_HIT_ID] = (double)hit_id; hb[CBEV_H_TILE] = (double)tile; hb[CBEV_H_NEARBY] = (double)n_nearby;
      hb[CBEV_H_DIST2GOAL] = d2g; hb[CBEV_H_T] = t_sim; hb[CBEV_H_SCENE] = (double)scene;
    }
  }
  __syncwarp(GM);
  if (hero_now) {
    for (int f = lane; f < CBEV_HERO_FIELDS; f += G) out.hero[(size_t)env * CBEV_HERO_FIELDS + f] = hb_s[f];
  }
  reward_out = reward;
  terminated_out = terminated;
  truncated_out = truncated;
  cause_out = cause;
}

template <int G>
__global__ void __launch_bounds__(32 * CBEV_WARPS_PER_BLOCK, 4)
k_judge(SimParams P, PoolDev pool, EnvState st, cbev_step_out out, const int32_t* __restrict__ desc,
        double* __restrict__ gstats, int32_t* __restrict__ move_order, int32_t* __restrict__ move_cnt) {
  constexpr int EPW = 32 / G;
  __shared__ double s_hero[CBEV_WARPS_PER_BLOCK][EPW][CBEV_HERO_FIELDS];
  const Group<G> g(P);
  const int lane = g.lane, env = g.env;
  if (env >= P.N) return;
  if (desc[(size_t)env * CBEV_DESC_WORDS + RD_FLAGS] & 1) {
    if (lane == 0) move_order[P.N - 1 - atomicAdd(move_cnt + 1, 1)] = env;
    return;
  }
  double reward;
  bool terminated, truncated;
  int cause;
  judge_body<G, JG_LIVE>(P, pool, st, out, gstats, move_order, move_cnt, s_hero[g.warp][g.grp], env, lane, g.gb, g.GM,
                       false, reward, terminated, truncated, cause);
}

__global__ void __launch_bounds__(32 * CBEV_WARPS_PER_BLOCK)
k_rollout(SimParams P, PoolDev pool) {
  const int scene = blockIdx.x * CBEV_WARPS_PER_BLOCK + (threadIdx.x >> 5);
  const int lane = threadIdx.x & 31;
  if (scene >= pool.n_scenes) return;
  const int A0 = pool.actor_off[scene], A = pool.actor_off[scene + 1] - A0;
  init_actors(P, pool, pool.roll, (size_t)scene, scene, lane, 32);
  __syncwarp();
  double t_sim = 0.0;
  for (int step = 0; step < pool.traj_steps; ++step) {
    t_sim += DT;
    for (int base = 0; base < A; base += 32) {
      const int a = base + lane;
      const bool has = a < A;
      const int ga = A0 + (has ? a : 0);
      const size_t o = (size_t)scene * P.max_actors + (has ? a : 0);
      Body b;
      int kind = 0;
      actor_chunk_step<32>(P, pool, pool.roll, (size_t)scene, ga, o, has, t_sim, lane, 0, FULL, b, kind);
      if (has) pool.traj[pool.traj_off[scene] + (size_t)step * A + a] = make_double4(b.x, b.y, b.yaw, b.v);
    }
    __syncwarp();
  }
}

struct LookaheadArgs {
  const uint8_t* src[CBEV_STATE_SECTIONS];
  uint8_t* dst[CBEV_STATE_SECTIONS];
  int32_t esize[CBEV_STATE_SECTIONS], count[CBEV_STATE_SECTIONS];
  const int32_t* live_scene;
  const uint8_t* live_done;
  const int32_t* roots;
  const void* actions;
  double gamma;
  int32_t n_live, horizon;
  cbev_lookahead_out out;
};

struct LookaheadRender {
  int32_t* stage_desc;
  uint32_t* stage_rects;
  int32_t* desc;
  uint32_t* rects;
  int32_t F;
};

struct LookaheadRoots {
  const int32_t* live_episode;
  const uint8_t* rows;
  int64_t row_bytes;
  int64_t off[CBEV_STATE_SECTIONS];
  int32_t count[CBEV_STATE_SECTIONS];
  int32_t n_rows;
};

template <int G, bool OBS, bool ROWS = false, bool LEAF = false>
__device__ __forceinline__ void lookahead_body(const SimParams& P, const PoolDev& pool, const EnvState& br,
                                               const LookaheadArgs& a, const LookaheadRender& rd,
                                               const LookaheadRoots& rr = LookaheadRoots{}) {
  constexpr int EPW = 32 / G;
  __shared__ double s_hero[CBEV_WARPS_PER_BLOCK][EPW][CBEV_HERO_FIELDS];
  const Group<G> g(P);
  const int lane = g.lane, b = g.env, B = P.N, H = a.horizon;
  const unsigned GM = g.GM;
  if (b >= B) return;
  const int root = a.roots ? a.roots[b] : b;
  bool live, valid;
  int4 hdr = make_int4(-1, 0, 1, 0);
  const uint8_t* row = nullptr;
  if constexpr (ROWS) {
    valid = root >= 0 && root < rr.n_rows;
    if (valid) {
      row = rr.rows + (size_t)root * rr.row_bytes;
      hdr = *(const int4*)row;
// ... 47 lines not shown
    int slot = 0;
    for (int t = 0; t < H; ++t) {
      const void* act = P.action_mode == CBEV_ACTION_DISCRETE
                            ? (const void*)((const long long*)a.actions + (size_t)t * B)
                            : (const void*)((const float*)a.actions + (size_t)t * B * 3);
      if constexpr (OBS) {
        move_body<G, MV_BRANCH_DRAW>(P, pool, br, act, so, rd.stage_desc + (size_t)slot * B * CBEV_DESC_WORDS,
                                     rd.stage_rects + (size_t)slot * B * P.max_rects * CBEV_RECT_WORDS, nullptr,
                                     nullptr, b, lane, g.gb, GM);
        slot = slot + 1 == rd.F ? 0 : slot + 1;
      } else {
        move_body<G, MV_BRANCH>(P, pool, br, act, so, nullptr, nullptr, nullptr, nullptr, b, lane, g.gb, GM);
      }
      __syncwarp(GM);
      double r;
      judge_body<G, LEAF ? JG_BRANCH_ROW : JG_BRANCH>(P, pool, br, so, nullptr, nullptr, nullptr,
                                                      s_hero[g.warp][g.grp], b, lane, g.gb, GM, t == H - 1, r,
                                                      terminated, truncated, cause);
      if (lane == 0 && o.reward) o.reward[(size_t)t * B + b] = r;
      ret = __dadd_rn(ret, __dmul_rn(w, r));
      w = __dmul_rn(w, a.gamma);
      steps = t + 1;
      if (terminated || truncated) break;
    }
  }
  if (o.reward)
    for (int t = steps + lane; t < H; t += G) o.reward[(size_t)t * B + b] = 0.0;
  if (steps == 0 && o.hero)
    for (int f = lane; f < CBEV_HERO_FIELDS; f += G) o.hero[(size_t)b * CBEV_HERO_FIELDS + f] = 0.0;
  if (lane == 0) {
    o.ret[b] = ret;
    if (o.steps) o.steps[b] = steps;
    if (o.terminated) o.terminated[b] = terminated;
    if (o.truncated) o.truncated[b] = truncated;
    if (o.cause) o.cause[b] = (uint8_t)cause;
  }
  if constexpr (OBS) {
    __syncwarp(GM);
    const int F = rd.F, first = F - (steps < F ? steps : F);
    const int RW = P.max_rects * CBEV_RECT_WORDS;
    for (int f = 0; f < F; ++f) {
      int32_t* dd = rd.desc + ((size_t)b * F + f) * CBEV_DESC_WORDS;
      if (f < first) {
        if (lane == 0) dd[RD_FLAGS] = 2;
        continue;
      }
      const int j = (steps - F + f) % F;
      const int32_t* sd = rd.stage_desc + ((size_t)j * B + b) * CBEV_DESC_WORDS;
      for (int k = lane; k < CBEV_DESC_WORDS; k += G) dd[k] = sd[k];
      const int nw = sd[RD_NRECTS] * CBEV_RECT_WORDS;
      const uint32_t* sr = rd.stage_rects + ((size_t)j * B + b) * RW;
      uint32_t* dr = rd.rects + ((size_t)b * F + f) * RW;
      for (int k = lane; k < nw; k += G) dr[k] = sr[k];
    }
  }
}

template <int G>
__global__ void __launch_bounds__(32 * CBEV_WARPS_PER_BLOCK, 4)
k_lookahead(SimParams P, PoolDev pool, EnvState br, LookaheadArgs a) {
  lookahead_body<G, false>(P, pool, br, a, LookaheadRender{});
}

template <int G>
__global__ void __launch_bounds__(32 * CBEV_WARPS_PER_BLOCK, 4)
k_lookahead_obs(SimParams P, PoolDev pool, EnvState br, LookaheadArgs a, LookaheadRender rd) {
  lookahead_body<G, true>(P, pool, br, a, rd);
}

template <int G, bool OBS, bool ROWS, bool LEAF>
__global__ void __launch_bounds__(32 * CBEV_WARPS_PER_BLOCK, 4)
k_lookahead_ex(SimParams P, PoolDev pool, EnvState br, LookaheadArgs a, LookaheadRender rd, LookaheadRoots rr) {
  lookahead_body<G, OBS, ROWS, LEAF>(P, pool, br, a, rd, rr);
}

}

static SimParams make_params(cbev_engine* e) {
  SimParams P;
  P.N = e->N;
  P.max_actors = e->cfg.max_actors;
  P.max_rects = e->max_rects;
  P.max_retreat = e->pool.max_retreat;
  P.map_w = e->map_w;
  P.map_h = e->map_h;
  P.fov = e->cfg.fov_size;
  P.hero_scale = (float)(1024 / e->cfg.fov_size);
  P.hero_w = 32 / (1024 / e->cfg.fov_size);
  P.win_max = e->win_max;
  P.crop = e->crop;
  P.pad = e->pad;
  P.anchor_x = e->anchor_x;
  P.anchor_y = e->anchor_y;
  P.action_mode = e->cfg.action_mode;
  P.n_discrete = e->cfg.n_discrete;
  P.reward_mode = e->cfg.reward_mode;
  P.autoreset = e->cfg.autoreset;
  P.seed = e->cfg.seed;
  P.map = e->map;
  for (int i = 0; i < 48; ++i) P.discrete_table[i] = e->cfg.discrete_table[i];
  P.cfg = e->cfg;
  return P;
}

void cbev_launch_reset(cbev_engine* e, const uint8_t* mask, const int32_t* scene_ids, cudaStream_t s) {
  SimParams P = make_params(e);
  int blocks = (e->N + CBEV_WARPS_PER_BLOCK - 1) / CBEV_WARPS_PER_BLOCK;
  k_reset<<<blocks, 32 * CBEV_WARPS_PER_BLOCK, 0, s>>>(P, e->pool, e->st, mask, scene_ids, e->desc, e->order, e->move_order);
  e->launches += 1;
}

static bool narrow_groups(const cbev_engine* e) {
  return e->pool.max_actors <= 8 || e->pool.traj_steps > 0;
}

void cbev_launch_move(cbev_engine* e, const void* actions, const cbev_step_out* out, cudaStream_t s) {
  SimParams P = make_params(e);
  const int32_t* mo = (e->debug_flags & CBEV_DBG_IDENTITY_MOVE_ORDER) ? nullptr : e->move_order;
  if (narrow_groups(e)) {
    constexpr int G = 8;
    int per_block = CBEV_WARPS_PER_BLOCK * (32 / G);
    int blocks = (e->N + per_block - 1) / per_block;
    k_move<G><<<blocks, 32 * CBEV_WARPS_PER_BLOCK, 0, s>>>(P, e->pool, e->st, actions, *out, e->desc, e->rects, e->order,
                                                           e->order_cnt, mo, e->move_cnt);
  } else {
    int blocks = (e->N + CBEV_WARPS_PER_BLOCK - 1) / CBEV_WARPS_PER_BLOCK;
    k_move<32><<<blocks, 32 * CBEV_WARPS_PER_BLOCK, 0, s>>>(P, e->pool, e->st, actions, *out, e->desc, e->rects, e->order,
                                                            e->order_cnt, mo, e->move_cnt);
  }
  e->launches += 1;
}

void cbev_launch_judge(cbev_engine* e, const cbev_step_out* out, cudaStream_t s) {
  SimParams P = make_params(e);
  constexpr int G = 8;
  int per_block = CBEV_WARPS_PER_BLOCK * (32 / G);
  int blocks = (e->N + per_block - 1) / per_block;
  k_judge<G><<<blocks, 32 * CBEV_WARPS_PER_BLOCK, 0, s>>>(P, e->pool, e->st, *out, e->desc, e->gstats, e->move_order,
                                                          e->move_cnt);
  e->launches += 1;
}

template <int G>
static void launch_lookahead(int blocks, cudaStream_t s, bool record, bool rows, bool leaf, const SimParams& P,
                             cbev_engine* e, const LookaheadArgs& a, const LookaheadRender& rd,
                             const LookaheadRoots& rr) {
  constexpr int T = 32 * CBEV_WARPS_PER_BLOCK;
  if (!rows && !leaf) {
    if (record) k_lookahead_obs<G><<<blocks, T, 0, s>>>(P, e->pool, e->branch, a, rd);
    else k_lookahead<G><<<blocks, T, 0, s>>>(P, e->pool, e->branch, a);
  } else if (leaf) {
    if (rows) k_lookahead_ex<G, true, true, true><<<blocks, T, 0, s>>>(P, e->pool, e->branch, a, rd, rr);
    else k_lookahead_ex<G, true, false, true><<<blocks, T, 0, s>>>(P, e->pool, e->branch, a, rd, rr);
  } else if (record) {
    k_lookahead_ex<G, true, true, false><<<blocks, T, 0, s>>>(P, e->pool, e->branch, a, rd, rr);
  } else {
    k_lookahead_ex<G, false, true, false><<<blocks, T, 0, s>>>(P, e->pool, e->branch, a, rd, rr);
  }
}

void cbev_launch_lookahead(cbev_engine* e, const int32_t* roots, int32_t n_branches, int32_t horizon,
                           const void* actions, double gamma, const cbev_lookahead_out* out, bool record,
                           const RowSource* rows, bool leaf, cudaStream_t s) {
  SimParams P = make_params(e);
  P.N = n_branches;
  LookaheadArgs a;
  const int32_t A = e->cfg.max_actors > 0 ? e->cfg.max_actors : 1, R = e->pool.max_retreat;
  const StateSections src = cbev_state_sections(e->st, A, R), dst = cbev_state_sections(e->branch, A, R);
  for (int k = 0; k < CBEV_STATE_SECTIONS; ++k) {
    a.src[k] = (const uint8_t*)*src.field[k];
    a.dst[k] = (uint8_t*)*dst.field[k];
    a.esize[k] = src.esize[k];
    a.count[k] = src.count[k];
  }
  a.live_scene = e->st.scene;
  a.live_done = e->st.done;
  a.roots = roots;
  a.actions = actions;
  a.gamma = gamma;
  a.n_live = e->N;
  a.horizon = horizon;
  a.out = *out;
  const LookaheadRender rd{e->br_stage_desc, e->br_stage_rects, e->br_desc, e->br_rects, e->cfg.frame_stack};
  LookaheadRoots rr = {};
  rr.live_episode = e->st.episode;
  if (rows) {
    rr.rows = (const uint8_t*)rows->rows;
    rr.row_bytes = rows->L.row_bytes;
    for (int k = 0; k < CBEV_STATE_SECTIONS; ++k) {
      rr.off[k] = rows->L.off[k];
      rr.count[k] = rows->L.count[k];
    }
    rr.n_rows = rows->n_rows;
  }
// ... 18 lines not shown
```

Baseline: 21.87 million.

## Pre-render per-scene reset frames and stamp them on a side stream

Renders each scene's initial observation once into a per-scene stamp buffer. Reset frames (explicit and next-step autoreset) are then filled by copying the stamp into the ring instead of re-rendering. The copy runs in a new k_stamp kernel on a separate stream that overlaps with the move kernel. Done-flag clearing moves so the stamp kernel can read the previous done state. This adds cache-invalidation logic, extra memory, and stream/event ordering dependencies.

```diff
diff --git a/carlabev_env_b200/csrc/api.cu b/carlabev_env_b200/csrc/api.cu
--- a/carlabev_env_b200/csrc/api.cu
+++ b/carlabev_env_b200/csrc/api.cu
@@ -211,6 +211,7 @@
   if (grow_rects) { dev_free(e->rects); e->rects = rects; e->max_rects = new_max_rects; }
   if (grow_retreat) { dev_free(e->st.retreat); dev_free(e->st.retreat_n); e->st.retreat = retreat; e->st.retreat_n = retreat_n; }
   e->has_pool = true;
+  e->stamps_valid = false;
   if (!live) e->pool_epoch += 1;
   if (e->pool.traj_steps > 0) {
     cbev_launch_rollout(e, 0);
@@ -343,6 +344,7 @@
   if (F == 1) e->cfg.ring_slots = 1;
   e->N = cfg->num_envs;
   cudaGetDevice(&e->device);
+  cudaDeviceGetAttribute(&e->num_sms, cudaDevAttrMultiProcessorCount, e->device);
   const int m = cfg->fov_size - 1;
   int ax = (int)nearbyint((double)m * cfg->anchor_x_frac), ay = (int)nearbyint((double)m * cfg->anchor_y_frac);
   ax = ax < 0 ? 0 : (ax > m ? m : ax);
@@ -431,7 +433,11 @@
   dev_free(e->map); dev_free(e->desc); dev_free(e->rects); dev_free(e->fov); dev_free(e->gstats);
   dev_free(e->h_reward_dev);
   { uint8_t* p = (uint8_t*)e->h_actions_dev; dev_free(p); }
+  dev_free(e->stamps); dev_free(e->stamp_fov);
   if (e->side_stream) cudaStreamDestroy(e->side_stream);
+  if (e->stamp_stream) cudaStreamDestroy(e->stamp_stream);
+  if (e->ev_head) cudaEventDestroy(e->ev_head);
+  if (e->ev_stamp) cudaEventDestroy(e->ev_stamp);
   if (e->ev_sim) cudaEventDestroy(e->ev_sim);
   if (e->ev_copy) cudaEventDestroy(e->ev_copy);
   if (e->ev_judge) cudaEventDestroy(e->ev_judge);
@@ -454,6 +460,7 @@
   if (rc) return rc;
   e->map_w = w;
   e->map_h = h_px;
+  e->stamps_valid = false;
   rc = build_tensor_map(e);
   if (rc) return rc;
   e->has_map = true;
@@ -703,6 +710,42 @@
   return CBEV_OK;
 }
 
+static int ensure_stamps(cbev_engine* e, cudaStream_t s) {
+  if (e->stamps_valid) return CBEV_OK;
+  const int n = e->pool.n_scenes;
+  const int stride = (e->cfg.obs_h * e->cfg.obs_w + 15) & ~15;
+  const size_t fov_bytes = (size_t)e->cfg.fov_size * e->cfg.fov_size;
+  if (n > e->stamp_rows || stride != e->stamp_stride || (e->keep_fov && !e->stamp_fov)) {
+    CU_TRY(cudaDeviceSynchronize());
+    dev_free(e->stamps);
+    dev_free(e->stamp_fov);
+    e->stamp_rows = 0;
+    int rc = dev_alloc(&e->stamps, (size_t)n * stride);
+    if (!rc && e->keep_fov) rc = dev_alloc(&e->stamp_fov, (size_t)n * fov_bytes);
+    if (rc) return rc;
+    e->stamp_rows = n;
+    e->stamp_stride = stride;
+  }
+  const size_t desc_bytes = (size_t)n * CBEV_DESC_WORDS * 4, rects_bytes = (size_t)n * e->max_rects * CBEV_RECT_WORDS * 4;
+  uint8_t* scratch = nullptr;
+  CU_TRY(cudaMalloc(&scratch, desc_bytes + rects_bytes));
+  int rc = CBEV_OK;
+  if (cudaMemsetAsync(scratch + desc_bytes, 0, rects_bytes, s) != cudaSuccess) {
+    cbev_set_error("zeroing the stamp draw lists failed: %s", cudaGetErrorString(cudaGetLastError()));
+    rc = CBEV_ERR_CUDA;
+  }
+  if (!rc) {
+    cbev_launch_stamp_desc(e, (int32_t*)scratch, s);
+    if (cbev_launch_render_stamps(e, (const int32_t*)scratch, (const uint32_t*)(scratch + desc_bytes), s)) rc = CBEV_ERR_CUDA;
+  }
+  const cudaError_t ce = cudaStreamSynchronize(s);
+  cudaFree(scratch);
+  if (rc) return rc;
+  if (ce != cudaSuccess) { cbev_set_error("rendering the reset stamps failed: %s", cudaGetErrorString(ce)); return CBEV_ERR_CUDA; }
+  e->stamps_valid = true;
+  return CBEV_OK;
+}
+
 int cbev_reset(cbev_handle e, const uint8_t* mask_dev, const int32_t* scene_ids_dev, void* stream) {
   int rc = check_ready(e, false);
   if (rc) return rc;
@@ -710,11 +753,16 @@
   if (mask_dev && !e->was_reset) { cbev_set_error("the first reset must cover every env (mask = NULL)"); return CBEV_ERR_STATE; }
   cudaStream_t s = (cudaStream_t)stream;
   const int F = e->cfg.frame_stack, L = e->cfg.ring_slots;
+  const int mirror = F > 1 ? L - F + 1 : 0;
   if (e->head < 0) e->head = F - 1;
+  const bool stamp = cbev_uses_stamps(e);
+  if (stamp && (rc = ensure_stamps(e, s))) return rc;
   cbev_launch_reset(e, mask_dev, scene_ids_dev, s);
   if ((rc = debug_sync("k_reset", s))) return rc;
-  if (cbev_launch_render(e, e->head, F > 1 ? L - F + 1 : 0, s)) return CBEV_ERR_CUDA;
-  if ((rc = debug_sync("k_render (reset frame)", s))) return rc;
+  if (stamp ? cbev_launch_stamp(e, e->head, mirror, nullptr, nullptr, mask_dev, scene_ids_dev, s)
+            : cbev_launch_render(e, e->head, mirror, s))
+    return CBEV_ERR_CUDA;
+  if ((rc = debug_sync("reset frames", s))) return rc;
   CU_TRY(cudaGetLastError());
   e->was_reset = true;
   return CBEV_OK;
@@ -728,6 +776,9 @@
   CU_TRY(cudaEventCreateWithFlags(&e->ev_sim, cudaEventDisableTiming));
   CU_TRY(cudaEventCreateWithFlags(&e->ev_judge, cudaEventDisableTiming));
   CU_TRY(cudaEventCreateWithFlags(&e->ev_copy, cudaEventDisableTiming));
+  CU_TRY(cudaStreamCreateWithFlags(&e->stamp_stream, cudaStreamNonBlocking));
+  CU_TRY(cudaEventCreateWithFlags(&e->ev_head, cudaEventDisableTiming));
+  CU_TRY(cudaEventCreateWithFlags(&e->ev_stamp, cudaEventDisableTiming));
   return CBEV_OK;
 }
 
@@ -749,17 +800,29 @@
   int head = e->head + 1;
   if (head >= L) head = F - 1;
   const int mirror = F > 1 ? L - F + 1 : 0;
+  const bool stamp = cbev_uses_stamps(e) && e->cfg.autoreset == CBEV_AUTORESET_NEXT_STEP;
+  if (stamp && (rc = ensure_stamps(e, s))) return rc;
   const bool prof = e->profiling && e->prof_n < CBEV_PROF_MAX;
   cudaEvent_t* pe = prof ? e->prof_ev + CBEV_PROF_EVENTS * e->prof_n : nullptr;
   if (prof) cudaEventRecord(pe[0], s);
+  if (stamp) {
+    CU_TRY(cudaEventRecord(e->ev_head, s));
+    CU_TRY(cudaStreamWaitEvent(e->stamp_stream, e->ev_head, 0));
+  }
   cbev_launch_move(e, actions_dev, out, s);
   if (prof) cudaEventRecord(pe[1], s);
   if ((rc = debug_sync("k_move", s))) return rc;
+  if (stamp) {
+    if (cbev_launch_stamp(e, head, mirror, e->st.done, e->st.episode, nullptr, nullptr, e->stamp_stream)) return CBEV_ERR_CUDA;
+    CU_TRY(cudaEventRecord(e->ev_stamp, e->stamp_stream));
+    if ((rc = debug_sync("k_stamp", e->stamp_stream))) return rc;
+  }
   cudaStream_t js = (e->debug_flags & CBEV_DBG_JUDGE_SERIAL) ? s : e->side_stream;
   if (js != s) {
     CU_TRY(cudaEventRecord(e->ev_sim, s));
     CU_TRY(cudaStreamWaitEvent(js, e->ev_sim, 0));
   }
+  if (stamp) CU_TRY(cudaStreamWaitEvent(js, e->ev_stamp, 0));
   if (prof) cudaEventRecord(pe[3], js);
   cbev_launch_judge(e, out, js);
   if (prof) cudaEventRecord(pe[4], js);
@@ -1125,6 +1188,7 @@
   { int rc0 = use_device(e); if (rc0) return rc0; }
   CU_TRY(cudaDeviceSynchronize());
   dev_free(e->fov_mask);
+  e->stamps_valid = false;
   if (!mask_host) return CBEV_OK;
   const size_t n = (size_t)e->cfg.fov_size * e->cfg.fov_size;
   std::vector<uint8_t> m(n);
@@ -1292,6 +1356,7 @@
 
 int cbev_keep_fov(cbev_handle e, int32_t on) {
   if (!e) { cbev_set_error("null handle"); return CBEV_ERR_ARG; }
+  if (on && !e->keep_fov) e->stamps_valid = false;
   e->keep_fov = on != 0;
   return CBEV_OK;
 }
diff --git a/carlabev_env_b200/csrc/engine.h b/carlabev_env_b200/csrc/engine.h
--- a/carlabev_env_b200/csrc/engine.h
+++ b/carlabev_env_b200/csrc/engine.h
@@ -91,6 +91,7 @@
 
 struct SimParams {
   int32_t N, max_actors, max_rects, max_retreat;
+  int32_t reset_flags;
   int32_t map_w, map_h, fov, crop, pad, anchor_x, anchor_y;
   int32_t hero_w, win_max;
   float hero_scale;
@@ -100,6 +101,17 @@
   float discrete_table[16 * 3];
   cbev_config cfg;
 };
+
+__device__ __forceinline__ uint64_t splitmix64(uint64_t z) {
+  z += 0x9E3779B97F4A7C15ull;
+  z = (z ^ (z >> 30)) * 0xBF58476D1CE4E5B9ull;
+  z = (z ^ (z >> 27)) * 0x94D049BB133111EBull;
+  return z ^ (z >> 31);
+}
+__device__ __forceinline__ int cbev_autoreset_scene(uint64_t seed, int env, int episode, int n_scenes) {
+  const uint64_t h = splitmix64(seed + (uint64_t)env * 0x9E3779B97F4A7C15ull + (uint64_t)episode * 0xD1B54A32D192ED03ull);
+  return (int)(h % (uint64_t)n_scenes);
+}
 
 #define CBEV_RS_FAST96 0
 #define CBEV_RS_TABLE 1
@@ -156,6 +168,13 @@
   uint8_t *h_term_dev = nullptr, *h_trunc_dev = nullptr;
   cudaStream_t side_stream = nullptr;
   cudaEvent_t ev_sim = nullptr, ev_copy = nullptr, ev_judge = nullptr;
+  uint8_t* stamps = nullptr;
+  uint8_t* stamp_fov = nullptr;
+  int32_t stamp_rows = 0, stamp_stride = 0;
+  bool stamps_valid = false;
+  int num_sms = 0;
+  cudaStream_t stamp_stream = nullptr;
+  cudaEvent_t ev_head = nullptr, ev_stamp = nullptr;
   bool host_copy_pending = false;
   int64_t launches = 0;
   int64_t steps = 0;
@@ -187,10 +206,18 @@
   int32_t n_rows;
 };
 
+inline bool cbev_uses_stamps(const cbev_engine* e) {
+  return e->cfg.obs_mode != CBEV_OBS_RGB && e->cfg.fov_size <= 128;
+}
+
 void cbev_launch_reset(cbev_engine* e, const uint8_t* mask, const int32_t* scene_ids, cudaStream_t s);
 void cbev_launch_move(cbev_engine* e, const void* actions, const cbev_step_out* out, cudaStream_t s);
 void cbev_launch_judge(cbev_engine* e, const cbev_step_out* out, cudaStream_t s);
 int cbev_launch_render(cbev_engine* e, int32_t head, int32_t mirror, cudaStream_t s);
+void cbev_launch_stamp_desc(cbev_engine* e, int32_t* desc, cudaStream_t s);
+int cbev_launch_render_stamps(cbev_engine* e, const int32_t* desc, const uint32_t* rects, cudaStream_t s);
+int cbev_launch_stamp(cbev_engine* e, int32_t head, int32_t mirror, const uint8_t* done, const int32_t* episode,
+                      const uint8_t* mask, const int32_t* scene_ids, cudaStream_t s);
 void cbev_set_error(const char* fmt, ...);
 int cbev_launch_fuse(cbev_engine* e, int32_t mode, const void* ring, int32_t n, int32_t L, int32_t head, void* out,
                      cudaStream_t s);
diff --git a/carlabev_env_b200/csrc/render.cu b/carlabev_env_b200/csrc/render.cu
--- a/carlabev_env_b200/csrc/render.cu
+++ b/carlabev_env_b200/csrc/render.cu
@@ -78,6 +78,8 @@
   unsigned long long* trace;
   int32_t hero_w;
   int32_t nbx, nby, box_h, region_bytes;
+  uint8_t* stamp_out;
+  int32_t stamp_stride;
 };
 
 __device__ __forceinline__ void trace_mark(const RenderParams& P, int env, int slot) {
@@ -143,16 +145,53 @@
   return (uint32_t)(int)g & 255u;
 }
 
-template <int CHANNELS>
-__device__ __forceinline__ void store_u8_planes(uint8_t* base, const uint8_t* s_out, int plane, int tid, int nt) {
-  for (int q = tid; q < plane / 16; q += nt) {
-    const uint4 m = ((const uint4*)s_out)[q];
-#pragma unroll
-    for (int c = 0; c < CHANNELS; ++c)
-      st_u4(base + (size_t)c * plane + 16 * q,
-            make_uint4((m.x >> c) & 0x01010101u, (m.y >> c) & 0x01010101u, (m.z >> c) & 0x01010101u,
-                       (m.w >> c) & 0x01010101u));
-  }
+template <int OBS_MODE, int CHANNELS, bool U8, int B = 1>
+__device__ __forceinline__ void store_frame(uint8_t* base, const uint8_t* src, int plane, int count, int tid, int nt) {
+  if (U8 || OBS_MODE != CBEV_OBS_SEMANTIC) {
+    const int n = count / 16;
+    for (int q0 = tid; q0 < n; q0 += B * nt) {
+      uint4 m[B];
+#pragma unroll
+      for (int j = 0; j < B; ++j)
+        if (q0 + j * nt < n) m[j] = ((const uint4*)src)[q0 + j * nt];
+#pragma unroll
+      for (int j = 0; j < B; ++j) {
+        const int q = q0 + j * nt;
+        if (q >= n) break;
+        if (U8) {
+#pragma unroll
+          for (int c = 0; c < CHANNELS; ++c)
+            st_u4(base + (size_t)c * plane + 16 * q,
+                  make_uint4((m[j].x >> c) & 0x01010101u, (m[j].y >> c) & 0x01010101u, (m[j].z >> c) & 0x01010101u,
+                             (m[j].w >> c) & 0x01010101u));
+        } else {
+          st_u4(base + 16 * q, m[j]);
+        }
+      }
+    }
+  } else {
+    float* fb = (float*)base;
+    const int n = count / 4;
+    for (int q0 = tid; q0 < n; q0 += B * nt) {
+      uint32_t m4[B];
+#pragma unroll
+      for (int j = 0; j < B; ++j)
+        if (q0 + j * nt < n) m4[j] = ((const uint32_t*)src)[q0 + j * nt];
+#pragma unroll
+      for (int j = 0; j < B; ++j) {
+        const int q = q0 + j * nt;
+        if (q >= n) break;
+#pragma unroll
+        for (int c = 0; c < CHANNELS; ++c)
+          st_b4(fb + c * plane + 4 * q, bit_to_f32(m4[j], c), bit_to_f32(m4[j], c + 8), bit_to_f32(m4[j], c + 16),
+                bit_to_f32(m4[j], c + 24));
+      }
+    }
+  }
+}
+
+__device__ __forceinline__ void write_stamp(uint8_t* dst, const uint8_t* s_out, int plane, int tid, int nt) {
+  for (int q = tid; q < plane / 4; q += nt) ((uint32_t*)dst)[q] = ((const uint32_t*)s_out)[q];
 }
 
 __device__ __forceinline__ int fov_word(int row, int cw) { return row * 32 + ((((cw >> 2) ^ row) & 7) << 2) + (cw & 3); }
@@ -352,9 +391,6 @@
     for (int u = tid; u < S * S / 16; u += RT) dst[u] = *(const uint4*)(s_fov + fov_byte(u >> 3, (u & 7) << 4));
   }
 
-  const int F = P.frame_stack;
-  const int first = (flags & 1) ? P.head - F + 1 : P.head;
-
   if (OBS_MODE == CBEV_OBS_RGB) {
     uint32_t f[S * S / 4 / RT];
 #pragma unroll
@@ -439,32 +475,17 @@
   __syncthreads();
   }
 
+  if (P.stamp_out != nullptr) {
+    write_stamp(P.stamp_out + (size_t)env * P.stamp_stride, s_out, OH * OW, tid, RT);
+    return;
+  }
   trace_mark(P, env, 4);
-  for (int slot = first; slot <= P.head; ++slot) {
 #pragma unroll 1
-    for (int rep = 0; rep < 2; ++rep) {
-      int sl = slot;
-      if (rep == 1) {
-        sl = slot - P.mirror;
-        if (P.mirror <= 0 || sl < 0) break;
-      }
-      uint8_t* base = (uint8_t*)P.ring + ((size_t)env * P.ring_slots + sl) * P.frame_bytes;
-      if (U8) {
-        store_u8_planes<CHANNELS>(base, s_out, OH * OW, tid, RT);
-      } else if (OBS_MODE == CBEV_OBS_SEMANTIC) {
-        float* fb = (float*)base;
-        const int plane = OH * OW;
-        for (int q = tid; q < plane / 4; q += RT) {
-          const uint32_t m4 = ((const uint32_t*)s_out)[q];
-#pragma unroll
-          for (int c = 0; c < CHANNELS; ++c)
-            st_b4(fb + c * plane + 4 * q, bit_to_f32(m4, c), bit_to_f32(m4, c + 8), bit_to_f32(m4, c + 16),
-                  bit_to_f32(m4, c + 24));
-        }
-      } else {
-        for (int q = tid; q < OH * OW / 16; q += RT) st_u4(base + 16 * q, ((const uint4*)s_out)[q]);
-      }
-    }
+  for (int rep = 0; rep < 2; ++rep) {
+    const int sl = rep == 0 ? P.head : P.head - P.mirror;
+    if (rep == 1 && (P.mirror <= 0 || sl < 0)) break;
+    store_frame<OBS_MODE, CHANNELS, U8>((uint8_t*)P.ring + ((size_t)env * P.ring_slots + sl) * P.frame_bytes, s_out,
+                                        OH * OW, OH * OW, tid, RT);
   }
   trace_mark(P, env, 5);
 }
@@ -681,9 +702,6 @@
     uint4* dst = (uint4*)(P.fov_out + (size_t)env * S * S);
     for (int u = tid; u < S * cq; u += NT) dst[u] = *(const uint4*)(s_fov + (u >> cq_log) * FP + ((u & (cq - 1)) << 4));
   }
-
-  const int F = P.frame_stack;
-  const int first = (flags & 1) ? P.head - F + 1 : P.head;
 
   if (OBS_MODE == CBEV_OBS_RGB) {
     uint8_t* dst = (uint8_t*)P.ring + (size_t)env * P.ring_slots * P.frame_bytes + (size_t)P.head * P.frame_bytes;
@@ -947,31 +965,18 @@
   }
   __syncthreads();
 
+  if (P.stamp_out != nullptr) {
+    write_stamp(P.stamp_out + (size_t)env * P.stamp_stride, s_out, OH * OW, tid, NT);
+    return;
+  }
   trace_mark(P, env, 4);
-  for (int slot = first; slot <= P.head; ++slot) {
+  for (int slot = (flags & 1) ? P.head - P.frame_stack + 1 : P.head; slot <= P.head; ++slot) {
 #pragma unroll 1
     for (int rep = 0; rep < 2; ++rep) {
-      int sl = slot;
-      if (rep == 1) {
-        sl = slot - P.mirror;
-        if (P.mirror <= 0 || sl < 0) break;
-      }
-      uint8_t* base = (uint8_t*)P.ring + ((size_t)env * P.ring_slots + sl) * P.frame_bytes;
-      if (U8) {
-        store_u8_planes<CHANNELS>(base, s_out, OH * OW, tid, NT);
-      } else if (OBS_MODE == CBEV_OBS_SEMANTIC) {
-        float* fb = (float*)base;
-        const int plane = OH * OW;
-        for (int q = tid; q < plane / 4; q += NT) {
-          const uint32_t m4 = ((const uint32_t*)s_out)[q];
-#pragma unroll
-          for (int c = 0; c < CHANNELS; ++c)
-            st_b4(fb + c * plane + 4 * q, bit_to_f32(m4, c), bit_to_f32(m4, c + 8), bit_to_f32(m4, c + 16),
-                  bit_to_f32(m4, c + 24));
-        }
-      } else {
-        for (int q = tid; q < OH * OW / 16; q += NT) st_u4(base + 16 * q, ((const uint4*)s_out)[q]);
-      }
+      const int sl = rep == 0 ? slot : slot - P.mirror;
+      if (rep == 1 && (P.mirror <= 0 || sl < 0)) break;
+      store_frame<OBS_MODE, CHANNELS, U8>((uint8_t*)P.ring + ((size_t)env * P.ring_slots + sl) * P.frame_bytes, s_out,
+                                          OH * OW, OH * OW, tid, NT);
     }
   }
   trace_mark(P, env, 5);
@@ -1029,6 +1034,101 @@
 #pragma unroll
       for (int g = 0; g < 4; ++g) st_f4(o + 4 * g, u8_lane(v, 4 * g), u8_lane(v, 4 * g + 1), u8_lane(v, 4 * g + 2), u8_lane(v, 4 * g + 3));
     }
+  }
+}
+
+constexpr int STAMP_PIECES = 4;
+struct StampParams {
+  int32_t N, F, ring_slots, head, mirror, plane, stamp_stride, n_scenes, fov_bytes;
+  int64_t frame_bytes;
+  uint64_t seed;
+  const uint8_t* stamps;
+  const uint8_t* stamp_fov;
+  uint8_t* fov_out;
+  void* ring;
+  const uint8_t* done;
+  const int32_t* episode;
+  const uint8_t* mask;
+  const int32_t* scene_ids;
+};
+
+template <int OBS_MODE, int CHANNELS, bool U8>
+__global__ void __launch_bounds__(128) k_stamp(StampParams P) {
+  constexpr unsigned FULL = 0xffffffffu;
+  const int lane = threadIdx.x & 31;
+  const int nw = gridDim.x * (blockDim.x >> 5);
+  const int gw = blockIdx.x * (blockDim.x >> 5) + (threadIdx.x >> 5);
+  const uint8_t* flag = P.done != nullptr ? P.done : P.mask;
+  const int per_env = P.F * STAMP_PIECES;
+  const int piece = ((P.plane / 16 + STAMP_PIECES - 1) / STAMP_PIECES) * 16;
+  long long next = gw;
+  int base = 0;
+  for (int c0 = 0; c0 < P.N; c0 += 512) {
+    const int e0 = c0 + 16 * lane;
+    uint32_t m = 0;
+    if (flag == nullptr) {
+      m = e0 + 16 <= P.N ? 0xffffu : (e0 < P.N ? (1u << (P.N - e0)) - 1u : 0u);
+    } else if (e0 + 16 <= P.N && ((uintptr_t)(flag + e0) & 15) == 0) {
+      const uint4 v = *(const uint4*)(flag + e0);
+#pragma unroll
+      for (int b = 0; b < 16; ++b) m |= (((&v.x)[b >> 2] >> (8 * (b & 3))) & 255u) != 0 ? 1u << b : 0u;
+    } else {
+      for (int b = 0; b < 16 && e0 + b < P.N; ++b) m |= flag[e0 + b] != 0 ? 1u << b : 0u;
+    }
+    const int cnt = __popc(m);
+    int incl = cnt;
+#pragma unroll
+    for (int o = 1; o < 32; o <<= 1) {
+      const int t = __shfl_up_sync(FULL, incl, o);
+      if (lane >= o) incl += t;
+    }
+    const int excl = incl - cnt, total = __shfl_sync(FULL, incl, 31);
+    while (next < (long long)(base + total) * per_env) {
+      const int k = (int)(next / per_env) - base, f = (int)(next % per_env) / STAMP_PIECES;
+      const int b0 = (int)(next % STAMP_PIECES) * piece, nb = min(piece, P.plane - b0);
+      const int src = __ffs(__ballot_sync(FULL, k >= excl && k < incl)) - 1;
+      int env = lane == src ? e0 + (int)__fns(m, 0, k - excl + 1) : 0;
+      env = __shfl_sync(FULL, env, src);
+      const int scene = P.done != nullptr ? cbev_autoreset_scene(P.seed, env, P.episode[env], P.n_scenes)
+                                          : min(max(P.scene_ids[env], 0), P.n_scenes - 1);
+      const uint8_t* st = P.stamps + (size_t)scene * P.stamp_stride;
+      const int slot = P.head - P.F + 1 + f;
+#pragma unroll 1
+      for (int rep = 0; rep < 2; ++rep) {
+        const int sl = rep == 0 ? slot : slot - P.mirror;
+        if (rep == 1 && (P.mirror <= 0 || sl < 0)) break;
+        uint8_t* fr = (uint8_t*)P.ring + ((size_t)env * P.ring_slots + sl) * P.frame_bytes;
+        if (nb > 0)
+          store_frame<OBS_MODE, CHANNELS, U8, U8 || OBS_MODE != CBEV_OBS_SEMANTIC ? 4 : 8>(
+              fr + (size_t)b0 * (U8 || OBS_MODE != CBEV_OBS_SEMANTIC ? 1 : 4), st + b0, P.plane, nb, lane, 32);
+      }
+      if (f == P.F - 1 && b0 == 0 && P.fov_out != nullptr) {
+        const uint4* fs = (const uint4*)(P.stamp_fov + (size_t)scene * P.fov_bytes);
+        uint4* fd = (uint4*)(P.fov_out + (size_t)env * P.fov_bytes);
+        for (int u = lane; u < P.fov_bytes / 16; u += 32) fd[u] = fs[u];
+      }
+      next += nw;
+    }
+    base += total;
+  }
+}
+
+template <int MODE, int CH, bool U8>
+int stamp_kernel(cbev_engine* e, const StampParams& P, int blocks, cudaStream_t s) {
+  k_stamp<MODE, CH, U8><<<blocks, 128, 0, s>>>(P);
+  return 0;
+}
+
+template <bool U8>
+int stamp_semantic(cbev_engine* e, const StampParams& P, int blocks, cudaStream_t s) {
+  switch (e->channels) {
+    case 1: return stamp_kernel<CBEV_OBS_SEMANTIC, 1, U8>(e, P, blocks, s);
+    case 2: return stamp_kernel<CBEV_OBS_SEMANTIC, 2, U8>(e, P, blocks, s);
+    case 4: return stamp_kernel<CBEV_OBS_SEMANTIC, 4, U8>(e, P, blocks, s);
+    case 5: return stamp_kernel<CBEV_OBS_SEMANTIC, 5, U8>(e, P, blocks, s);
+    case 6: return stamp_kernel<CBEV_OBS_SEMANTIC, 6, U8>(e, P, blocks, s);
+    case 7: return stamp_kernel<CBEV_OBS_SEMANTIC, 7, U8>(e, P, blocks, s);
+    default: cbev_set_error("no stamp kernel for %d mask channels", e->channels); return 1;
   }
 }
 
@@ -1190,6 +1290,8 @@
   P.fov_out = e->keep_fov ? e->fov : nullptr;
   P.ring = e->ring;
   P.trace = (e->debug_flags & CBEV_DBG_TRACE) ? e->trace : nullptr;
+  P.stamp_out = nullptr;
+  P.stamp_stride = 0;
   return render_launch(e, P, s);
 }
 
@@ -1206,7 +1308,59 @@
   P.fov_out = nullptr;
   P.ring = windows;
   P.trace = nullptr;
+  P.stamp_out = nullptr;
+  P.stamp_stride = 0;
   return render_launch(e, P, s);
+}
+
+int cbev_launch_render_stamps(cbev_engine* e, const int32_t* desc, const uint32_t* rects, cudaStream_t s) {
+  RenderParams P;
+  P.N = e->pool.n_scenes;
+  P.ring_slots = 1;
+  P.head = 0;
+  P.mirror = 0;
+  P.desc = desc;
+  P.rects = rects;
+  P.order = nullptr;
+  P.order_cnt = nullptr;
+  P.fov_out = e->stamp_fov;
+  P.ring = nullptr;
+  P.trace = nullptr;
+  P.stamp_out = e->stamps;
+  P.stamp_stride = e->stamp_stride;
+  return render_launch(e, P, s);
+}
+
+int cbev_launch_stamp(cbev_engine* e, int32_t head, int32_t mirror, const uint8_t* done, const int32_t* episode,
+                      const uint8_t* mask, const int32_t* scene_ids, cudaStream_t s) {
+  StampParams P;
+  P.N = e->N;
+  P.F = e->cfg.frame_stack;
+  P.ring_slots = e->cfg.ring_slots;
+  P.head = head;
+  P.mirror = mirror;
+  P.plane = e->cfg.obs_h * e->cfg.obs_w;
+  P.stamp_stride = e->stamp_stride;
+  P.n_scenes = e->pool.n_scenes;
+  P.fov_bytes = e->cfg.fov_size * e->cfg.fov_size;
+  P.frame_bytes = e->frame_bytes;
+  P.seed = e->cfg.seed;
+  P.stamps = e->stamps;
+  P.stamp_fov = e->keep_fov ? e->stamp_fov : nullptr;
+  P.fov_out = e->keep_fov ? e->fov : nullptr;
+  P.ring = e->ring;
+  P.done = done;
+  P.episode = episode;
+  P.mask = mask;
+  P.scene_ids = scene_ids;
+  const int blocks = 4 * (e->num_sms > 0 ? e->num_sms : 148);
+  int rc = 0;
+  if (e->cfg.obs_mode == CBEV_OBS_GRAY) rc = stamp_kernel<CBEV_OBS_GRAY, 1, false>(e, P, blocks, s);
+  else if (e->cfg.obs_mode == CBEV_OBS_SEMANTIC_U8) rc = stamp_semantic<true>(e, P, blocks, s);
+  else if (e->cfg.obs_mode == CBEV_OBS_SEMANTIC) rc = stamp_semantic<false>(e, P, blocks, s);
+  else { cbev_set_error("no reset stamps for raw RGB frames (cbev_uses_stamps)"); rc = 1; }
+  if (rc == 0) e->launches += 1;
+  return rc;
 }
 
 int cbev_launch_fuse(cbev_engine* e, int32_t mode, const void* ring, int32_t n, int32_t L, int32_t head, void* out,
diff --git a/carlabev_env_b200/csrc/sim.cu b/carlabev_env_b200/csrc/sim.cu
--- a/carlabev_env_b200/csrc/sim.cu
+++ b/carlabev_env_b200/csrc/sim.cu
@@ -50,13 +50,6 @@
 
 __device__ __forceinline__ bool overlap(int ax, int ay, int aw, int bx, int by, int bw) {
   return ax < bx + bw && ay < by + bw && ax + aw > bx && ay + aw > by;
-}
-
-__device__ __forceinline__ uint64_t splitmix64(uint64_t z) {
-  z += 0x9E3779B97F4A7C15ull;
-  z = (z ^ (z >> 30)) * 0xBF58476D1CE4E5B9ull;
-  z = (z ^ (z >> 27)) * 0x94D049BB133111EBull;
-  return z ^ (z >> 31);
 }
 
 template <int G>
@@ -238,6 +231,13 @@
   }
 }
 
+__device__ void write_reset_header(const SimParams& P, const PoolDev& pool, int scene, int32_t* d, int flags) {
+  const double* s0 = pool.ego_state0 + (size_t)scene * 4;
+  View v;
+  compute_view(P, s0[0], s0[1], 0.0, v);
+  write_desc_header(P, d, v, 0, flags, crop_corner_class(P, v));
+}
+
 __device__ void reset_env(const SimParams& P, const PoolDev& pool, const EnvState& st, int env, int scene, int lane,
                           int stride = 32) {
   const int r0 = pool.ego_off[scene], nt = pool.ego_off[scene + 1] - r0;
@@ -265,7 +265,6 @@
     ei[I_OFFROAD] = 0;
     ei[I_STEP] = 0;
     st.scene[env] = scene;
-    st.done[env] = 0;
     for (int w = 0; w < CBEV_TGT_WORDS; ++w) {
       const int n = nt - 64 * w;
       st.tgt_vis[(size_t)env * CBEV_TGT_WORDS + w] = n >= 64 ? ~0ull : (n > 0 ? ((1ull << n) - 1ull) : 0ull);
@@ -292,11 +291,14 @@
   scene = min(max(scene, 0), pool.n_scenes - 1);
   reset_env(P, pool, st, env, scene, lane);
   if (lane == 0) {
-    const double* s0 = pool.ego_state0 + (size_t)scene * 4;
-    View v;
-    compute_view(P, s0[0], s0[1], 0.0, v);
-    write_desc_header(P, desc + (size_t)env * CBEV_DESC_WORDS, v, 0, 1, crop_corner_class(P, v));
-  }
+    st.done[env] = 0;
+    write_reset_header(P, pool, scene, desc + (size_t)env * CBEV_DESC_WORDS, 1);
+  }
+}
+
+__global__ void __launch_bounds__(128) k_stamp_desc(SimParams P, PoolDev pool, int32_t* __restrict__ desc) {
+  const int scene = blockIdx.x * blockDim.x + threadIdx.x;
+  if (scene < pool.n_scenes) write_reset_header(P, pool, scene, desc + (size_t)scene * CBEV_DESC_WORDS, 0);
 }
 
 __device__ void start_retreat(const PoolDev& pool, double* rbuf, int32_t* rn, int ga, Body& b, int& tidx, int& rxlen) {
@@ -544,17 +546,13 @@
 template <int G>
 __device__ __forceinline__ void auto_reset_env(const SimParams& P, const PoolDev& pool, const EnvState& st, const cbev_step_out& out,
                                             int32_t* d, int32_t* order, int32_t* order_cnt, int env, int lane, unsigned GM) {
-  int ep = st.episode[env];
-  uint64_t h = splitmix64(P.seed + (uint64_t)env * 0x9E3779B97F4A7C15ull + (uint64_t)ep * 0xD1B54A32D192ED03ull);
-  int scene = (int)(h % (uint64_t)pool.n_scenes);
+  const int scene = cbev_autoreset_scene(P.seed, env, st.episode[env], pool.n_scenes);
   __syncwarp(GM);
   reset_env(P, pool, st, env, scene, lane, G);
   if (lane == 0) {
     order[atomicAdd(order_cnt, 1)] = env;
     const double* s0 = pool.ego_state0 + (size_t)scene * 4;
-    View v;
-    compute_view(P, s0[0], s0[1], 0.0, v);
-    write_desc_header(P, d, v, 0, 1, crop_corner_class(P, v));
+    write_reset_header(P, pool, scene, d, P.reset_flags);
     out.reward[env] = 0.0;
     out.terminated[env] = 0;
     out.truncated[env] = 0;
@@ -1151,7 +1149,10 @@
   const int lane = g.lane, env = g.env;
   if (env >= P.N) return;
   if (desc[(size_t)env * CBEV_DESC_WORDS + RD_FLAGS] & 1) {
-    if (lane == 0) move_order[P.N - 1 - atomicAdd(move_cnt + 1, 1)] = env;
+    if (lane == 0) {
+      st.done[env] = 0;
+      move_order[P.N - 1 - atomicAdd(move_cnt + 1, 1)] = env;
+    }
     return;
   }
   double reward;
@@ -1365,6 +1366,7 @@
   P.max_actors = e->cfg.max_actors;
   P.max_rects = e->max_rects;
   P.max_retreat = e->pool.max_retreat;
+  P.reset_flags = cbev_uses_stamps(e) ? 3 : 1;
   P.map_w = e->map_w;
   P.map_h = e->map_h;
   P.fov = e->cfg.fov_size;
@@ -1393,6 +1395,12 @@
   e->launches += 1;
 }
 
+void cbev_launch_stamp_desc(cbev_engine* e, int32_t* desc, cudaStream_t s) {
+  SimParams P = make_params(e);
+  k_stamp_desc<<<(e->pool.n_scenes + 127) / 128, 128, 0, s>>>(P, e->pool, desc);
+  e->launches += 1;
+}
+
 static bool narrow_groups(const cbev_engine* e) {
   return e->pool.max_actors <= 8 || e->pool.traj_steps > 0;
 }
```

Result: faster. 22.84 million, median of 6 (+4.4%).
